# Quantco/tabmat

Hardware: AMD Instinct MI355X
Metric: SplitMatrix.sandwich GFLOP/s + effective HBM GB/s, 10M×1k mixed (higher is better)
Workload: dtype f64; 1 GPU; SplitMatrix.sandwich: dense128 + csr512@5% + cats(256,96,32), 10000000 rows/GPU, p=1024, float64 (BASELINE configs[3]); rows_per_gpu=10000000, p=1024, launch=eager, collective=none

## Files before the change

include/tabmat_hip.h:

```cpp
#ifndef TABMAT_HIP_H
#define TABMAT_HIP_H

#include <stddef.h>
#include <stdint.h>

#ifdef __cplusplus
extern "C" {
#endif

#define TM_OK 0
#define TM_EINVAL (-1)
#define TM_ENOMEM (-2)
#define TM_EUNSUPPORTED (-3)

int tm_version(void);
const char *tm_last_error(void);
int tm_device_count(int *count);
int tm_set_device(int device);
int tm_device_info(char *name, int name_len, int *compute_units, int64_t *hbm_bytes);
int tm_malloc(void **ptr, size_t bytes);
int tm_free(void *ptr);
int tm_memcpy_h2d(void *dst, const void *h_src, size_t bytes, void *stream);
int tm_memcpy_d2h(void *h_dst, const void *src, size_t bytes, void *stream);
int tm_memset(void *dst, int value, size_t bytes, void *stream);
// ... 408 lines not shown
                                    float *out, void *stream);
int tm_multi_cat_dense_sandwich_f64(const void *const *h_codes, const int64_t *h_ncols,
                                    const int32_t *h_drop_first, int n_cats, int64_t n,
                                    const double *d, const double *M, int64_t M_ncol, int order_f,
                                    double *out, void *stream);
int tm_multi_cat_dense_sandwich_rows_f32(const void *const *h_codes, const int64_t *h_ncols,
                                         const int32_t *h_drop_first, int n_cats, int64_t n,
                                         const float *d, const float *M, int64_t M_ncol,
                                         const int32_t *rows, int64_t n_rows, float *out,
                                         void *stream);
int tm_multi_cat_dense_sandwich_rows_f64(const void *const *h_codes, const int64_t *h_ncols,
                                         const int32_t *h_drop_first, int n_cats, int64_t n,
                                         const double *d, const double *M, int64_t M_ncol,
                                         const int32_t *rows, int64_t n_rows, double *out,
                                         void *stream);
int tm_multi_cat_sparse_sandwich_rows_f32(const void *const *h_codes, const int64_t *h_ncols,
                                          const int32_t *h_drop_first, int n_cats,
                                          const float *cm_data, const int32_t *cm_indices,
                                          const int32_t *row_ranges, const int32_t *rows,
                                          int64_t n_sel, int64_t m, const float *d_sel, float *out,
                                          void *stream);
int tm_multi_cat_sparse_sandwich_rows_f64(const void *const *h_codes, const int64_t *h_ncols,
                                          const int32_t *h_drop_first, int n_cats,
                                          const double *cm_data, const int32_t *cm_indices,
                                          const int32_t *row_ranges, const int32_t *rows,
                                          int64_t n_sel, int64_t m, const double *d_sel, double *out,
                                          void *stream);
int tm_multi_cat_sparse_sandwich_rows_u8_f32(const void *const *h_codes, const int64_t *h_ncols,
                                             const int32_t *h_drop_first, int n_cats,
                                             const float *cm_data, const uint8_t *cm_col8,
                                             const int32_t *row_ranges, const int32_t *rows,
                                             int64_t n_sel, int64_t m, const float *d_sel, float *out,
                                             void *stream);
int tm_multi_cat_sparse_sandwich_rows_u8_f64(const void *const *h_codes, const int64_t *h_ncols,
                                             const int32_t *h_drop_first, int n_cats,
                                             const double *cm_data, const uint8_t *cm_col8,
                                             const int32_t *row_ranges, const int32_t *rows,
                                             int64_t n_sel, int64_t m, const double *d_sel, double *out,
                                             void *stream);
int tm_multi_cat_sparse_sandwich_ent_f32(const void *const *h_codes, const int64_t *h_ncols,
                                         const int32_t *h_drop_first, int n_cats, int64_t n, const float *d,
                                         const float *vals, const uint16_t *meta, const uint32_t *bstart,
                                         int64_t n_slots, int64_t mk, float *out, void *stream);
int tm_multi_cat_sparse_sandwich_ent_f64(const void *const *h_codes, const int64_t *h_ncols,
                                         const int32_t *h_drop_first, int n_cats, int64_t n, const double *d,
                                         const double *vals, const uint16_t *meta, const uint32_t *bstart,
                                         int64_t n_slots, int64_t mk, double *out, void *stream);
int tm_multi_cat_pack_codes(const void *const *h_codes, const int64_t *h_ncols, const int32_t *h_drop_first, int n_cats,
                            int64_t n, uint32_t *packed, void *stream);
int tm_multi_cat_sparse_sandwich_entp_f32(const void *const *h_codes, const int64_t *h_ncols,
                                          const int32_t *h_drop_first, int n_cats, int64_t n, const float *d,
                                          const float *vals, const uint16_t *meta, const uint32_t *bstart,
                                          int64_t n_slots, int64_t mk, const uint32_t *packed, float *out, void *stream);
int tm_multi_cat_sparse_sandwich_entp_f64(const void *const *h_codes, const int64_t *h_ncols,
                                          const int32_t *h_drop_first, int n_cats, int64_t n, const double *d,
                                          const double *vals, const uint16_t *meta, const uint32_t *bstart,
                                          int64_t n_slots, int64_t mk, const uint32_t *packed, double *out, void *stream);

int tm_multi_cat_sparse_sandwich_slab_f32(const void *const *h_codes, const int64_t *h_ncols,
                                          const int32_t *h_drop_first, int n_cats, int64_t n,
                                          const float *d, const float *vals, const uint32_t *koff,
                                          const uint8_t *ecol, const int64_t *gptr, int64_t m,
                                          float *out, void *stream);
int tm_multi_cat_sparse_sandwich_slab_f64(const void *const *h_codes, const int64_t *h_ncols,
                                          const int32_t *h_drop_first, int n_cats, int64_t n,
                                          const double *d, const double *vals, const uint32_t *koff,
                                          const uint8_t *ecol, const int64_t *gptr, int64_t m,
                                          double *out, void *stream);

int tm_multi_cat_pairs_max_bins(void);
int tm_multi_cat_pairs_max_slots(void);
int tm_multi_cat_pairs_row_words(void);
int tm_multi_cat_pairs_f32(const int64_t *cat_tab, int64_t n, const float *d, const int32_t *rows,
                           int64_t n_rows, const int32_t *bundles, int n_bundles,
                           const int32_t *wg_map, int n_wg, int slots, int64_t bins,
                           const int64_t *desc, int64_t n_pairs, const int64_t *pos, double *tables,
                           double *out, int64_t p, void *stream);
int tm_multi_cat_pairs_f64(const int64_t *cat_tab, int64_t n, const double *d, const int32_t *rows,
                           int64_t n_rows, const int32_t *bundles, int n_bundles,
                           const int32_t *wg_map, int n_wg, int slots, int64_t bins,
                           const int64_t *desc, int64_t n_pairs, const int64_t *pos, double *tables,
                           double *out, int64_t p, void *stream);

int tm_multi_cat_matvec_f32(const int64_t *cat_tab, int n_cats, const int64_t *pos, const float *v,
                            int64_t n, float *out, void *stream);
int tm_multi_cat_matvec_f64(const int64_t *cat_tab, int n_cats, const int64_t *pos, const double *v,
                            int64_t n, double *out, void *stream);

int tm_csr_densify_cols_f32(const float *data, const int32_t *indices, const int64_t *indptr, int64_t n,
                            const int32_t *colmap, float *T, int64_t ld, void *stream);
int tm_csr_densify_cols_f64(const double *data, const int32_t *indices, const int64_t *indptr, int64_t n,
                            const int32_t *colmap, double *T, int64_t ld, void *stream);
int tm_csc_densify_cols_f32(const int32_t *rows, const float *vals, const int64_t *seg, const int32_t *tcol,
                            int64_t n_sel, int64_t max_len, float *T, int64_t ld, void *stream);
int tm_csc_densify_cols_f64(const int32_t *rows, const double *vals, const int64_t *seg, const int32_t *tcol,
                            int64_t n_sel, int64_t max_len, double *T, int64_t ld, void *stream);
int tm_dense_gather_cols_f32(const float *X, int64_t n, int64_t m, int order_f, const int32_t *cols,
                             int64_t n_sel, float *T, int64_t ld, int64_t t0, void *stream);
int tm_dense_gather_cols_f64(const double *X, int64_t n, int64_t m, int order_f, const int32_t *cols,
                             int64_t n_sel, double *T, int64_t ld, int64_t t0, void *stream);

int tm_scatter_block_f32(const float *src, int64_t nr, int64_t nc, const int64_t *ri,
                         const int64_t *ci, double *out, int64_t p, int mirror, int diag,
                         void *stream);
int tm_scatter_block_f64(const double *src, int64_t nr, int64_t nc, const int64_t *ri,
                         const int64_t *ci, double *out, int64_t p, int mirror, int diag,
                         void *stream);

int tm_sparse_sandwich_chunked_rows_f32(const float *cm_data, const int32_t *cm_indices,
                                        const int32_t *row_ranges, int64_t n_sel, int64_t m,
                                        int64_t nnz, const float *d_sel, float *out, void *stream);
int tm_sparse_sandwich_chunked_rows_f64(const double *cm_data, const int32_t *cm_indices,
                                        const int32_t *row_ranges, int64_t n_sel, int64_t m,
                                        int64_t nnz, const double *d_sel, double *out, void *stream);

int tm_sparse_sandwich_chunked_u8_f32(const float *cm_data, const uint8_t *cm_col8, const int32_t *cptr, int64_t n,
                                      int64_t m, int64_t nnz, const float *d, float *out, void *stream);
int tm_sparse_sandwich_chunked_u8_f64(const double *cm_data, const uint8_t *cm_col8, const int32_t *cptr, int64_t n,
                                      int64_t m, int64_t nnz, const double *d, double *out, void *stream);
int tm_sparse_sandwich_chunked_rows_u8_f32(const float *cm_data, const uint8_t *cm_col8, const int32_t *row_ranges,
                                           int64_t n_sel, int64_t m, int64_t nnz, const float *d_sel, float *out,
                                           void *stream);
int tm_sparse_sandwich_chunked_rows_u8_f64(const double *cm_data, const uint8_t *cm_col8, const int32_t *row_ranges,
                                           int64_t n_sel, int64_t m, int64_t nnz, const double *d_sel, double *out,
                                           void *stream);
int tm_sparse_sandwich_direct_f32(const float *csr_data, const int32_t *csr_indices,
                                  const int64_t *csr_indptr, int64_t n, int64_t m, const float *d,
                                  float *out, void *stream);
int tm_sparse_sandwich_direct_f64(const double *csr_data, const int32_t *csr_indices,
                                  const int64_t *csr_indptr, int64_t n, int64_t m, const double *d,
                                  double *out, void *stream);
int tm_csr_dense_sandwich_rows_f32(const float *cm_data, const int32_t *cm_indices,
                                   const int32_t *row_ranges, int64_t n_sel, const int32_t *rows,
                                   const float *d_sel, int64_t n, int64_t m, const float *B, int64_t r,
                                   int order_f, float *out, void *stream);
int tm_csr_dense_sandwich_rows_f64(const double *cm_data, const int32_t *cm_indices,
                                   const int32_t *row_ranges, int64_t n_sel, const int32_t *rows,
                                   const double *d_sel, int64_t n, int64_t m, const double *B, int64_t r,
                                   int order_f, double *out, void *stream);
int tm_csr_dense_sandwich_rows_u8_f32(const float *cm_data, const uint8_t *cm_col8,
                                      const int32_t *row_ranges, int64_t n_sel, const int32_t *rows,
                                      const float *d_sel, int64_t n, int64_t m, const float *B, int64_t r,
                                      int order_f, float *out, void *stream);
int tm_csr_dense_sandwich_rows_u8_f64(const double *cm_data, const uint8_t *cm_col8,
                                      const int32_t *row_ranges, int64_t n_sel, const int32_t *rows,
                                      const double *d_sel, int64_t n, int64_t m, const double *B, int64_t r,
                                      int order_f, double *out, void *stream);

int tm_cat_det_block_rows(void);
int tm_cat_transpose_matvec_det_f32(const int32_t *perm, const int64_t *bstart, int64_t n_blocks,
                                    const int64_t *cat_bptr, int64_t n_cols, const float *v,
                                    float *out, int accumulate, void *stream);
int tm_cat_transpose_matvec_det_f64(const int32_t *perm, const int64_t *bstart, int64_t n_blocks,
                                    const int64_t *cat_bptr, int64_t n_cols, const double *v,
                                    double *out, int accumulate, void *stream);

int tm_cat_dense_sandwich_sorted_f32(const int32_t *perm, const int64_t *bstart, int64_t n_blocks,
                                     const int64_t *cat_bptr, int64_t n_cols, const float *d,
                                     const float *Y, int64_t m, float *out, void *stream);
int tm_cat_dense_sandwich_sorted_f64(const int32_t *perm, const int64_t *bstart, int64_t n_blocks,
                                     const int64_t *cat_bptr, int64_t n_cols, const double *d,
                                     const double *Y, int64_t m, double *out, void *stream);
int tm_csc_dense_sandwich_sorted_f32(const int32_t *rows, const float *vals, const int64_t *bstart,
                                     int64_t n_blocks, const int64_t *col_bptr, int64_t n_cols,
                                     const float *d, const float *Y, int64_t m, float *out,
                                     void *stream);
// ... 56 lines not shown
```

tabmat_amd/csrc/cat.hip:

```cpp
#include <algorithm>

#include "common.hpp"
#include "reduce.hpp"

namespace tmh {

__global__ void fill_i32_kernel(int32_t *p, int64_t n, int32_t v) {
    int64_t i = (int64_t)blockIdx.x * blockDim.x + threadIdx.x;
    if (i < n) p[i] = v;
}

__global__ void scatter_iota_i32_kernel(int32_t *map, const int32_t *cols, int64_t n_cols) {
    int64_t i = (int64_t)blockIdx.x * blockDim.x + threadIdx.x;
    if (i < n_cols) map[cols[i]] = (int32_t)i;
}

int build_col_map(int32_t *map, int64_t m, const int32_t *cols, int64_t n_cols, hipStream_t st) {
    if (m > 0) {
        hipLaunchKernelGGL(fill_i32_kernel, dim3((unsigned)ceil_div(m, 256)), dim3(256), 0, st, map,
                           m, -1);
        TM_LAUNCH_CHECK();
    }
    if (n_cols > 0) {
        hipLaunchKernelGGL(scatter_iota_i32_kernel, dim3((unsigned)ceil_div(n_cols, 256)),
                           dim3(256), 0, st, map, cols, n_cols);
        TM_LAUNCH_CHECK();
    }
    return TM_OK;
}

template <typename F, bool TWO>
__global__ __launch_bounds__(1024) void hist_lds_kernel(
    const int32_t *__restrict__ ci, const int32_t *__restrict__ cj, const F *__restrict__ w,
    const int32_t *__restrict__ rows, int64_t n_iter, int64_t rows_per_block, int drop_i,
    int drop_j, int i_ncol, int j_ncol, int ti, const int32_t *__restrict__ col_map,
    F *__restrict__ ws, int64_t stride) {
    extern __shared__ __attribute__((aligned(16))) unsigned char smem_raw[];
    lds_acc_t *bins = reinterpret_cast<lds_acc_t *>(smem_raw);
    const int part = blockIdx.y;
    const int i0 = part * ti;
    const int i1 = min(i0 + ti, i_ncol);
    const int nbins = TWO ? (i1 - i0) * j_ncol : (i1 - i0);
    for (int b = threadIdx.x; b < nbins; b += blockDim.x) bins[b] = 0.0;
    __syncthreads();

    const int64_t t0 = (int64_t)blockIdx.x * rows_per_block;
    const int64_t t1 = min(t0 + rows_per_block, n_iter);
    int64_t tbeg = t0;
    if (!TWO && rows == nullptr && (t0 & 3) == 0 &&
        ((reinterpret_cast<uintptr_t>(ci) | reinterpret_cast<uintptr_t>(w)) & 15) == 0) {
        typedef int i4 __attribute__((ext_vector_type(4)));
        const int64_t nvec = (t1 - t0) / 4;
        for (int64_t q = threadIdx.x; q < nvec; q += blockDim.x) {
            const int64_t k = t0 + q * 4;
            const i4 cc = *reinterpret_cast<const i4 *>(ci + k);
            F ww[4];
#pragma unroll
            for (int e = 0; e < 4; ++e) ww[e] = w[k + e];
#pragma unroll
            for (int e = 0; e < 4; ++e) {
                const int c = cc[e] - drop_i;
                if (c >= i0 && c < i1 && !(col_map && col_map[c] < 0)) atomic_add(&bins[c - i0], (lds_acc_t)ww[e]);
            }
        }
        tbeg = t0 + nvec * 4;
    }
    for (int64_t t = tbeg + threadIdx.x; t < t1; t += blockDim.x) {
        const int64_t k = rows ? (int64_t)rows[t] : t;
        const int c = ci[k] - drop_i;
        if (c < i0 || c >= i1) continue;
        if (TWO) {
            const int c2 = cj[k] - drop_j;
            if (c2 < 0) continue;
            atomic_add(&bins[(c - i0) * j_ncol + c2], (lds_acc_t)w[k]);
        } else {
            if (col_map && col_map[c] < 0) continue;
            atomic_add(&bins[c - i0], (lds_acc_t)w[k]);
        }
    }
    __syncthreads();
    F *dst = ws + ((int64_t)part * gridDim.x + blockIdx.x) * stride;
    for (int b = threadIdx.x; b < nbins; b += blockDim.x) dst[b] = (F)bins[b];
}

template <typename F, bool TWO>
__global__ __launch_bounds__(256) void hist_global_kernel(
// ... 1137 lines not shown
        }
    }
    __syncthreads();
    F *dst = ws + ((int64_t)blockIdx.y * gridDim.x + blockIdx.x) * stride;
    for (int b = threadIdx.x; b < cs.total * GC; b += blockDim.x)
        dst[b] = (F)tile[(b / GC) * TSTR + (b % GC)];
}

template <typename F, typename IX>
__global__ __launch_bounds__(1024) void multi_cat_sparse_rows_kernel(
    CatSet cs, const F *__restrict__ cm_data, const IX *__restrict__ cm_ind,
    const int32_t *__restrict__ ranges, const int32_t *__restrict__ rows, const F *__restrict__ d_sel,
    int64_t n_sel, int64_t rows_per_block, F *__restrict__ ws, int64_t stride) {
    constexpr int GC = 32;
    extern __shared__ __attribute__((aligned(16))) unsigned char smem_raw[];
    lds_acc_t *tile = reinterpret_cast<lds_acc_t *>(smem_raw);
    constexpr int tstr = GC + 1;
    const int nel = cs.total * tstr;
    for (int b = threadIdx.x; b < nel; b += blockDim.x) tile[b] = 0.0;
    __syncthreads();
    static_assert(SPARSE_CHUNK_COLS == 4 * GC, "the chunk of the chunk-major twin must hold four 32-column groups");
    const int g = blockIdx.y;
    const int ch = g >> 2;
    const int lane = threadIdx.x & 63, wave = threadIdx.x >> 6, nwave = blockDim.x >> 6;
    const int lr = lane >> 3, lt = lane & 7;
    const int64_t t0 = (int64_t)blockIdx.x * rows_per_block;
    const int64_t t1 = min(t0 + rows_per_block, n_sel);
    const int32_t *rg = ranges + (int64_t)ch * n_sel * 2;
    for (int64_t k0 = t0 + wave * 8; k0 < t1; k0 += (int64_t)nwave * 8) {
        const int64_t k = k0 + lr;
        if (k >= t1) continue;
        const F dk = d_sel[k];
        if (dk == F(0)) continue;
        const int e0 = rg[2 * k], e1 = rg[2 * k + 1];
        if (e0 >= e1) continue;
        const int64_t row = rows[k];
        int off[MAX_CATS];
#pragma unroll
        for (int c = 0; c < MAX_CATS; ++c) {
            off[c] = -1;
            if (c < cs.n_cats) {
                const int col = cs.codes[c][row] - cs.drop[c];
                off[c] = col >= 0 ? (cs.off[c] + col) * tstr : -1;
            }
        }
        for (int e = e0 + lt; e < e1; e += 8) {
            const int col = (int)cm_ind[e] - (sizeof(IX) == 1 ? (g & 3) : g) * GC;
            if (col < 0 || col >= GC) continue;
            const lds_acc_t x = (lds_acc_t)(dk * cm_data[e]);
#pragma unroll
            for (int c = 0; c < MAX_CATS; ++c)
                if (off[c] >= 0) atomic_add(&tile[off[c] + col], x);
        }
    }
    __syncthreads();
    F *dst = ws + ((int64_t)blockIdx.y * gridDim.x + blockIdx.x) * stride;
    for (int b = threadIdx.x; b < cs.total * GC; b += blockDim.x)
        dst[b] = (F)tile[(b / GC) * tstr + (b % GC)];
}

static int make_catset(const void *const *h_codes, const int64_t *h_ncols, const int32_t *h_drop,
                       int n_cats, CatSet *cs) {
    if (n_cats < 1 || n_cats > MAX_CATS) {
        set_error("multi-cat call supports 1..%d categoricals, got %d", MAX_CATS, n_cats);
        return TM_EINVAL;
    }
    int off = 0;
    for (int c = 0; c < MAX_CATS; ++c) {
        cs->codes[c] = c < n_cats ? reinterpret_cast<const int32_t *>(h_codes[c]) : nullptr;
        cs->ncol[c] = c < n_cats ? (int)h_ncols[c] : 0;
        cs->drop[c] = c < n_cats ? h_drop[c] : 0;
        cs->off[c] = off;
        off += cs->ncol[c];
    }
    cs->n_cats = n_cats;
    cs->total = off;
    return TM_OK;
}

template <typename F>
static int run_multi_cat_dense(const void *const *h_codes, const int64_t *h_ncols,
                               const int32_t *h_drop, int n_cats, int64_t n, const F *d, const F *M,
                               int64_t m, int order_f, F *out, hipStream_t st,
                               const int32_t *rows = nullptr, int64_t n_rows = 0) {
    CatSet cs;
    int rc = make_catset(h_codes, h_ncols, h_drop, n_cats, &cs);
    if (rc) return rc;
    const int64_t total = (int64_t)cs.total * m;
    if (total == 0) return TM_OK;
    if (rows != nullptr) n = n_rows;
    if (n == 0) {
        TM_HIP(hipMemsetAsync(out, 0, sizeof(F) * (size_t)total, st));
        return TM_OK;
    }
    {
        constexpr int VEC = MCW_VEC;
        constexpr int TJW = 16 * VEC;
        const size_t tile_b = ((sizeof(lds_acc_t) * (size_t)cs.total * TJW + 15) / 16) * 16;
        const size_t lds_w = tile_b + (size_t)16 * MCW_RS * (sizeof(F) + (size_t)n_cats * sizeof(int));
        if (!order_f && n_cats <= 8 && m >= VEC && m % VEC == 0 &&
            (reinterpret_cast<uintptr_t>(M) & 15) == 0 && lds_w <= 150 * 1024 &&
            (int64_t)cs.total * TJW * (int64_t)sizeof(lds_acc_t) < (1ll << 30)) {
            const int64_t n_parts = ceil_div(m, TJW);
            const int64_t stride = (int64_t)cs.total * TJW;
            int64_t nblk = std::max<int64_t>(1, tune("catdense_rounds", 1) * NUM_CU / n_parts);
            nblk = std::min<int64_t>(nblk, std::max<int64_t>(1, ceil_div(n, 4096)));
            const int64_t rpb = ceil_div(ceil_div(n, nblk), MCW_RS) * MCW_RS;
            nblk = ceil_div(n, rpb);
            const size_t tmp_bytes = ((sizeof(F) * (size_t)(n_parts * stride) + 255) / 256) * 256;
            void *wsv = nullptr;
            rc = get_workspace(tmp_bytes + sizeof(F) * (size_t)(n_parts * nblk * stride) + 256, &wsv, st);
            if (rc) return rc;
            F *tmp = reinterpret_cast<F *>(wsv);
            F *ws = reinterpret_cast<F *>(reinterpret_cast<char *>(wsv) + tmp_bytes);
            auto gow = [&](auto kern) -> int {
                TM_HIP(hipFuncSetAttribute(reinterpret_cast<const void *>(kern),
                                           hipFuncAttributeMaxDynamicSharedMemorySize, (int)lds_w));
                prof_begin(st);
                const int nw_dflt = (sizeof(F) == 8 && tile_b > 64 * 1024) ? 8 : 16;
                const int nw = (int)std::min<int64_t>(16, std::max<int64_t>(4, tune("catdense_waves", nw_dflt)));
                hipLaunchKernelGGL(kern, dim3((unsigned)nblk, (unsigned)n_parts), dim3(nw * 64), lds_w, st,
                                   cs, d, M, n, m, rpb, ws, stride, rows, wg_log_ptr());
                prof_end(st);
                TM_LAUNCH_CHECK();
                return TM_OK;
            };
            if (n_cats == 1) rc = gow(&multi_cat_dense_wide_kernel<F, 1>);
            else if (n_cats == 2) rc = gow(&multi_cat_dense_wide_kernel<F, 2>);
            else if (n_cats == 3) rc = gow(&multi_cat_dense_wide_kernel<F, 3>);
            else if (n_cats == 4) rc = gow(&multi_cat_dense_wide_kernel<F, 4>);
            else if (n_cats == 5) rc = gow(&multi_cat_dense_wide_kernel<F, 5>);
            else if (n_cats == 6) rc = gow(&multi_cat_dense_wide_kernel<F, 6>);
            else if (n_cats == 7) rc = gow(&multi_cat_dense_wide_kernel<F, 7>);
            else rc = gow(&multi_cat_dense_wide_kernel<F, 8>);
            if (rc) return rc;
            rc = launch_reduce_partials<F>(ws, stride, (int)nblk, (int)n_parts, tmp, n_parts * stride,
                                           false, st);
            if (rc) return rc;
            hipLaunchKernelGGL((multi_cat_untile_kernel<F>), dim3((unsigned)ceil_div(total, 256)),
                               dim3(256), 0, st, tmp, (int64_t)cs.total, m, TJW, out);
            TM_LAUNCH_CHECK();
            return TM_OK;
        }
    }
    if (rows != nullptr) {
        set_error("multi_cat_dense: the row-list form needs the wide-load path");
        return TM_EUNSUPPORTED;
    }
    int TJ = 64;
    while (TJ > 1 && sizeof(lds_acc_t) * (size_t)cs.total * TJ > HIST_LDS_MAX) TJ >>= 1;
    while (TJ > 1 && TJ / 2 >= m) TJ >>= 1;
    if (sizeof(lds_acc_t) * (size_t)cs.total * TJ > HIST_LDS_MAX) {
        set_error("multi_cat_dense: %d stacked categories exceed the LDS tile", cs.total);
        return TM_EUNSUPPORTED;
    }
    const int64_t n_parts = ceil_div(m, TJ);
    const int64_t stride = (int64_t)cs.total * TJ;
    const size_t lds = sizeof(lds_acc_t) * (size_t)stride;
    int64_t nblk = std::max<int64_t>(1, NUM_CU / n_parts);
    nblk = std::min<int64_t>(nblk, std::max<int64_t>(1, ceil_div(n, 4096)));
    const int64_t rpb = ceil_div(n, nblk);
    nblk = ceil_div(n, rpb);
    const size_t tmp_bytes = ((sizeof(F) * (size_t)(n_parts * stride) + 255) / 256) * 256;
    void *wsv = nullptr;
    rc = get_workspace(tmp_bytes + sizeof(F) * (size_t)(n_parts * nblk * stride) + 256, &wsv, st);
    if (rc) return rc;
    F *tmp = reinterpret_cast<F *>(wsv);
    F *ws = reinterpret_cast<F *>(reinterpret_cast<char *>(wsv) + tmp_bytes);
    auto go = [&](auto kern) -> int {
        if (lds > 48 * 1024)
            TM_HIP(hipFuncSetAttribute(reinterpret_cast<const void *>(kern),
                                       hipFuncAttributeMaxDynamicSharedMemorySize, (int)lds));
        prof_begin(st);
        hipLaunchKernelGGL(kern, dim3((unsigned)nblk, (unsigned)n_parts), dim3(1024), lds, st, cs, d,
                           M, n, m, rpb, ws, stride);
        prof_end(st);
        TM_LAUNCH_CHECK();
        return TM_OK;
    };
#define TM_MCD_CASE(V)                                                                       \
    case V:                                                                                  \
        if (order_f) rc = go(&multi_cat_dense_f_kernel<F, V>);                               \
        else if (n_cats == 1) rc = go(&multi_cat_dense_c_kernel<F, V, 1>);                   \
        else if (n_cats == 2) rc = go(&multi_cat_dense_c_kernel<F, V, 2>);                   \
        else if (n_cats == 3) rc = go(&multi_cat_dense_c_kernel<F, V, 3>);                   \
        else if (n_cats == 4) rc = go(&multi_cat_dense_c_kernel<F, V, 4>);                   \
        else rc = go(&multi_cat_dense_c_kernel<F, V, 0>);                                    \
        break;
    switch (TJ) {
        TM_MCD_CASE(64)
        TM_MCD_CASE(32)
        TM_MCD_CASE(16)
        TM_MCD_CASE(8)
        TM_MCD_CASE(4)
        TM_MCD_CASE(2)
        TM_MCD_CASE(1)
        default:
            rc = TM_EINVAL;
    }
#undef TM_MCD_CASE
    if (rc) return rc;
    rc = launch_reduce_partials<F>(ws, stride, (int)nblk, (int)n_parts, tmp, n_parts * stride, false,
                                   st);
    if (rc) return rc;
    hipLaunchKernelGGL((multi_cat_untile_kernel<F>), dim3((unsigned)ceil_div(total, 256)),
                       dim3(256), 0, st, tmp, (int64_t)cs.total, m, TJ, out);
    TM_LAUNCH_CHECK();
    return TM_OK;
}

template <typename F, typename IX>
static int run_multi_cat_sparse_rows(const void *const *h_codes, const int64_t *h_ncols,
                                     const int32_t *h_drop, int n_cats, const F *cm_data,
                                     const IX *cm_ind, const int32_t *ranges, const int32_t *rows,
                                     int64_t n_sel, int64_t m, const F *d_sel, F *out, hipStream_t st);

template <typename F>
static int run_multi_cat_sparse(const void *const *h_codes, const int64_t *h_ncols,
                                const int32_t *h_drop, int n_cats, int64_t n, const F *d,
                                const F *vals, const unsigned *koff, const unsigned char *ecol,
                                const int64_t *gptr, int64_t m, int slab_rows, int group_cols,
                                F *out, hipStream_t st) {
    CatSet cs;
    int rc = make_catset(h_codes, h_ncols, h_drop, n_cats, &cs);
    if (rc) return rc;
    const int64_t total = (int64_t)cs.total * m;
    if (total == 0) return TM_OK;
    if (n == 0) {
        TM_HIP(hipMemsetAsync(out, 0, sizeof(F) * (size_t)total, st));
        return TM_OK;
    }
    const int64_t stride = (int64_t)cs.total * group_cols;
    const size_t tile_bytes = ((sizeof(lds_acc_t) * (size_t)cs.total * (group_cols + 1) + 15) / 16) * 16;
    if (tile_bytes > HIST_LDS_MAX) {
        set_error("multi_cat_sparse: %d stacked categories exceed the LDS tile", cs.total);
        return TM_EUNSUPPORTED;
    }
    const int nw = (int)std::min<int64_t>(16, std::max<int64_t>(4, tune("catsparse_waves", 16)));
    const size_t stage_bytes = (size_t)nw * slab_rows * (sizeof(F) + sizeof(int32_t) * (size_t)n_cats);
    const bool stage = tile_bytes + stage_bytes <= 150 * 1024;
    const size_t lds = tile_bytes + (stage ? stage_bytes : 0);
    const int n_groups = (int)ceil_div(m, group_cols);
    const int64_t n_slabs = ceil_div(n, slab_rows);
    int64_t nblk = std::max<int64_t>(1, tune("catsparse_rounds", 1) * NUM_CU / n_groups);
    nblk = std::min<int64_t>(nblk, n_slabs);
    const int64_t spb = ceil_div(n_slabs, nblk);
    nblk = ceil_div(n_slabs, spb);
    const size_t tmp_bytes = ((sizeof(F) * (size_t)(n_groups * stride) + 255) / 256) * 256;
    void *wsv = nullptr;
    rc = get_workspace(tmp_bytes + sizeof(F) * (size_t)((int64_t)n_groups * nblk * stride) + 256,
                       &wsv, st);
    if (rc) return rc;
    F *tmp = reinterpret_cast<F *>(wsv);
    F *ws = reinterpret_cast<F *>(reinterpret_cast<char *>(wsv) + tmp_bytes);
    if (stage && n_cats <= 8 && slab_rows == 128) {
        auto kpf = n_cats == 1   ? &multi_cat_sparse_pf_kernel<F, 1>
                   : n_cats == 2 ? &multi_cat_sparse_pf_kernel<F, 2>
                   : n_cats == 3 ? &multi_cat_sparse_pf_kernel<F, 3>
                   : n_cats == 4 ? &multi_cat_sparse_pf_kernel<F, 4>
                   : n_cats == 5 ? &multi_cat_sparse_pf_kernel<F, 5>
                   : n_cats == 6 ? &multi_cat_sparse_pf_kernel<F, 6>
                   : n_cats == 7 ? &multi_cat_sparse_pf_kernel<F, 7>
                                 : &multi_cat_sparse_pf_kernel<F, 8>;
        if (lds > 48 * 1024)
            TM_HIP(hipFuncSetAttribute(reinterpret_cast<const void *>(kpf),
                                       hipFuncAttributeMaxDynamicSharedMemorySize, (int)lds));
        prof_begin(st);
        hipLaunchKernelGGL(kpf, dim3((unsigned)nblk, (unsigned)n_groups), dim3(nw * 64), lds, st, cs, d,
                           vals, koff, ecol, gptr, n_groups, n_slabs, spb, group_cols, n, ws, stride,
                           wg_log_ptr());
        prof_end(st);
        TM_LAUNCH_CHECK();
    } else {
        auto kern = stage ? &multi_cat_sparse_kernel<F, true> : &multi_cat_sparse_kernel<F, false>;
        if (lds > 48 * 1024)
            TM_HIP(hipFuncSetAttribute(reinterpret_cast<const void *>(kern),
                                       hipFuncAttributeMaxDynamicSharedMemorySize, (int)lds));
        prof_begin(st);
        hipLaunchKernelGGL(kern, dim3((unsigned)nblk, (unsigned)n_groups), dim3(nw * 64), lds, st, cs,
                           d, vals, koff, ecol, gptr, n_groups, n_slabs, spb, slab_rows, group_cols,
                           n, ws, stride);
        prof_end(st);
        TM_LAUNCH_CHECK();
    }
    rc = launch_reduce_partials<F>(ws, stride, (int)nblk, n_groups, tmp,
                                   (int64_t)n_groups * stride, false, st);
    if (rc) return rc;
    hipLaunchKernelGGL((multi_cat_untile_kernel<F>), dim3((unsigned)ceil_div(total, 256)),
                       dim3(256), 0, st, tmp, (int64_t)cs.total, m, group_cols, out);
    TM_LAUNCH_CHECK();
    return TM_OK;
}

__global__ __launch_bounds__(256) void multi_cat_pack_codes_kernel(CatSet cs, int64_t n, unsigned *__restrict__ out) {
    for (int64_t r = (int64_t)blockIdx.x * blockDim.x + threadIdx.x; r < n; r += (int64_t)gridDim.x * blockDim.x) {
        unsigned pk = 0u;
#pragma unroll
        for (int c = 0; c < 3; ++c) {
            unsigned f = 1023u;
            if (c < cs.n_cats) {
                const int col = cs.codes[c][r] - cs.drop[c];
                if (col >= 0 && col < cs.ncol[c]) f = (unsigned)(cs.off[c] + col);
            }
            pk |= f << (10 * c);
        }
        out[r] = pk;
    }
}

template <typename F>
static int run_multi_cat_sparse_ent(const void *const *h_codes, const int64_t *h_ncols, const int32_t *h_drop,
                                    int n_cats, int64_t n, const F *d, const F *vals, const unsigned short *meta,
                                    const unsigned *bstart, int64_t mk, F *out, hipStream_t st,
                                    const unsigned *packed = nullptr, int64_t n_slots = 0) {
    CatSet cs;
    int rc = make_catset(h_codes, h_ncols, h_drop, n_cats, &cs);
    if (rc) return rc;
    const int64_t total = (int64_t)cs.total * mk;
    if (total == 0) return TM_OK;
    if (n == 0) {
        TM_HIP(hipMemsetAsync(out, 0, sizeof(F) * (size_t)total, st));
        return TM_OK;
    }
    TM_REQUIRE(mk % 16 == 0 && n_cats >= 1 && n_cats <= 8, "kernel columns in groups of 16, 1 .. 8 categoricals");
    TM_REQUIRE(n < (1ll << 28), "at most 2^28 - 1 rows per block");
    constexpr int GC = 32;
    const int64_t stride = (int64_t)cs.total * GC;
    const size_t lds = ((sizeof(lds_acc_t) * (size_t)cs.total * (GC + 1) + 15) / 16) * 16;
    if (lds > HIST_LDS_MAX) {
        set_error("multi_cat_sparse_ent: %d stacked categories exceed the LDS tile", cs.total);
        return TM_EUNSUPPORTED;
    }
    const int nw = (int)std::min<int64_t>(16, std::max<int64_t>(4, tune("catsparse_waves", 16)));
    const int n_groups = (int)(mk / 16);
    const int n_pairs = (n_groups + 1) / 2;
    const int64_t n_slabs = ceil_div(n, 64);
    int64_t nblk = std::max<int64_t>(1, tune("catsparse_rounds", 1) * NUM_CU / n_pairs);
    nblk = std::min<int64_t>(nblk, n_slabs);
    const int64_t spb = ceil_div(n_slabs, nblk);
    nblk = ceil_div(n_slabs, spb);
    const size_t tmp_bytes = ((sizeof(F) * (size_t)(n_pairs * stride) + 255) / 256) * 256;
    void *wsv = nullptr;
    rc = get_workspace(tmp_bytes + sizeof(F) * (size_t)((int64_t)n_pairs * nblk * stride) + 256, &wsv, st);
    if (rc) return rc;
    F *tmp = reinterpret_cast<F *>(wsv);
    F *ws = reinterpret_cast<F *>(reinterpret_cast<char *>(wsv) + tmp_bytes);
    auto kern = n_cats == 1   ? &multi_cat_sparse_ent_kernel<F, 1>
                : n_cats == 2 ? &multi_cat_sparse_ent_kernel<F, 2>
                : n_cats == 3 ? &multi_cat_sparse_ent_kernel<F, 3>
                : n_cats == 4 ? &multi_cat_sparse_ent_kernel<F, 4>
                : n_cats == 5 ? &multi_cat_sparse_ent_kernel<F, 5>
                : n_cats == 6 ? &multi_cat_sparse_ent_kernel<F, 6>
                : n_cats == 7 ? &multi_cat_sparse_ent_kernel<F, 7>
                              : &multi_cat_sparse_ent_kernel<F, 8>;
    TM_REQUIRE(packed == nullptr || (n_cats <= 3 && cs.total < 1023), "packed codes: at most 3 categoricals, 1022 levels");
    const int ncw = packed != nullptr ? 1 : n_cats;
    const size_t lds_staged = lds + (size_t)nw * 64 * (sizeof(F) + 4 * (size_t)ncw);
    const double fill = (double)n_slots / ((double)std::max(n_groups, 1) * (double)n_slabs);
    if (tune("catsparse_staged", 1) != 0 && lds_staged <= 156 * 1024 &&
        fill >= (double)tune("catsparse_staged_fill", 44)) {
        using KS = void (*)(CatSet, const F *, const F *, const unsigned short *, const unsigned *, int, int64_t, int64_t,
                            int64_t, F *, int64_t, const unsigned *, int);
        KS ks = nullptr;
        if (packed != nullptr) {
            ks = n_cats == 1 ? &multi_cat_sparse_ent_staged_kernel<F, 1, true>
                 : n_cats == 2 ? &multi_cat_sparse_ent_staged_kernel<F, 2, true>
                               : &multi_cat_sparse_ent_staged_kernel<F, 3, true>;
        } else {
            ks = n_cats == 1   ? &multi_cat_sparse_ent_staged_kernel<F, 1, false>
                 : n_cats == 2 ? &multi_cat_sparse_ent_staged_kernel<F, 2, false>
                 : n_cats == 3 ? &multi_cat_sparse_ent_staged_kernel<F, 3, false>
                 : n_cats == 4 ? &multi_cat_sparse_ent_staged_kernel<F, 4, false>
                 : n_cats == 5 ? &multi_cat_sparse_ent_staged_kernel<F, 5, false>
                 : n_cats == 6 ? &multi_cat_sparse_ent_staged_kernel<F, 6, false>
                 : n_cats == 7 ? &multi_cat_sparse_ent_staged_kernel<F, 7, false>
                               : &multi_cat_sparse_ent_staged_kernel<F, 8, false>;
        }
        if (lds_staged > 48 * 1024)
            TM_HIP(hipFuncSetAttribute(reinterpret_cast<const void *>(ks),
                                       hipFuncAttributeMaxDynamicSharedMemorySize, (int)lds_staged));
        prof_begin(st);
        hipLaunchKernelGGL(ks, dim3((unsigned)nblk, (unsigned)n_pairs), dim3(nw * 64), lds_staged, st, cs, d, vals,
                           meta, bstart, n_groups, n, n_slabs, spb, ws, stride, packed, (int)lds);
        prof_end(st);
        TM_LAUNCH_CHECK();
    } else {
        if (lds > 48 * 1024)
            TM_HIP(hipFuncSetAttribute(reinterpret_cast<const void *>(kern),
                                       hipFuncAttributeMaxDynamicSharedMemorySize, (int)lds));
        prof_begin(st);
        hipLaunchKernelGGL(kern, dim3((unsigned)nblk, (unsigned)n_pairs), dim3(nw * 64), lds, st, cs, d, vals, meta,
                           bstart, n_groups, n, n_slabs, spb, ws, stride, packed);
        prof_end(st);
        TM_LAUNCH_CHECK();
    }
    rc = launch_reduce_partials<F>(ws, stride, (int)nblk, n_pairs, tmp, (int64_t)n_pairs * stride, false, st);
    if (rc) return rc;
    hipLaunchKernelGGL((multi_cat_untile_kernel<F>), dim3((unsigned)ceil_div(total, 256)), dim3(256), 0, st, tmp,
                       (int64_t)cs.total, mk, GC, out);
    TM_LAUNCH_CHECK();
    return TM_OK;
}

}

using namespace tmh;

#define TM_CHECK_COMMON(nn) \
    TM_REQUIRE((nn) >= 0, "negative size")

extern "C" {

int tm_cat_transpose_matvec_f32(const int32_t *codes, int64_t n, int64_t n_cols, int drop_first,
                                const float *v, const int32_t *rows, int64_t n_rows,
                                const int32_t *cols, int64_t n_cols_sel, float *out, void *stream) {
    TM_CHECK_COMMON(n);
    return run_cat_tmv<float>(codes, n, n_cols, drop_first, v, rows, n_rows, cols, n_cols_sel, out,
                              as_stream(stream));
}
int tm_cat_transpose_matvec_f64(const int32_t *codes, int64_t n, int64_t n_cols, int drop_first,
                                const double *v, const int32_t *rows, int64_t n_rows,
                                const int32_t *cols, int64_t n_cols_sel, double *out,
                                void *stream) {
    TM_CHECK_COMMON(n);
    return run_cat_tmv<double>(codes, n, n_cols, drop_first, v, rows, n_rows, cols, n_cols_sel,
                               out, as_stream(stream));
}

int tm_cat_matvec_f32(const int32_t *codes, int64_t n, int64_t n_cols, int drop_first,
                      const float *v, const int32_t *cols, int64_t n_cols_sel, float *out,
                      void *stream) {
    TM_CHECK_COMMON(n);
    return run_cat_matvec<float>(codes, n, n_cols, drop_first, v, cols, n_cols_sel, out,
                                 as_stream(stream));
}
int tm_cat_matvec_f64(const int32_t *codes, int64_t n, int64_t n_cols, int drop_first,
                      const double *v, const int32_t *cols, int64_t n_cols_sel, double *out,
                      void *stream) {
    TM_CHECK_COMMON(n);
    return run_cat_matvec<double>(codes, n, n_cols, drop_first, v, cols, n_cols_sel, out,
                                  as_stream(stream));
}

int tm_cat_matvec_assign_f32(const int32_t *codes, int64_t n, int64_t n_cols, int drop_first,
                             const float *v, const int32_t *cols, int64_t n_cols_sel, float *out,
                             void *stream) {
    TM_CHECK_COMMON(n);
    return run_cat_matvec<float>(codes, n, n_cols, drop_first, v, cols, n_cols_sel, out,
                                 as_stream(stream), true);
}
int tm_cat_matvec_assign_f64(const int32_t *codes, int64_t n, int64_t n_cols, int drop_first,
                             const double *v, const int32_t *cols, int64_t n_cols_sel, double *out,
                             void *stream) {
    TM_CHECK_COMMON(n);
    return run_cat_matvec<double>(codes, n, n_cols, drop_first, v, cols, n_cols_sel, out,
                                  as_stream(stream), true);
}

int tm_cat_cat_sandwich_f32(const int32_t *i_codes, const int32_t *j_codes, int64_t n,
                            const float *d, const int32_t *rows, int64_t n_rows, int64_t i_ncol,
                            int64_t j_ncol, int i_drop_first, int j_drop_first, float *out,
                            void *stream) {
    TM_CHECK_COMMON(n);
    return run_hist<float, true>(i_codes, j_codes, d, rows, rows ? n_rows : n, i_drop_first,
                                 j_drop_first, i_ncol, j_ncol, nullptr, out, false,
                                 as_stream(stream));
}
int tm_cat_cat_sandwich_f64(const int32_t *i_codes, const int32_t *j_codes, int64_t n,
                            const double *d, const int32_t *rows, int64_t n_rows, int64_t i_ncol,
                            int64_t j_ncol, int i_drop_first, int j_drop_first, double *out,
                            void *stream) {
    TM_CHECK_COMMON(n);
    return run_hist<double, true>(i_codes, j_codes, d, rows, rows ? n_rows : n, i_drop_first,
                                  j_drop_first, i_ncol, j_ncol, nullptr, out, false,
                                  as_stream(stream));
}

int tm_cat_cat_sandwich_atomic_f32(const int32_t *i_codes, const int32_t *j_codes, int64_t n,
// ... 30 lines not shown
                                   as_stream(stream));
}

int tm_cat_dense_sandwich_f32(const int32_t *codes, int64_t n, int64_t i_ncol, int drop_first,
                              const float *d, const int32_t *rows, int64_t n_rows, const float *M,
                              int64_t M_ncol, int order_f, const int32_t *j_cols, int64_t n_j,
                              float *out, void *stream) {
    TM_CHECK_COMMON(n);
    return run_cat_dense<float>(codes, n, i_ncol, drop_first, d, rows, n_rows, M, M_ncol, order_f,
                                j_cols, j_cols ? n_j : M_ncol, out, as_stream(stream));
}
int tm_cat_dense_sandwich_f64(const int32_t *codes, int64_t n, int64_t i_ncol, int drop_first,
                              const double *d, const int32_t *rows, int64_t n_rows,
                              const double *M, int64_t M_ncol, int order_f, const int32_t *j_cols,
                              int64_t n_j, double *out, void *stream) {
    TM_CHECK_COMMON(n);
    return run_cat_dense<double>(codes, n, i_ncol, drop_first, d, rows, n_rows, M, M_ncol, order_f,
                                 j_cols, j_cols ? n_j : M_ncol, out, as_stream(stream));
}

int tm_cat_sparse_sandwich_f32(const int32_t *codes, int64_t n, int64_t i_ncol, int drop_first,
                               const float *csr_data, const int32_t *csr_indices,
                               const int64_t *csr_indptr, int64_t s_ncol, const float *d,
                               const int32_t *rows, int64_t n_rows, const int32_t *cols,
                               int64_t n_cols, float *out, void *stream) {
    TM_CHECK_COMMON(n);
    return run_cat_sparse<float>(codes, n, i_ncol, drop_first, csr_data, csr_indices, csr_indptr,
                                 s_ncol, d, rows, n_rows, cols, n_cols, out, as_stream(stream));
}
int tm_cat_sparse_sandwich_f64(const int32_t *codes, int64_t n, int64_t i_ncol, int drop_first,
                               const double *csr_data, const int32_t *csr_indices,
                               const int64_t *csr_indptr, int64_t s_ncol, const double *d,
                               const int32_t *rows, int64_t n_rows, const int32_t *cols,
                               int64_t n_cols, double *out, void *stream) {
    TM_CHECK_COMMON(n);
    return run_cat_sparse<double>(codes, n, i_ncol, drop_first, csr_data, csr_indices, csr_indptr,
                                  s_ncol, d, rows, n_rows, cols, n_cols, out, as_stream(stream));
}

int tm_multi_cat_dense_sandwich_f32(const void *const *h_codes, const int64_t *h_ncols,
                                    const int32_t *h_drop_first, int n_cats, int64_t n,
                                    const float *d, const float *M, int64_t M_ncol, int order_f,
                                    float *out, void *stream) {
    return run_multi_cat_dense<float>(h_codes, h_ncols, h_drop_first, n_cats, n, d, M, M_ncol,
                                      order_f, out, as_stream(stream));
}
int tm_multi_cat_dense_sandwich_f64(const void *const *h_codes, const int64_t *h_ncols,
                                    const int32_t *h_drop_first, int n_cats, int64_t n,
                                    const double *d, const double *M, int64_t M_ncol, int order_f,
                                    double *out, void *stream) {
    return run_multi_cat_dense<double>(h_codes, h_ncols, h_drop_first, n_cats, n, d, M, M_ncol,
                                       order_f, out, as_stream(stream));
}
int tm_multi_cat_dense_sandwich_rows_f32(const void *const *h_codes, const int64_t *h_ncols,
                                         const int32_t *h_drop_first, int n_cats, int64_t n,
                                         const float *d, const float *M, int64_t M_ncol,
                                         const int32_t *rows, int64_t n_rows, float *out,
                                         void *stream) {
    return run_multi_cat_dense<float>(h_codes, h_ncols, h_drop_first, n_cats, n, d, M, M_ncol, 0, out,
                                      as_stream(stream), rows, n_rows);
}
int tm_multi_cat_dense_sandwich_rows_f64(const void *const *h_codes, const int64_t *h_ncols,
                                         const int32_t *h_drop_first, int n_cats, int64_t n,
                                         const double *d, const double *M, int64_t M_ncol,
                                         const int32_t *rows, int64_t n_rows, double *out,
                                         void *stream) {
    return run_multi_cat_dense<double>(h_codes, h_ncols, h_drop_first, n_cats, n, d, M, M_ncol, 0, out,
                                       as_stream(stream), rows, n_rows);
}
int tm_multi_cat_sparse_sandwich_ent_f32(const void *const *h_codes, const int64_t *h_ncols,
                                         const int32_t *h_drop_first, int n_cats, int64_t n, const float *d,
                                         const float *vals, const uint16_t *meta, const uint32_t *bstart,
                                         int64_t n_slots, int64_t mk, float *out, void *stream) {
    return run_multi_cat_sparse_ent<float>(h_codes, h_ncols, h_drop_first, n_cats, n, d, vals, meta, bstart, mk,
                                           out, as_stream(stream), nullptr, n_slots);
}
int tm_multi_cat_sparse_sandwich_ent_f64(const void *const *h_codes, const int64_t *h_ncols,
                                         const int32_t *h_drop_first, int n_cats, int64_t n, const double *d,
                                         const double *vals, const uint16_t *meta, const uint32_t *bstart,
                                         int64_t n_slots, int64_t mk, double *out, void *stream) {
    return run_multi_cat_sparse_ent<double>(h_codes, h_ncols, h_drop_first, n_cats, n, d, vals, meta, bstart, mk,
                                            out, as_stream(stream), nullptr, n_slots);
}
int tm_multi_cat_pack_codes(const void *const *h_codes, const int64_t *h_ncols, const int32_t *h_drop_first, int n_cats,
                            int64_t n, uint32_t *packed, void *stream) {
    CatSet cs;
    int rc = make_catset(h_codes, h_ncols, h_drop_first, n_cats, &cs);
    if (rc) return rc;
    TM_REQUIRE(n_cats <= 3 && cs.total < 1023, "packed codes: at most 3 categoricals, 1022 stacked levels");
    if (n == 0) return TM_OK;
    hipLaunchKernelGGL(multi_cat_pack_codes_kernel, dim3((unsigned)std::min<int64_t>(4 * NUM_CU, ceil_div(n, 256))),
                       dim3(256), 0, as_stream(stream), cs, n, packed);
    TM_LAUNCH_CHECK();
    return TM_OK;
}
int tm_multi_cat_sparse_sandwich_entp_f32(const void *const *h_codes, const int64_t *h_ncols,
                                          const int32_t *h_drop_first, int n_cats, int64_t n, const float *d,
                                          const float *vals, const uint16_t *meta, const uint32_t *bstart,
                                          int64_t n_slots, int64_t mk, const uint32_t *packed, float *out, void *stream) {
    return run_multi_cat_sparse_ent<float>(h_codes, h_ncols, h_drop_first, n_cats, n, d, vals, meta, bstart, mk, out,
                                           as_stream(stream), packed, n_slots);
}
int tm_multi_cat_sparse_sandwich_entp_f64(const void *const *h_codes, const int64_t *h_ncols,
                                          const int32_t *h_drop_first, int n_cats, int64_t n, const double *d,
                                          const double *vals, const uint16_t *meta, const uint32_t *bstart,
                                          int64_t n_slots, int64_t mk, const uint32_t *packed, double *out, void *stream) {
    return run_multi_cat_sparse_ent<double>(h_codes, h_ncols, h_drop_first, n_cats, n, d, vals, meta, bstart, mk,
                                            out, as_stream(stream), packed, n_slots);
}
int tm_multi_cat_sparse_sandwich_slab_f32(const void *const *h_codes, const int64_t *h_ncols,
                                          const int32_t *h_drop_first, int n_cats, int64_t n,
                                          const float *d, const float *vals, const uint32_t *koff,
                                          const uint8_t *ecol, const int64_t *gptr, int64_t m,
                                          float *out, void *stream) {
    return run_multi_cat_sparse<float>(h_codes, h_ncols, h_drop_first, n_cats, n, d, vals, koff,
                                       ecol, gptr, m, tm_slab_rows(), tm_slab_group_cols(), out,
                                       as_stream(stream));
}
int tm_multi_cat_sparse_sandwich_slab_f64(const void *const *h_codes, const int64_t *h_ncols,
                                          const int32_t *h_drop_first, int n_cats, int64_t n,
                                          const double *d, const double *vals, const uint32_t *koff,
                                          const uint8_t *ecol, const int64_t *gptr, int64_t m,
                                          double *out, void *stream) {
    return run_multi_cat_sparse<double>(h_codes, h_ncols, h_drop_first, n_cats, n, d, vals, koff,
                                        ecol, gptr, m, tm_slab_rows(), tm_slab_group_cols(), out,
                                        as_stream(stream));
}

}

namespace tmh {
template <typename F, typename IX>
static int run_multi_cat_sparse_rows(const void *const *h_codes, const int64_t *h_ncols,
                                     const int32_t *h_drop, int n_cats, const F *cm_data,
                                     const IX *cm_ind, const int32_t *ranges, const int32_t *rows,
                                     int64_t n_sel, int64_t m, const F *d_sel, F *out, hipStream_t st) {
    CatSet cs;
    int rc = make_catset(h_codes, h_ncols, h_drop, n_cats, &cs);
    if (rc) return rc;
    const int64_t total = (int64_t)cs.total * m;
    if (total == 0) return TM_OK;
    if (n_sel == 0) {
        TM_HIP(hipMemsetAsync(out, 0, sizeof(F) * (size_t)total, st));
        return TM_OK;
    }
    constexpr int GC = 32;
    const size_t lds = ((sizeof(lds_acc_t) * (size_t)cs.total * (GC + 1) + 15) / 16) * 16;
    if (lds > HIST_LDS_MAX) {
        set_error("multi_cat_sparse_rows: %d stacked categories exceed the LDS tile", cs.total);
        return TM_EUNSUPPORTED;
    }
    const int n_groups = (int)ceil_div(m, GC);
    const int64_t stride = (int64_t)cs.total * GC;
    int64_t nblk = std::max<int64_t>(1, tune("catsparse_rounds", 1) * NUM_CU / n_groups);
    nblk = std::min<int64_t>(nblk, std::max<int64_t>(1, ceil_div(n_sel, 2048)));
    const int64_t rpb = ceil_div(n_sel, nblk);
    nblk = ceil_div(n_sel, rpb);
    const size_t tmp_bytes = ((sizeof(F) * (size_t)(n_groups * stride) + 255) / 256) * 256;
    void *wsv = nullptr;
    rc = get_workspace(tmp_bytes + sizeof(F) * (size_t)((int64_t)n_groups * nblk * stride) + 256, &wsv, st);
    if (rc) return rc;
    F *tmp = reinterpret_cast<F *>(wsv);
    F *ws = reinterpret_cast<F *>(reinterpret_cast<char *>(wsv) + tmp_bytes);
    auto kern = &multi_cat_sparse_rows_kernel<F, IX>;
    if (lds > 48 * 1024)
        TM_HIP(hipFuncSetAttribute(reinterpret_cast<const void *>(kern),
// ... 58 lines not shown
```

tabmat_amd/csrc/cat_pairs.hip:

```cpp
#include "common.hpp"
#include "reduce.hpp"

namespace tmh {

constexpr int CP_BINS = 16384;
constexpr int CP_SLOTS = 16;
constexpr int CP_ROW = 8 + 4 * CP_SLOTS;
constexpr int CP_NEG = -(1 << 28);

template <typename F, int NS>
__global__ __launch_bounds__(1024) void multi_cat_pairs_kernel(
    const int64_t *__restrict__ cat_tab, const F *__restrict__ d, const int32_t *__restrict__ rows,
    int64_t n_iter, const int32_t *__restrict__ bundles, const int32_t *__restrict__ wg_map,
    int max_bins, double *__restrict__ ws) {
    extern __shared__ double tile[];
    const int y = __builtin_amdgcn_readfirstlane(wg_map[blockIdx.x]);
    const int32_t *br = bundles + (int64_t)y * CP_ROW;
    const int na = __builtin_amdgcn_readfirstlane(br[0]), nb = __builtin_amdgcn_readfirstlane(br[1]);
    const int mode = __builtin_amdgcn_readfirstlane(br[2]), lbs = __builtin_amdgcn_readfirstlane(br[3]);
    const int wg0 = __builtin_amdgcn_readfirstlane(br[4]);
    const int bins = __builtin_amdgcn_readfirstlane(br[6]);
    const int parts = (int)min((int64_t)__builtin_amdgcn_readfirstlane(br[5]),
                               max((int64_t)1, (n_iter + 8191) / 8192));
    const int part = (int)blockIdx.x - wg0;
    if (part >= parts) return;
    for (int b = threadIdx.x; b < bins; b += blockDim.x) tile[b] = 0.0;
    __syncthreads();
    const int32_t *pa[NS], *pb[NS];
    int dropa[NS], dropb[NS], offa[NS], offb[NS];
    static_for<NS>([&](auto sc) {
        constexpr int s = decltype(sc)::value;
        pa[s] = pb[s] = nullptr;
        dropa[s] = dropb[s] = offa[s] = offb[s] = 0;
        if (s < na) {
            const int id = __builtin_amdgcn_readfirstlane(br[8 + 2 * s]);
            offa[s] = __builtin_amdgcn_readfirstlane(br[9 + 2 * s]);
            pa[s] = reinterpret_cast<const int32_t *>(cat_tab[4 * id]);
            dropa[s] = (int)cat_tab[4 * id + 1];
        }
        if (s < nb) {
            const int id = __builtin_amdgcn_readfirstlane(br[8 + 2 * CP_SLOTS + 2 * s]);
            offb[s] = __builtin_amdgcn_readfirstlane(br[9 + 2 * CP_SLOTS + 2 * s]);
            pb[s] = reinterpret_cast<const int32_t *>(cat_tab[4 * id]);
            dropb[s] = (int)cat_tab[4 * id + 1];
        }
    });
    constexpr int UNR = NS <= 8 ? 4 : 2;
    const int64_t rpp = (n_iter + parts - 1) / parts;
    const int64_t t0 = (int64_t)part * rpp, t1 = min(t0 + rpp, n_iter);
    for (int64_t tb = t0; tb < t1; tb += (int64_t)UNR * blockDim.x) {
        int64_t k[UNR], kc[UNR];
        double dk[UNR];
        int ya[UNR][NS], xb[UNR][NS];
#pragma unroll
        for (int u = 0; u < UNR; ++u) {
            const int64_t t = tb + (int64_t)u * blockDim.x + threadIdx.x;
            k[u] = t < t1 ? (rows ? (int64_t)rows[t] : t) : -1;
        }
#pragma unroll
        for (int u = 0; u < UNR; ++u) {
            kc[u] = k[u] >= 0 ? k[u] : 0;
            dk[u] = (double)d[kc[u]];
        }
        static_for<NS>([&](auto sc) {
            constexpr int s = decltype(sc)::value;
            if (s < na) {
#pragma unroll
                for (int u = 0; u < UNR; ++u) ya[u][s] = __builtin_nontemporal_load(pa[s] + kc[u]);
            }
        });
        if (mode == 0) {
            static_for<NS>([&](auto sc) {
                constexpr int s = decltype(sc)::value;
                if (s < nb) {
#pragma unroll
                    for (int u = 0; u < UNR; ++u) xb[u][s] = __builtin_nontemporal_load(pb[s] + kc[u]);
                }
            });
        }
        bool live[UNR];
#pragma unroll
        for (int u = 0; u < UNR; ++u) {
            if (k[u] < 0) dk[u] = 0.0;
            live[u] = dk[u] != 0.0;
        }
        static_for<NS>([&](auto sc) {
            constexpr int s = decltype(sc)::value;
#pragma unroll
            for (int u = 0; u < UNR; ++u) {
                const int ca = ya[u][s] - dropa[s];
                const int cb = (mode == 0 ? xb[u][s] : ya[u][s]) - dropb[s];
                ya[u][s] = (s < na && live[u] && ca >= 0) ? offa[s] + ca * lbs : CP_NEG;
                xb[u][s] = mode == 2 ? 0 : ((s < nb && cb >= 0) ? offb[s] + cb : CP_NEG);
            }
        });
        static_for<NS>([&](auto ac) {
            constexpr int a = decltype(ac)::value;
            if (a < na) {
                static_for<NS>([&](auto bc) {
                    constexpr int b = decltype(bc)::value;
                    const bool on = b == a ? (mode != 0 || b < nb)
                                           : (b < nb && (mode == 0 || (mode == 1 && b > a)));
                    if (on) {
#pragma unroll
                        for (int u = 0; u < UNR; ++u) {
                            const int bin = ya[u][a] + xb[u][b];
                            if (bin >= 0) atomicAdd(tile + bin, dk[u]);
                        }
                    }
                });
            }
        });
    }
    __syncthreads();
    double *dst = ws + (int64_t)blockIdx.x * max_bins;
    for (int b = threadIdx.x; b < bins; b += blockDim.x) dst[b] = tile[b];
}

__global__ __launch_bounds__(256) void multi_cat_pairs_reduce_kernel(
    const double *__restrict__ ws, const int32_t *__restrict__ bundles, int64_t n_iter, int max_bins,
    double *__restrict__ tables) {
    __shared__ double part_sum[4][64];
    const int32_t *br = bundles + (int64_t)blockIdx.x * CP_ROW;
    const int wg0 = br[4], bins = br[6];
    const int parts = (int)min((int64_t)br[5], max((int64_t)1, (n_iter + 8191) / 8192));
    const int lane = threadIdx.x & 63, sl = threadIdx.x >> 6;
    for (int e0 = blockIdx.y * 64; e0 < bins; e0 += gridDim.y * 64) {
        const int e = e0 + lane;
        double s0 = 0.0, s1 = 0.0;
        if (e < bins) {
            int q = sl;
            for (; q + 4 < parts; q += 8) {
                s0 += ws[(int64_t)(wg0 + q) * max_bins + e];
                s1 += ws[(int64_t)(wg0 + q + 4) * max_bins + e];
            }
            if (q < parts) s0 += ws[(int64_t)(wg0 + q) * max_bins + e];
        }
        part_sum[sl][lane] = s0 + s1;
        __syncthreads();
        if (sl == 0 && e < bins)
            tables[(int64_t)blockIdx.x * max_bins + e] =
                (part_sum[0][lane] + part_sum[1][lane]) + (part_sum[2][lane] + part_sum[3][lane]);
        __syncthreads();
    }
}

__global__ __launch_bounds__(256) void multi_cat_pairs_scatter_kernel(
    const double *__restrict__ tables, const int64_t *__restrict__ desc,
    const int64_t *__restrict__ pos, double *__restrict__ out, int64_t p) {
    const int64_t *q = desc + (int64_t)blockIdx.x * 8;
    const int64_t toff = q[0], li = q[1], lj = q[2], w = q[3], pi = q[4], pj = q[5];
    const bool diag = q[6] != 0;
    const int64_t total = diag ? li : li * lj;
    for (int64_t e = (int64_t)blockIdx.y * blockDim.x + threadIdx.x; e < total;
         e += (int64_t)gridDim.y * blockDim.x) {
        if (diag) {
            const int64_t r = pos[pi + e];
            if (r >= 0) out[r * p + r] = tables[toff + e * w];
        } else {
            const int64_t ei = e / lj, ej = e % lj;
            const double v = tables[toff + ei * w + ej];
            const int64_t r = pos[pi + ei], cc = pos[pj + ej];
            if (r >= 0 && cc >= 0) {
                out[r * p + cc] = v;
                out[cc * p + r] = v;
            }
        }
    }
}

template <typename F>
__global__ __launch_bounds__(256) void multi_cat_matvec_kernel(
    const int64_t *__restrict__ cat_tab, int n_cats, const int64_t *__restrict__ pos,
    const F *__restrict__ v, int64_t n, F *__restrict__ out) {
    constexpr int UNR = 4;
    const int lane = threadIdx.x & 63;
// ... 165 lines not shown
```

tabmat_amd/csrc/sparse_blocks.hip:

```cpp
#include <algorithm>

#include "common.hpp"
#include "reduce.hpp"

namespace tmh {

constexpr int KB_WAVES = 16;
constexpr int KB_TS = 128;

template <typename F>
__global__ void blocks_assemble_kernel(const F *__restrict__ tiles, int n_out, F *__restrict__ out) {
    const int j = blockIdx.x * blockDim.x + threadIdx.x;
    const int i = blockIdx.y;
    if (i >= n_out || j >= n_out) return;
    const int hi = max(i, j), lo = min(i, j);
    const int I = hi / KB_TS, J = lo / KB_TS;
    const int part = I * (I + 1) / 2 + J;
    out[(int64_t)i * n_out + j] = tiles[(int64_t)part * KB_TS * KB_TS + (hi % KB_TS) * KB_TS + (lo % KB_TS)];
}

constexpr int KB_FLAG_REP_A = 1 << 16;
constexpr int KB_FLAG_REP_B = 1 << 17;

template <typename F, bool U8, bool D12 = false>
__global__ __launch_bounds__(KB_WAVES * 64) void sparse_sandwich_blocks_kernel(
    const F *__restrict__ data, const int32_t *__restrict__ ind, const int32_t *__restrict__ cptr,
    int64_t n, int64_t nnz1, const int32_t *__restrict__ blocks, const int4 *__restrict__ wg_tab,
    const F *__restrict__ d, int max_nb, F *__restrict__ ws, WgLogBuf *__restrict__ wglog) {
    constexpr int TS = KB_TS;
    const unsigned long long t_begin = wg_log_begin(wglog);
    extern __shared__ __attribute__((aligned(16))) unsigned char smem_raw[];
    lds_acc_t *tile = reinterpret_cast<lds_acc_t *>(smem_raw);
    const int4 w = wg_tab[2 * blockIdx.x], x = wg_tab[2 * blockIdx.x + 1];
    const int part = __builtin_amdgcn_readfirstlane(w.x), slot = __builtin_amdgcn_readfirstlane(w.y);
    const int b0 = __builtin_amdgcn_readfirstlane(w.z), b1 = __builtin_amdgcn_readfirstlane(w.w);
    const int bfull = __builtin_amdgcn_readfirstlane(x.x);
    int wfull = __builtin_amdgcn_readfirstlane(x.y);
    {
        const int nwv = (int)(blockDim.x >> 6);
        if (nwv != KB_WAVES) {
            wfull = (wfull * nwv + KB_WAVES / 2) / KB_WAVES;
            if (bfull > b0) wfull = max(wfull, 1);
            if (b1 > bfull) wfull = min(wfull, nwv - 1);
            if (bfull == b0) wfull = 0;
            if (b1 == bfull) wfull = nwv;
        }
    }
    int I = (int)((sqrtf(8.0f * (float)part + 1.0f) - 1.0f) * 0.5f);
    while ((I + 1) * (I + 2) / 2 <= part) ++I;
    while (I * (I + 1) / 2 > part) --I;
    const int J = part - I * (I + 1) / 2;
    const int i0 = I * TS, j0 = J * TS;
    for (int b = threadIdx.x; b < TS * TS; b += blockDim.x) tile[b] = 0.0;
    __syncthreads();

    const int lane = threadIdx.x & 63;
    const int wave = __builtin_amdgcn_readfirstlane(threadIdx.x >> 6);
    const int lr = lane >> 3, lt = lane & 7;
    if (b1 > b0) {
        const int row_first = __builtin_amdgcn_readfirstlane(x.z), row_last = __builtin_amdgcn_readfirstlane(x.w);
        const int32_t *cpA = cptr + (int64_t)I * (n + 1), *cpB = cptr + (int64_t)J * (n + 1);
        const int baseA = __builtin_amdgcn_readfirstlane(cpA[row_first]);
        const int baseB = __builtin_amdgcn_readfirstlane(cpB[row_first]);
        const unsigned spanA1 = (unsigned)max(__builtin_amdgcn_readfirstlane(cpA[row_last + 1]) - baseA - 1, 0);
        const unsigned spanB1 = (unsigned)max(__builtin_amdgcn_readfirstlane(cpB[row_last + 1]) - baseB - 1, 0);
        const F *dataA = data + min((int64_t)baseA, nnz1), *dataB = data + min((int64_t)baseB, nnz1);
        const int32_t *indA = ind + min((int64_t)baseA, nnz1), *indB = ind + min((int64_t)baseB, nnz1);
        const unsigned char *ind8 = reinterpret_cast<const unsigned char *>(ind);
        const unsigned char *ind8A = ind8 + min((int64_t)baseA, nnz1), *ind8B = ind8 + min((int64_t)baseB, nnz1);
        const int i0c = U8 ? 0 : i0, j0c = U8 ? 0 : j0;
        const unsigned nrow1 = (unsigned)max(n - 1, (int64_t)0);
        auto ldi = [](const int32_t *base, unsigned i) {
            return *reinterpret_cast<const int32_t *>(reinterpret_cast<const char *>(base) + (i << 2));
        };
        auto ldf = [](const F *base, unsigned i) {
            return *reinterpret_cast<const F *>(reinterpret_cast<const char *>(base) + (i * (unsigned)sizeof(F)));
        };
        constexpr int SH = 3;
        constexpr int BIGKEY = 0x7ffffff0;
        char *const tile_bytes = reinterpret_cast<char *>(tile);
        auto add_pair = [&](int kb, int la, int ba, F prod) {
            if (kb <= la)
                atomic_add(reinterpret_cast<lds_acc_t *>(tile_bytes + (unsigned)(kb ^ ba)), (lds_acc_t)prod);
        };

        auto run_list = [&](auto diag_c, auto full_c, int s0, int s1, int w0, int nw) {
// ... 34 lines not shown
                const unsigned iA = min((unsigned)(sd.q.x - baseA) + min((unsigned)e.ta, (unsigned)max(e.nA - 1, 0)), spanA1);
                const unsigned iB = min((unsigned)(sd.q.y - baseB) + min((unsigned)e.tb, (unsigned)max(e.nB - 1, 0)), spanB1);
#ifdef KB_ABL_WRAP
                const unsigned iAw = iA & (unsigned)(KB_ABL_WRAP), iBw = iB & (unsigned)(KB_ABL_WRAP);
                e.ca = ldi(indA, min(iAw, spanA1));
                e.va = ldf(dataA, min(iAw, spanA1));
                e.cb = ldi(indB, min(iBw, spanB1));
                e.vb = ldf(dataB, min(iBw, spanB1));
                return e;
#endif
                e.ca = U8 ? (int)ind8A[iA] : ldi(indA, iA);
                e.va = ldf(dataA, iA);
                e.cb = U8 ? (int)ind8B[iB] : ldi(indB, iB);
                e.vb = ldf(dataB, iB);
                return e;
            };
            auto process = [&](const Grp &cur) {
                __builtin_amdgcn_s_setprio(1);
                const int colA = cur.ta < cur.nA ? cur.ca - i0c : -1;
                const int colB = cur.tb < cur.nB ? cur.cb - j0c : -1;
                const int la = (colA < 0 ? -8 : colA << SH) | offmask;
                const int ba = (int)(((unsigned)colA << (7 + SH)) | ((colA & 15) << (3 + SH)));
                const int kb = colB < 0 ? BIGKEY : colB << SH;
                const F av = cur.va * cur.d, vb = cur.vb;
                add_pair(kb, la, ba, av * vb);
                add_pair(dpp_xor_i32<1>(kb), la, ba, av * dpp_xor<1>(vb));
                add_pair(dpp_xor_i32<2>(kb), la, ba, av * dpp_xor<2>(vb));
                add_pair(dpp_xor_i32<3>(kb), la, ba, av * dpp_xor<3>(vb));
#ifndef KB_ABL_HALFSTEPS
                if constexpr (FULL) {
                    const int kb4 = dpp_xor_i32<4>(kb);
                    const F vb4 = dpp_xor<4>(vb);
                    add_pair(kb4, la, ba, av * vb4);
                    add_pair(dpp_xor_i32<1>(kb4), la, ba, av * dpp_xor<1>(vb4));
                    add_pair(dpp_xor_i32<2>(kb4), la, ba, av * dpp_xor<2>(vb4));
                    add_pair(dpp_xor_i32<3>(kb4), la, ba, av * dpp_xor<3>(vb4));
                }
#endif
                __builtin_amdgcn_s_setprio(0);
            };
            const int gstep = nw * 8;
            const int gw = (wave - w0) * 8;
            Grp ea[2], eb[2];
            Dsc ps[2];
            ea[0] = load_entries(load_desc(gw));
            ea[1] = load_entries(load_desc(gw + gstep));
            ps[0] = load_desc(gw + 2 * gstep);
            ps[1] = load_desc(gw + 3 * gstep);
            for (int g = gw; g < nseg; g += 4 * gstep) {
                eb[0] = load_entries(ps[0]);
                eb[1] = load_entries(ps[1]);
                ps[0] = load_desc(g + 4 * gstep);
                ps[1] = load_desc(g + 5 * gstep);
                process(ea[0]);
                if (g + gstep < nseg) process(ea[1]);
                if (g + 2 * gstep >= nseg) break;
                ea[0] = load_entries(ps[0]);
                ea[1] = load_entries(ps[1]);
                ps[0] = load_desc(g + 6 * gstep);
                ps[1] = load_desc(g + 7 * gstep);
                process(eb[0]);
                if (g + 3 * gstep < nseg) process(eb[1]);
            }
        };
        auto run_tile = [&](auto diag_c) {
            if (wave < wfull) run_list(diag_c, std::true_type{}, b0, bfull, 0, wfull);
            else run_list(diag_c, std::false_type{}, bfull, b1, wfull, (int)(blockDim.x >> 6) - wfull);
        };
        if (I == J) run_tile(std::true_type{});
        else run_tile(std::false_type{});
    }
    __syncthreads();
    if (threadIdx.x == 0) wg_log_end(wglog, t_begin, WG_K2);
    F *dst = ws + ((int64_t)part * max_nb + slot) * (TS * TS);
    for (int b = threadIdx.x; b < TS * TS; b += blockDim.x) {
        const int r = b / TS, c = b % TS;
        dst[b] = (F)tile[r * TS + (c ^ ((r & 15) << 3))];
    }
}

template <typename F, bool U8 = false, bool D12 = false>
static int run_sparse_sandwich_blocks(const F *data, const int32_t *ind, const int32_t *cptr, int64_t n,
                                      int64_t m, int64_t nnz, const int32_t *blocks, const int32_t *wg_tab,
                                      int n_wg, int max_nb, const F *d, F *out, hipStream_t st) {
    if (m == 0) return TM_OK;
    if (n == 0 || nnz == 0 || n_wg == 0) {
        TM_HIP(hipMemsetAsync(out, 0, sizeof(F) * (size_t)(m * m), st));
        return TM_OK;
    }
    constexpr int TS = KB_TS;
    const int nchunk = (int)ceil_div(m, TS);
    const int n_parts = nchunk * (nchunk + 1) / 2;
    TM_REQUIRE(nnz < (1ll << 31) && n < (1ll << 29), "sparse block too large for the block-list sandwich");
    TM_REQUIRE(!D12 || n < (1ll << 24), "12-byte block descriptors hold 24 bits of row");
    TM_REQUIRE(max_nb >= 1 && n_wg >= 1, "empty workgroup table");
    const size_t lds = sizeof(lds_acc_t) * (size_t)(TS * TS);
    const size_t tmp_bytes = (sizeof(F) * (size_t)n_parts * TS * TS + 255) / 256 * 256;
    const size_t ws_bytes = sizeof(F) * (size_t)n_parts * (size_t)max_nb * TS * TS;
    void *wsv = nullptr;
    int rc = get_workspace(tmp_bytes + ws_bytes + 256, &wsv, st);
    if (rc) return rc;
    F *tmp = reinterpret_cast<F *>(wsv);
    F *ws = reinterpret_cast<F *>(reinterpret_cast<char *>(wsv) + tmp_bytes);
    TM_HIP(hipMemsetAsync(ws, 0, ws_bytes, st));
    auto kern = &sparse_sandwich_blocks_kernel<F, U8, D12>;
    TM_HIP(hipFuncSetAttribute(reinterpret_cast<const void *>(kern),
                               hipFuncAttributeMaxDynamicSharedMemorySize, (int)lds));
    prof_begin(st);
    const int kb_waves = (int)std::min<int64_t>(KB_WAVES, std::max<int64_t>(2, tune("k2b_waves", KB_WAVES)));
    hipLaunchKernelGGL(kern, dim3((unsigned)n_wg), dim3(kb_waves * 64), lds, st, data, ind, cptr, n, nnz - 1,
                       blocks, reinterpret_cast<const int4 *>(wg_tab), d,
                       max_nb, ws, wg_log_ptr());
    prof_end(st);
    TM_LAUNCH_CHECK();
    rc = launch_reduce_partials<F>(ws, (int64_t)TS * TS, max_nb, n_parts, tmp, (int64_t)n_parts * TS * TS,
                                   false, st);
    if (rc) return rc;
    hipLaunchKernelGGL((blocks_assemble_kernel<F>), dim3((unsigned)ceil_div(m, 64), (unsigned)m), dim3(64),
                       0, st, tmp, (int)m, out);
    TM_LAUNCH_CHECK();
    return TM_OK;
}

}

extern "C" {

int tm_sparse_sandwich_blocks_f32(const float *cm_data, const int32_t *cm_indices, const int32_t *cptr,
                                  int64_t n, int64_t m, int64_t nnz, const int32_t *blocks,
                                  const int32_t *wg_tab, int n_wg, int max_nb, const float *d, float *out,
                                  void *stream) {
    return tmh::run_sparse_sandwich_blocks<float>(cm_data, cm_indices, cptr, n, m, nnz, blocks, wg_tab, n_wg,
                                                  max_nb, d, out, tmh::as_stream(stream));
}
int tm_sparse_sandwich_blocks_f64(const double *cm_data, const int32_t *cm_indices, const int32_t *cptr,
                                  int64_t n, int64_t m, int64_t nnz, const int32_t *blocks,
                                  const int32_t *wg_tab, int n_wg, int max_nb, const double *d, double *out,
                                  void *stream) {
    return tmh::run_sparse_sandwich_blocks<double>(cm_data, cm_indices, cptr, n, m, nnz, blocks, wg_tab, n_wg,
                                                   max_nb, d, out, tmh::as_stream(stream));
}

int tm_sparse_sandwich_blocks_u8_f32(const float *cm_data, const uint8_t *cm_col8, const int32_t *cptr,
                                     int64_t n, int64_t m, int64_t nnz, const int32_t *blocks,
                                     const int32_t *wg_tab, int n_wg, int max_nb, const float *d, float *out,
                                     void *stream) {
    return tmh::run_sparse_sandwich_blocks<float, true>(cm_data, reinterpret_cast<const int32_t *>(cm_col8), cptr, n, m,
                                                        nnz, blocks, wg_tab, n_wg, max_nb, d, out,
                                                        tmh::as_stream(stream));
}
int tm_sparse_sandwich_blocks_u8_f64(const double *cm_data, const uint8_t *cm_col8, const int32_t *cptr,
                                     int64_t n, int64_t m, int64_t nnz, const int32_t *blocks,
                                     const int32_t *wg_tab, int n_wg, int max_nb, const double *d, double *out,
                                     void *stream) {
    return tmh::run_sparse_sandwich_blocks<double, true>(cm_data, reinterpret_cast<const int32_t *>(cm_col8), cptr, n, m,
                                                         nnz, blocks, wg_tab, n_wg, max_nb, d, out,
                                                         tmh::as_stream(stream));
}

int tm_sparse_sandwich_blocks_p12_f32(const float *cm_data, const uint8_t *cm_col8, const int32_t *cptr,
                                      int64_t n, int64_t m, int64_t nnz, const int32_t *blocks12,
                                      const int32_t *wg_tab, int n_wg, int max_nb, const float *d, float *out,
                                      void *stream) {
    return tmh::run_sparse_sandwich_blocks<float, true, true>(cm_data, reinterpret_cast<const int32_t *>(cm_col8), cptr,
                                                              n, m, nnz, blocks12, wg_tab, n_wg, max_nb, d, out,
                                                              tmh::as_stream(stream));
}
int tm_sparse_sandwich_blocks_p12_f64(const double *cm_data, const uint8_t *cm_col8, const int32_t *cptr,
                                      int64_t n, int64_t m, int64_t nnz, const int32_t *blocks12,
                                      const int32_t *wg_tab, int n_wg, int max_nb, const double *d, double *out,
                                      void *stream) {
    return tmh::run_sparse_sandwich_blocks<double, true, true>(cm_data, reinterpret_cast<const int32_t *>(cm_col8), cptr,
                                                               n, m, nnz, blocks12, wg_tab, n_wg, max_nb, d, out,
                                                               tmh::as_stream(stream));
}

}
```

tabmat_amd/csrc/sparse_ent.hip:

```cpp
#include "common.hpp"
#include "reduce.hpp"

namespace tmh {

constexpr int EN_R = 64;
constexpr int EN_C = 16;
constexpr int EN_NW = 16;
constexpr int EN_THREADS = EN_NW * 64;
constexpr int EN_W = 128;
constexpr int EN_B = 16;
constexpr int EN_SB = 64;

template <typename F>
struct EnLds {
    static constexpr int ROWB = EN_W * (int)sizeof(F);
    static constexpr int SLABB = EN_R * ROWB;
    static constexpr int SCR_OFF = ROWB + 2 * SLABB;
    static constexpr int CS_OFF = SCR_OFF + EN_NW * EN_SB * 16;
    static constexpr int TOTAL = CS_OFF + EN_NW * EN_C * (int)sizeof(double);
};

constexpr int EN_CVGPR = 24;
#define EN_LD "40"

#if defined(__HIP_DEVICE_COMPILE__)
typedef __amdgpu_buffer_rsrc_t en_rsrc_t;
__device__ __forceinline__ en_rsrc_t en_rsrc(const void *base, int64_t bytes) {
    const unsigned nb = bytes <= 0 ? 0u : (bytes > 0xFFFFFFFFll ? 0xFFFFFFFFu : (unsigned)bytes);
    return __builtin_amdgcn_make_buffer_rsrc(const_cast<void *>(base), 0, (int)nb, 0x00020000);
}
__device__ __forceinline__ void en_buf_to_lds16(en_rsrc_t rs, void *lds, int voff, int soff) {
    __builtin_amdgcn_raw_ptr_buffer_load_lds(rs, (__attribute__((address_space(3))) void *)lds, 16, voff,
                                             soff, 0, 0);
}
template <typename F>
__device__ __forceinline__ void en_zero_acc() {
    if constexpr (sizeof(F) == 8) {
        static_for<16>([&](auto jc) {
            asm volatile("v_mov_b32 v[64+4*%0], 0\n\tv_mov_b32 v[64+4*%0+1], 0\n\t"
                         "v_mov_b32 v[64+4*%0+2], 0\n\tv_mov_b32 v[64+4*%0+3], 0"
                         :: "n"(decltype(jc)::value) : "v127");
        });
    } else {
        static_for<16>([&](auto jc) {
            asm volatile("v_mov_b32 v[64+2*%0], 0\n\tv_mov_b32 v[64+2*%0+1], 0" :: "n"(decltype(jc)::value) : "v95");
        });
    }
}
template <int K>
__device__ __forceinline__ unsigned en_read_acc() {
    unsigned x;
    asm volatile("v_mov_b32 %0, v[64+%1]" : "=v"(x) : "n"(K));
    return x;
}
template <typename F>
__device__ __forceinline__ void en_load_stream(unsigned voff_v, const F *vp, unsigned voff_m, const unsigned short *mp) {
    if constexpr (sizeof(F) == 8)
        asm volatile("global_load_dwordx2 v[" EN_LD ":" EN_LD "+1], %0, %1\n\t"
                     "global_load_ushort v[" EN_LD "+2], %2, %3" :: "v"(voff_v), "s"(vp), "v"(voff_m), "s"(mp) : "memory");
    else
        asm volatile("global_load_dword v[" EN_LD "], %0, %1\n\t"
                     "global_load_ushort v[" EN_LD "+2], %2, %3" :: "v"(voff_v), "s"(vp), "v"(voff_m), "s"(mp) : "memory");
}
template <typename F>
__device__ __forceinline__ void en_load_d(unsigned voff, const F *dp) {
    if constexpr (sizeof(F) == 8)
        asm volatile("global_load_dwordx2 v[" EN_LD "+4:" EN_LD "+5], %0, %1" :: "v"(voff), "s"(dp) : "memory");
    else
        asm volatile("global_load_dword v[" EN_LD "+4], %0, %1" :: "v"(voff), "s"(dp) : "memory");
}
template <int N>
__device__ __forceinline__ void en_take(double &v, unsigned &m, double &dd) {
    unsigned vl, vh, dl, dh;
    asm volatile("s_waitcnt vmcnt(%5)\n\t"
                 "v_mov_b32 %0, v[" EN_LD "]\n\tv_mov_b32 %1, v[" EN_LD "+1]\n\tv_mov_b32 %2, v[" EN_LD "+2]\n\t"
                 "v_mov_b32 %3, v[" EN_LD "+4]\n\tv_mov_b32 %4, v[" EN_LD "+5]"
                 : "=v"(vl), "=v"(vh), "=v"(m), "=v"(dl), "=v"(dh) : "n"(N) : "memory");
    v = __hiloint2double((int)vh, (int)vl);
    dd = __hiloint2double((int)dh, (int)dl);
}
template <int N>
__device__ __forceinline__ void en_take(float &v, unsigned &m, float &dd) {
    unsigned vl, dl;
    asm volatile("s_waitcnt vmcnt(%3)\n\t"
// ... 194 lines not shown
        if (q != 3) enext = scratch[(q + 1) * EN_B + l16];
        EN_TICK(pt_a)
        const int slab = __builtin_amdgcn_readlane((int)e[3], 1);
        while (w < slab) end_slab();
        if (ncopied == 0 && w + 1 < ns) {
            issue_pieces((w & 1) ^ 1, 0, NV);

            ncopied = NV;
            psince += NV;
            lsince = 0;
        }
        EN_TICK(pt_p)
        F a;
        if constexpr (sizeof(F) == 8) a = __hiloint2double((int)e[1], (int)e[0]);
        else a = __uint_as_float(e[0]);
#if defined(EN_ABL_NOBATCH)
        asm volatile("" ::"v"(a), "v"(e[2]), "v"(e[3]));
#else
        const unsigned live = (unsigned)__builtin_amdgcn_ballot_w64(a != F(0)) & 0xffffu;
        const int nq = live ? ((31 - __builtin_clz(live)) >> 2) + 1 : 0;
        unsigned p0 = (unsigned)__builtin_amdgcn_readlane((int)e[3], 0);
        unsigned p1 = (unsigned)__builtin_amdgcn_readlane((int)e[3], 4);
        unsigned p2 = (unsigned)__builtin_amdgcn_readlane((int)e[3], 8);
        unsigned p3 = (unsigned)__builtin_amdgcn_readlane((int)e[3], 12);
        if (nq == 4) en_batch_asm<16, F>(p0, p1, p2, p3, a, e[2], lane_off);
        else if (nq == 3) en_batch_asm<12, F>(p0, p1, p2, p3, a, e[2], lane_off);
        else if (nq == 2) en_batch_asm<8, F>(p0, p1, p2, p3, a, e[2], lane_off);
        else if (nq == 1) en_batch_asm<4, F>(p0, p1, p2, p3, a, e[2], lane_off);
#endif
        EN_TICK(pt_x)
#if defined(EN_PROF)
        ++pt_n;
#endif
    }
    while (w < ns) end_slab();
    wait_loads(std::integral_constant<int, 0>{});
#if defined(EN_PROF)
    if (prof != nullptr && lane == 0) {
        long long *o = prof + (((int64_t)blockIdx.z * gridDim.y + blockIdx.y) * gridDim.x + blockIdx.x) * (EN_NW * 8) + wave * 8;
        o[0] = pt_a; o[1] = pt_p; o[2] = pt_x; o[3] = pt_b; o[4] = pt_bar; o[5] = pt_n; o[6] = clock64() - pt_start; o[7] = ns;
    }
#endif

    if (active) {
        F *dst = ws + (((int64_t)blockIdx.y * gridDim.x + blockIdx.x) * n_groups + group) * (EN_C * EN_W);
        static_for<EN_C>([&](auto jc) {
            constexpr int j = decltype(jc)::value;
            if constexpr (sizeof(F) == 8) {
                const u4 o = u4{en_read_acc<4 * j>(), en_read_acc<4 * j + 1>(), en_read_acc<4 * j + 2>(),
                                en_read_acc<4 * j + 3>()};
                *reinterpret_cast<u4 *>(dst + j * EN_W + 2 * lane) = o;
            } else {
                typedef unsigned u2 __attribute__((ext_vector_type(2)));
                const u2 o = u2{en_read_acc<2 * j>(), en_read_acc<2 * j + 1>()};
                *reinterpret_cast<u2 *>(dst + j * EN_W + 2 * lane) = o;
            }
        });
        if constexpr (CSUM) {
            if (blockIdx.y == 0 && lane < EN_C)
                ws_csum[(int64_t)blockIdx.x * (n_groups * EN_C) + group * EN_C + lane] = (F)cs_lds[lane];
        }
    }
}

template <typename F>
__global__ void en_untile_kernel(const F *__restrict__ tmp, int64_t m, int64_t nB, F *__restrict__ out) {
    const int64_t e = (int64_t)blockIdx.x * blockDim.x + threadIdx.x;
    if (e >= m * nB) return;
    const int64_t i = e / nB, j = e % nB;
    out[e] = tmp[((j / EN_W) * m + i) * EN_W + (j % EN_W)];
}

template <typename F>
__global__ void en_csum_kernel(const F *__restrict__ part, int nblk, int64_t m, F *__restrict__ csum) {
    const int64_t c = (int64_t)blockIdx.x * blockDim.x + threadIdx.x;
    if (c >= m) return;
    double a = 0.0;
    for (int b = 0; b < nblk; ++b) a += (double)part[(int64_t)b * m + c];
    csum[c] = (F)a;
}

template <typename F>
static int run_csr_dense_ent(const F *vals, const uint16_t *meta, const uint32_t *bstart, int64_t n, int64_t m,
                             const F *B, int64_t r, const F *d, F *out, F *colsum, hipStream_t st) {
    const int64_t nB = r;
    const int64_t total = m * nB;
    if (total == 0) return TM_OK;
    constexpr int VEC = 16 / (int)sizeof(F);
    if ((reinterpret_cast<uintptr_t>(B) & 15) != 0 || r % VEC != 0 || nB < VEC) {
        set_error("tm_csr_dense_sandwich_ent: B must be C-ordered with 16-byte aligned rows");
        return TM_EUNSUPPORTED;
    }
    if (m % EN_C != 0) {
        set_error("tm_csr_dense_sandwich_ent: m must be a multiple of tm_ent_group_cols()");
        return TM_EINVAL;
    }
    if (n >= (1ll << 28)) {
        set_error("tm_csr_dense_sandwich_ent: at most 2^28 - 1 rows per block (work in row parts)");
        return TM_EUNSUPPORTED;
    }
    const int64_t n_slabs = ceil_div(n, EN_R);
    const int n_groups = (int)(m / EN_C);
    const int n_parts = (int)ceil_div(nB, EN_W);
    const int nz = (int)ceil_div(n_groups, EN_NW);
    const bool want_csum = colsum != nullptr;
    if (n_slabs == 0) {
        TM_HIP(hipMemsetAsync(out, 0, sizeof(F) * (size_t)total, st));
        if (want_csum) TM_HIP(hipMemsetAsync(colsum, 0, sizeof(F) * (size_t)m, st));
        return TM_OK;
    }
    int64_t nblk = std::max<int64_t>(1, tune("ent_rounds", 1) * NUM_CU / ((int64_t)n_parts * nz));
    nblk = std::min<int64_t>(nblk, n_slabs);
    const int64_t spb = ceil_div(n_slabs, nblk);
    nblk = ceil_div(n_slabs, spb);
    const int64_t stride = m * EN_W;
    const size_t tmp_bytes = (sizeof(F) * (size_t)(n_parts * stride) + 255) / 256 * 256;
    const size_t part_bytes = (sizeof(F) * (size_t)((int64_t)n_parts * nblk * stride) + 255) / 256 * 256;
    const size_t csum_bytes = ((want_csum ? sizeof(F) * (size_t)(nblk * m) : 0) + 255) / 256 * 256 + 256;
    void *wsv = nullptr;
    int rc = get_workspace(tmp_bytes + part_bytes + csum_bytes + 256, &wsv, st);
    if (rc) return rc;
    F *tmp = reinterpret_cast<F *>(wsv);
    F *ws = reinterpret_cast<F *>(reinterpret_cast<char *>(wsv) + tmp_bytes);
    F *ws_csum = reinterpret_cast<F *>(reinterpret_cast<char *>(wsv) + tmp_bytes + part_bytes);
    const size_t lds = (size_t)EnLds<F>::TOTAL;
    auto kern = want_csum ? &csr_dense_ent_kernel<F, true> : &csr_dense_ent_kernel<F, false>;
    TM_HIP(hipFuncSetAttribute(reinterpret_cast<const void *>(kern),
                               hipFuncAttributeMaxDynamicSharedMemorySize, (int)lds));
    prof_begin(st);
    hipLaunchKernelGGL(kern, dim3((unsigned)nblk, (unsigned)n_parts, (unsigned)nz), dim3(EN_THREADS), lds, st,
                       vals, meta, bstart, n_groups, n_slabs, spb, B, n, r, (int)nB, d, ws, ws_csum,
                       reinterpret_cast<long long *>((uintptr_t)tune("ent_prof", 0)));
    prof_end(st);
    TM_LAUNCH_CHECK();
    rc = launch_reduce_partials<F>(ws, stride, (int)nblk, n_parts, tmp, n_parts * stride, false, st);
    if (rc) return rc;
    hipLaunchKernelGGL((en_untile_kernel<F>), dim3((unsigned)ceil_div(total, 256)), dim3(256), 0, st, tmp, m,
                       nB, out);
    TM_LAUNCH_CHECK();
    if (want_csum) {
        hipLaunchKernelGGL((en_csum_kernel<F>), dim3((unsigned)ceil_div(m, 256)), dim3(256), 0, st, ws_csum,
                           (int)nblk, m, colsum);
        TM_LAUNCH_CHECK();
    }
    return TM_OK;
}

}

extern "C" {
int tm_ent_rows(void) { return tmh::EN_R; }
int tm_ent_group_cols(void) { return tmh::EN_C; }
int tm_ent_batch_slots(void) { return tmh::EN_B; }

int tm_csr_dense_sandwich_ent_f32(const float *vals, const uint16_t *meta, const uint32_t *bstart, int64_t n,
                                  int64_t m, const float *B, int64_t r, const float *d, float *out,
                                  float *colsum, void *stream) {
    return tmh::run_csr_dense_ent<float>(vals, meta, bstart, n, m, B, r, d, out, colsum, tmh::as_stream(stream));
}
int tm_csr_dense_sandwich_ent_f64(const double *vals, const uint16_t *meta, const uint32_t *bstart, int64_t n,
                                  int64_t m, const double *B, int64_t r, const double *d, double *out,
                                  double *colsum, void *stream) {
    return tmh::run_csr_dense_ent<double>(vals, meta, bstart, n, m, B, r, d, out, colsum, tmh::as_stream(stream));
}
}
```

tabmat_amd/ext/sparse.py:

```python
from __future__ import annotations

import os


from .. import _device as D
from .._lib import call
from ._types import CsrDev, DenseDev, SlabCsc, SlabEll, SlabEnt, SlabLg


def _csr_args(A: CsrDev):
    return (D.p(A.data), D.p(A.indices), D.p(A.indptr), A.n, A.m)


def sparse_sandwich(A: CsrDev, d, rows, cols):
    m = A.m if cols is None else D.nlen(cols)
    out = D.zeros((m, m), A.dtype)
    if m == 0 or (rows is not None and D.nlen(rows) == 0):
        return out
    D.same_float("sparse_sandwich", A.data, d)
    call(f"tm_sparse_sandwich_{D.fsuf(A.data)}", *_csr_args(A), D.p(d), D.p(rows), D.nlen(rows),
         D.p(cols), D.nlen(cols), D.p(out), D.stream_ptr())
    return out


# ... 55 lines not shown

def csr_matvec_multi(X: CsrDev, V, rows, cols, transpose):
    K = int(V.shape[1])
    n_cols = X.m if cols is None else D.nlen(cols)
    n_rows = X.n if rows is None else D.nlen(rows)
    out = D.zeros((n_cols if transpose else n_rows, K), X.dtype)
    if K == 0 or n_rows == 0 or n_cols == 0:
        return out
    D.same_float("csr_matvec_multi", X.data, V)
    Vc = V.contiguous()
    fn = "tm_csr_rmatvec_multi_" if transpose else "tm_csr_matvec_multi_"
    call(fn + D.fsuf(X.data), *_csr_args(X), D.p(Vc), K, D.p(rows), D.nlen(rows), D.p(cols),
         D.nlen(cols), D.p(out), D.stream_ptr())
    return out


def csr_dense_sandwich_slab(A: SlabCsc, B: DenseDev, d):
    assert B.n == A.n
    out = D.zeros((A.m, B.m), A.vals.dtype)
    if A.m == 0 or B.m == 0 or A.n == 0:
        return out
    D.same_float("csr_dense_sandwich_slab", A.vals, B.buf, d)
    call(f"tm_csr_dense_sandwich_slab_{D.fsuf(A.vals)}", D.p(A.vals), D.p(A.koff), D.p(A.cnt),
         D.p(A.gptr), A.n, A.m, D.p(B.buf), B.m, B.order_f, D.p(d), D.p(out), D.stream_ptr())
    return out


def ell_supported(B: DenseDev) -> bool:
    vec = 16 // B.buf.element_size()
    return (not B.order_f) and B.m % vec == 0 and B.m >= vec and B.buf.data_ptr() % 16 == 0


def csr_dense_sandwich_ell(A: SlabEll, B: DenseDev, d):
    assert B.n == A.n and ell_supported(B)
    if A.m == 0 or B.m == 0 or A.n == 0:
        return D.zeros((A.m, B.m), A.vals.dtype)
    out = D.zeros((A.mk, B.m), A.vals.dtype)
    D.same_float("csr_dense_sandwich_ell", A.vals, B.buf, d)
    fn = "tm_csr_dense_sandwich_ellw_" if A.wide else "tm_csr_dense_sandwich_ell_"
    call(fn + D.fsuf(A.vals), D.p(A.vals), D.p(A.koff), D.p(A.gptr),
         A.n, A.mk, D.p(B.buf), B.m, D.p(d), D.p(out), D.stream_ptr())
    return out[A.inv]


def csr_dense_sandwich_lg(A: SlabLg, B: DenseDev, d, unc=None, want_colsum=False):
    assert B.n == A.n and ell_supported(B)
    dt = A.dtype
    if A.m == 0 or B.m == 0 or A.n == 0:
        z = D.zeros((A.m, B.m), dt)
        return (z, D.zeros((A.m,), dt)) if want_colsum else z
    out = D.out_buf((A.mk, B.m), dt)
    u = int(A.unc if unc is None else unc)
    cs = D.out_buf((A.mk,), dt) if want_colsum else None
    if A.cvals is not None:
        D.same_float("csr_dense_sandwich_lg", A.cvals, B.buf, d)
        call("tm_csr_dense_sandwich_lgc_" + D.fsuf(A.cvals), D.p(A.cvals), D.p(A.cmap), D.p(A.crec),
             D.p(A.xkoff), A.n, A.mk, D.p(B.buf), B.m, D.p(d), u, D.p(out), D.p(cs), D.stream_ptr())
    elif want_colsum:
        D.same_float("csr_dense_sandwich_lg", A.vals, B.buf, d)
        call("tm_csr_dense_sandwich_lg_xtd_" + D.fsuf(A.vals), D.p(A.vals), D.p(A.koff), D.p(A.xptr),
             D.p(A.xvals), D.p(A.xkoff), A.n, A.mk, D.p(B.buf), B.m, D.p(d), u, D.p(out), D.p(cs),
             D.stream_ptr())
    else:
        D.same_float("csr_dense_sandwich_lg", A.vals, B.buf, d)
        call("tm_csr_dense_sandwich_lg_" + D.fsuf(A.vals), D.p(A.vals), D.p(A.koff), D.p(A.xptr),
             D.p(A.xvals), D.p(A.xkoff), A.n, A.mk, D.p(B.buf), B.m, D.p(d), u, D.p(out), D.stream_ptr())
    return (out[A.inv], cs[A.inv]) if want_colsum else out[A.inv]


def csr_dense_sandwich_ent(A: SlabEnt, B: DenseDev, d, want_colsum=False):
    assert B.n == A.n and ell_supported(B)
    dt = A.dtype
    if A.m == 0 or B.m == 0 or A.n == 0:
        z = D.zeros((A.m, B.m), dt)
        return (z, D.zeros((A.m,), dt)) if want_colsum else z
    out = D.out_buf((A.mk, B.m), dt)
    cs = D.out_buf((A.mk,), dt) if want_colsum else None
    D.same_float("csr_dense_sandwich_ent", A.vals, B.buf, d)
    call("tm_csr_dense_sandwich_ent_" + D.fsuf(A.vals), D.p(A.vals), D.p(A.meta), D.p(A.bstart), A.n, A.mk,
         D.p(B.buf), B.m, D.p(d), D.p(out), D.p(cs), D.stream_ptr())
    return (out[A.inv], cs[A.inv]) if want_colsum else out[A.inv]


def _row_table(A: CsrDev, rows, d, as_set: bool):
    import weakref

    import torch

    cm_data, cm_c8, cptr = A.chunk_major()
    cached = getattr(A, "_row_table", None)
    stamp = (rows.data_ptr(), rows._version, int(rows.numel()))
    if cached is not None and cached[0]() is rows and cached[4] == stamp:
        _, r64, dup, tabs, _ = cached
    else:
        r64 = torch.sort(rows.to(torch.int64)).values
        dup = bool((r64[1:] == r64[:-1]).any().item()) if r64.numel() > 1 else False
        tabs = {}
        A._row_table = (weakref.ref(rows), r64, dup, tabs, stamp)
    key = bool(as_set and dup)
    if key not in tabs:
        rr = torch.unique_consecutive(r64) if key else r64
        tabs[key] = (rr, torch.stack([cptr[:, rr], cptr[:, rr + 1]], dim=2).contiguous())
    rr, ranges = tabs[key]
    return cm_data, cm_c8, ranges, rr.to(torch.int32).contiguous(), d[rr].contiguous()


def sparse_sandwich_rows(A: CsrDev, d, rows):
    out = D.zeros((A.m, A.m), A.dtype)
    if A.m == 0 or D.nlen(rows) == 0 or A.data.numel() == 0:
        return out
    D.same_float("sparse_sandwich_rows", A.data, d)
    cm_data, cm_c8, ranges, r32, d_sel = _row_table(A, rows, d, True)
    cols = cm_c8 if K2B_U8 else A.chunk_cols32()
    call(f"tm_sparse_sandwich_chunked_rows_{'u8_' if K2B_U8 else ''}{D.fsuf(A.data)}", D.p(cm_data),
         D.p(cols), D.p(ranges),
         int(r32.numel()), A.m, int(cm_data.numel()), D.p(d_sel), D.p(out), D.stream_ptr())
    return out


def csr_dense_sandwich_rows(A: CsrDev, B: DenseDev, d, rows):
    out = D.zeros((A.m, B.m), A.dtype)
    if A.m == 0 or B.m == 0 or D.nlen(rows) == 0 or A.data.numel() == 0:
        return out
    D.same_float("csr_dense_sandwich_rows", A.data, B.buf, d)
    cm_data, cm_c8, ranges, r32, d_sel = _row_table(A, rows, d, False)
    call(f"tm_csr_dense_sandwich_rows_u8_{D.fsuf(A.data)}", D.p(cm_data), D.p(cm_c8), D.p(ranges),
         int(r32.numel()), D.p(r32), D.p(d_sel), A.n, A.m, D.p(B.buf), B.m, B.order_f, D.p(out),
         D.stream_ptr())
    return out


def sparse_sandwich_chunked(A: CsrDev, d):
    if A.m == 0 or A.n == 0:
        return D.zeros((A.m, A.m), A.dtype)
    out = D.out_buf((A.m, A.m), A.dtype)
    D.same_float("sparse_sandwich_chunked", A.data, d)
    cm_data, cm_c8, cptr = A.chunk_major()
    cols = cm_c8 if K2B_U8 else A.chunk_cols32()
    call(f"tm_sparse_sandwich_chunked_{'u8_' if K2B_U8 else ''}{D.fsuf(A.data)}", D.p(cm_data),
         D.p(cols), D.p(cptr),
         A.n, A.m, int(cm_data.numel()), D.p(d), D.p(out), D.stream_ptr())
    return out


K2_BLOCKS = True


def blocks_sandwich_pays(A: CsrDev) -> bool:
    import torch

    if not K2_BLOCKS or A.n == 0 or A.m == 0 or A.n >= 2**29:
        return False
    nnz = int(A.data.numel())
    nch = -(-A.m // 128)
    if not (0 < nnz < 2**31) or nnz / (A.n * nch) <= 4.5 or nch > 32:
        return False
    est = 16 * 2 * A.n * nch * (nch + 1) // 2
    return est * 3 < torch.cuda.mem_get_info(A.data.device)[0] or bool(getattr(A, "_pb", None))


K2B_U8 = os.environ.get("TABMAT_AMD_K2B_U8", "1") == "1"


def sparse_sandwich_blocks(A: CsrDev, d):
    if A.m == 0 or A.n == 0:
        return D.zeros((A.m, A.m), A.dtype)
    out = D.out_buf((A.m, A.m), A.dtype)
    D.same_float("sparse_sandwich_blocks", A.data, d)
    cm_data, cm_c8, cptr = A.chunk_major()
    blocks, wg_tab, max_nb = A.pair_blocks(d12=None if K2B_U8 else False)
    if int(blocks.shape[1]) == 3:
        call(f"tm_sparse_sandwich_blocks_p12_{D.fsuf(A.data)}", D.p(cm_data), D.p(cm_c8), D.p(cptr), A.n, A.m,
             int(cm_data.numel()), D.p(blocks), D.p(wg_tab), int(wg_tab.shape[0]), int(max_nb), D.p(d),
             D.p(out), D.stream_ptr())
        return out
    if K2B_U8:
        call(f"tm_sparse_sandwich_blocks_u8_{D.fsuf(A.data)}", D.p(cm_data), D.p(cm_c8), D.p(cptr), A.n, A.m,
             int(cm_data.numel()), D.p(blocks), D.p(wg_tab), int(wg_tab.shape[0]), int(max_nb), D.p(d),
             D.p(out), D.stream_ptr())
        return out
    cm_ind = A.chunk_cols32()
    call(f"tm_sparse_sandwich_blocks_{D.fsuf(A.data)}", D.p(cm_data), D.p(cm_ind), D.p(cptr), A.n, A.m,
         int(cm_data.numel()), D.p(blocks), D.p(wg_tab), int(wg_tab.shape[0]), int(max_nb), D.p(d),
         D.p(out), D.stream_ptr())
    return out


def sparse_sandwich_pairs(A: CsrDev, d):
    if A.m == 0 or A.n == 0:
        return D.zeros((A.m, A.m), A.dtype)
    out = D.out_buf((A.m, A.m), A.dtype)
    D.same_float("sparse_sandwich_pairs", A.data, d)
    _, _, cptr = A.chunk_major()
    if K2_PAIRS_PACKED and A.n < 2**25:
        rec = A.chunk_records_packed()
        call(f"tm_sparse_sandwich_pairs_pk_{D.fsuf(A.data)}", D.p(rec), D.p(cptr), A.n, A.m, int(A.data.numel()), D.p(d),
             D.p(out), D.stream_ptr())
        return out
    rec = A.chunk_records()
    call(f"tm_sparse_sandwich_pairs_{D.fsuf(A.data)}", D.p(rec), D.p(cptr), A.n, A.m, int(rec.shape[0]), D.p(d),
         D.p(out), D.stream_ptr())
    return out


def csc_dense_sandwich_sorted(A: CsrDev, B: DenseDev, d):
    if A.m == 0 or B.m == 0:
        return D.zeros((A.m, B.m), A.dtype)
    rows, vals, bstart, n_blocks, col_bptr = A.csc_blocks()
    out = D.out_buf((A.m, B.m), A.dtype)
    D.same_float("csc_dense_sandwich_sorted", vals, B.buf, d)
    call(f"tm_csc_dense_sandwich_sorted_{D.fsuf(vals)}", D.p(rows), D.p(vals), D.p(bstart),
         int(n_blocks), D.p(col_bptr), A.m, D.p(d), D.p(B.buf), B.m, D.p(out), D.stream_ptr())
    return out


def sparse_sandwich_direct(A: CsrDev, d):
    if A.m == 0 or A.n == 0:
        return D.zeros((A.m, A.m), A.dtype)
    out = D.out_buf((A.m, A.m), A.dtype)
    D.same_float("sparse_sandwich_direct", A.data, d)
    call(f"tm_sparse_sandwich_direct_{D.fsuf(A.data)}", D.p(A.data), D.p(A.indices), D.p(A.indptr),
         A.n, A.m, D.p(d), D.p(out), D.stream_ptr())
    return out


def direct_sandwich_pays(A: CsrDev) -> bool:
    nnz, n, m = int(A.data.numel()), A.n, A.m
    if n == 0 or nnz == 0 or m <= 1024:
        return False
    nch = (m + 127) // 128
    per_row = nnz / n
    pairs = n * per_row * (per_row + 1.0) / 2.0 * 1.3
    if nch > 32:
        return pairs / 15e9 < n * (nch * (nch + 1) / 2) * 0.3e-9
    if per_row / nch > 0.6:
        return False
    return pairs / 15e9 < n * (nch * (nch + 1) / 2) * 15e-12


K2_PAIRS = "auto"
K2_PAIRS_PACKED = os.environ.get("TABMAT_AMD_K2_PAIRS_PACKED", "1") == "1"
K2_PAIRS_MAX_M = 16384
K2_PAIRS_MAX_NNZ = 2**31 - 4 * 16 * 64


def pairs_sandwich_pays(A: CsrDev) -> bool:
    if K2_PAIRS != "auto":
        return K2_PAIRS == "1" and A.m <= K2_PAIRS_MAX_M and 0 < int(A.data.numel()) < K2_PAIRS_MAX_NNZ
    nnz, n, m = int(A.data.numel()), A.n, A.m
    if n == 0 or nnz == 0 or m <= 512 or m > K2_PAIRS_MAX_M or nnz >= K2_PAIRS_MAX_NNZ:
        return False
    nch = (m + 127) // 128
    parts = nch * (nch + 1) / 2
    per_row = nnz / n
    k = per_row / nch
    pairs = n * per_row * (per_row + 2.0) / 2.0
    pk = 0.75 if (K2_PAIRS_PACKED and n < 2**25) else 1.0
    t_pairs = (nnz * (nch + 1) / 2.0 * 2.3e-12 * pk * min(6.0, max(1.0, (1.6 / k) ** 0.8)) + pairs * 2.7e-12 * pk
               + min(parts, 768) * 0.8e-6 + max(0.0, parts - 768) * 0.1e-6)
    t_direct = pairs / 21e9
    if nch > 32:
        t_tiled = n * parts * 0.3e-9
    else:
        t_tiled = pairs * 1.15e-12 if k > 4.5 else n * parts * 17e-12 + pairs * 0.8e-12
    return t_pairs < 0.9 * min(t_direct, t_tiled)


def transpose_square_dot_weights(A: CsrDev, weights):
# ... 51 lines not shown
```

tabmat_amd/ext/split.py:

```python
from __future__ import annotations

import ctypes as C

import numpy as np

from .. import _device as D
from .._lib import call
from ._types import CsrDev, DenseDev, SlabCsc


def sandwich_cat_dense(i_indices, i_ncol, d, mat_j: DenseDev, rows, j_cols, drop_first=False):
    n_j = mat_j.m if j_cols is None else D.nlen(j_cols)
    res = D.zeros((i_ncol, n_j), mat_j.dtype)
    n_rows = i_indices.numel() if rows is None else D.nlen(rows)
    if d.numel() == 0 or n_rows == 0 or n_j == 0 or i_ncol == 0:
        return res
    D.same_float("sandwich_cat_dense", mat_j.buf, d)
    call(f"tm_cat_dense_sandwich_{D.fsuf(mat_j.buf)}", D.p(i_indices), i_indices.numel(), i_ncol,
         int(drop_first), D.p(d), D.p(rows), D.nlen(rows), D.p(mat_j.buf), mat_j.m, mat_j.order_f,
         D.p(j_cols), D.nlen(j_cols), D.p(res), D.stream_ptr())
    return res


def sandwich_cat_cat(i_indices, j_indices, i_ncol, j_ncol, d, rows, i_drop_first=False,
                     j_drop_first=False, hot=None):
    if i_ncol == 0 or j_ncol == 0 or (rows is not None and D.nlen(rows) == 0):
        return D.zeros((i_ncol, j_ncol), d.dtype)
    res = D.out_buf((i_ncol, j_ncol), d.dtype)
    fn = "tm_cat_cat_sandwich_atomic_" if (hot is not None and hot <= 4096) else "tm_cat_cat_sandwich_"
    call(fn + D.fsuf(d), D.p(i_indices), D.p(j_indices), i_indices.numel(),
         D.p(d), D.p(rows), D.nlen(rows), i_ncol, j_ncol, int(i_drop_first), int(j_drop_first),
         D.p(res), D.stream_ptr())
    return res


CAT_CAT_SORTED_MIN_ROWS = 500_000


def cat_cat_sorted_pays(n, i_ncol, j_ncol, itemsize=8) -> bool:
    if not (n >= CAT_CAT_SORTED_MIN_ROWS and 0 < j_ncol * 8 <= 128 * 1024 and i_ncol * j_ncol < 2**31 - 1):
        return False
    ti = (128 * 1024) // (8 * j_ncol)
    return -(-i_ncol // ti) >= 8


def sandwich_cat_cat_sorted(twin, i_ncol, j_ncol, d):
    ci_s, cj_s, perm, lptr = twin
    res = D.out_buf((i_ncol, j_ncol), d.dtype)
    call("tm_cat_cat_sandwich_sorted_" + D.fsuf(d), D.p(ci_s), D.p(cj_s), D.p(perm), D.p(lptr), int(perm.numel()),
         D.p(d), i_ncol, j_ncol, D.p(res), D.stream_ptr())
    return res


def sandwich_cat_sparse(i_indices, i_ncol, d, S: CsrDev, rows, cols, drop_first=False):
    n_cols = S.m if cols is None else D.nlen(cols)
    res = D.zeros((i_ncol, n_cols), S.dtype)
    if i_ncol == 0 or n_cols == 0 or (rows is not None and D.nlen(rows) == 0):
        return res
    D.same_float("sandwich_cat_sparse", S.data, d)
    call(f"tm_cat_sparse_sandwich_{D.fsuf(S.data)}", D.p(i_indices), i_indices.numel(), i_ncol,
         int(drop_first), D.p(S.data), D.p(S.indices), D.p(S.indptr), S.m, D.p(d), D.p(rows),
         D.nlen(rows), D.p(cols), D.nlen(cols), D.p(res), D.stream_ptr())
    return res


def cat_dense_sandwich_sorted(plan, n_cols, d, mat_j: DenseDev):
    perm, bstart, n_blocks, cat_bptr = plan
    if n_cols == 0 or mat_j.m == 0:
        return D.zeros((n_cols, mat_j.m), mat_j.dtype)
    res = D.out_buf((n_cols, mat_j.m), mat_j.dtype)
    D.same_float("cat_dense_sandwich_sorted", mat_j.buf, d)
    call(f"tm_cat_dense_sandwich_sorted_{D.fsuf(mat_j.buf)}", D.p(perm), D.p(bstart), int(n_blocks),
         D.p(cat_bptr), int(n_cols), D.p(d), D.p(mat_j.buf), mat_j.m, D.p(res), D.stream_ptr())
    return res


def cat_dense_sorted_ok(mat_j: DenseDev) -> bool:
    vec = 16 // mat_j.buf.element_size()
    return (not mat_j.order_f and mat_j.m >= vec and mat_j.m % vec == 0
            and mat_j.buf.data_ptr() % 16 == 0)


def cat_sparse_sandwich_sorted(plan, n_cols, d, S: CsrDev):
    perm, bstart, n_blocks, cat_bptr = plan
    if n_cols == 0 or S.m == 0:
        return D.zeros((n_cols, S.m), S.dtype)
    res = D.out_buf((n_cols, S.m), S.dtype)
    D.same_float("cat_sparse_sandwich_sorted", S.data, d)
    call(f"tm_cat_sparse_sandwich_sorted_{D.fsuf(S.data)}", D.p(perm), D.p(bstart), int(n_blocks),
         D.p(cat_bptr), int(n_cols), D.p(d), D.p(S.data), D.p(S.indices), D.p(S.indptr), S.m, D.p(res),
         D.stream_ptr())
    return res


class CatPairsPlan:

    N_WG = 512

    def __init__(self, cats, pos_arrays, diag_only=False):
        from .._lib import lib
        import torch

        self.cat_ids = [c[0] for c in cats]
        k = len(cats)
        cap = int(lib().tm_multi_cat_pairs_max_bins())
        slots = int(lib().tm_multi_cat_pairs_max_slots())
        roww = int(lib().tm_multi_cat_pairs_row_words())
        L = [int(c[1]) for c in cats]
        bundles = []
        lone = []

        def tot(g):
            return sum(L[a] for a in g)

        def halves(g):
            h = len(g) // 2
            return g[:h], g[h:]

        def cross(A, B):
            if tot(A) * tot(B) <= cap and len(A) <= slots and len(B) <= slots:
                bundles.append((A, B, 0))
            elif len(A) == 1 and len(B) == 1:
                return
            elif len(B) == 1 or (len(A) > 1 and (tot(A) >= tot(B) or len(A) > slots)
                                 and not len(B) > slots):
                a1, a2 = halves(A)
                cross(a1, B)
                cross(a2, B)
            else:
                b1, b2 = halves(B)
                cross(A, b1)
                cross(A, b2)

        def tri(G):
            if tot(G) ** 2 <= cap and len(G) <= slots:
                bundles.append((G, G, 1))
            elif len(G) == 1:
                lone.append(G[0])
            else:
                g1, g2 = halves(G)
                tri(g1)
                tri(g2)
                cross(g1, g2)

        live = [a for a in range(k) if L[a] > 0]
        if diag_only:
            lone = list(live)
        elif live:
            tri(live)
        cur = []
        for a in lone:
            if L[a] > cap:
                continue
            if cur and (tot(cur) + L[a] > cap or len(cur) >= slots):
                bundles.append((cur, cur, 2))
                cur = []
            cur.append(a)
        if cur:
            bundles.append((cur, cur, 2))
        self.n_bundles = len(bundles)
        self.slots = max((max(len(A), len(B)) for A, B, _ in bundles), default=1)
        def cost(A, B, mode):
            nt = len(A) * len(B) if mode == 0 else (len(A) * (len(A) + 1) // 2 if mode == 1 else len(A))
            nl = len(A) + (len(B) if mode == 0 else 0)
            return nt + 0.5 * nl + 1.0

        costs = [cost(*bd) for bd in bundles]
        n_wg = max(self.N_WG, self.n_bundles)
        share = [max(1, int(n_wg * c / max(sum(costs), 1e-9))) for c in costs]
        rows_w = np.zeros((max(self.n_bundles, 1), roww), dtype=np.int32)
        pstart = self.pstart = np.concatenate([[0], np.cumsum(L)]).astype(np.int64)
        desc, self.pairs, wg_map = [], [], []
        self.bins = max((tot(A) * (tot(B) if mode != 2 else 1) for A, B, mode in bundles), default=1)
        for y, (A, B, mode) in enumerate(bundles):
            width = tot(B) if mode != 2 else 1
            r = rows_w[y]
            r[0], r[1], r[2], r[3] = len(A), len(B), mode, width
            r[4], r[5], r[6] = len(wg_map), share[y], tot(A) * width
            wg_map += [y] * share[y]
            ra = np.concatenate([[0], np.cumsum([L[a] for a in A])]).astype(np.int64)
            cb = np.concatenate([[0], np.cumsum([L[b] for b in B])]).astype(np.int64)
            for s, a in enumerate(A):
                r[8 + 2 * s], r[9 + 2 * s] = a, ra[s] * width
            for s, b in enumerate(B):
                r[8 + 2 * slots + 2 * s], r[9 + 2 * slots + 2 * s] = b, (cb[s] if mode != 2 else 0)
            base = y * self.bins
            for s, a in enumerate(A):
                for t, b in enumerate(B):
                    if (mode == 1 and t < s) or (mode == 2 and t != s):
                        continue
                    if a == b:
                        off = base + ra[s] * width + (cb[s] if mode == 1 else 0)
                        stride = width + 1 if mode == 1 else 1
                        desc.append([off, L[a], L[a], stride, pstart[a], pstart[a], 1, 0])
                    else:
                        i, j = (a, b)
                        off = base + ra[s] * width + cb[t]
                        stride = width
                        desc.append([off, L[i], L[j], stride, pstart[i], pstart[j], 0, 0])
                    self.pairs.append((self.cat_ids[a], self.cat_ids[b], int(off), L[a], L[b], int(stride)))
        self.n_wg = len(wg_map)
        self.n_pairs = len(desc)
        self.h_bundles = rows_w
        self.h_wg_map = np.asarray(wg_map if wg_map else [0], dtype=np.int32)
        self.h_desc = np.asarray(desc, dtype=np.int64).reshape(-1, 8)
        if pos_arrays is None:
            self.covered = {(min(i, j), max(i, j)) for i, j, *_ in self.pairs}
            return
        self.bundles = D.to_dev(rows_w.reshape(-1))
        self.wg_map = D.to_dev(self.h_wg_map)
        self.desc = D.to_dev(self.h_desc)
        self.pos = torch.cat([p.to(torch.int64) for p in pos_arrays]) if pos_arrays else \
            D.zeros((0,), torch.int64)
        self.covered = {(min(i, j), max(i, j)) for i, j, *_ in self.pairs}
        self._cat_tab = (None, None)

    def cat_tab(self, cats):
        key = tuple((c[0].data_ptr(), bool(c[2])) for c in cats)
        if self._cat_tab[0] != key:
            tab = np.asarray([[c[0].data_ptr(), int(bool(c[2])), int(self.pstart[a]), 0]
                              for a, c in enumerate(cats)], dtype=np.int64)
            self._cat_tab = (key, D.to_dev(tab.reshape(-1)))
        return self._cat_tab[1]


def multi_cat_pairs(plan: CatPairsPlan, cats, d, rows, out, vector=False, pos=None):
    import torch

    tables = D.out_buf((max(plan.n_bundles, 1) * plan.bins,), torch.float64)
    if plan.n_pairs == 0:
        return tables
    if rows is not None and rows.numel() == 0:
        return tables.zero_()
    nrows = int(cats[0][0].numel())
    call(f"tm_multi_cat_pairs_{D.fsuf(d)}", D.p(plan.cat_tab(cats)), nrows, D.p(d), D.p(rows),
         D.nlen(rows), D.p(plan.bundles), plan.n_bundles, D.p(plan.wg_map), plan.n_wg, plan.slots,
         plan.bins, D.p(plan.desc), plan.n_pairs, D.p(plan.pos if pos is None else pos), D.p(tables),
         D.p(out), 0 if (vector or out is None) else out.shape[0], D.stream_ptr())
    return tables


def multi_cat_matvec(plan: CatPairsPlan, cats, v, out):
    D.same_float("multi_cat_matvec", v, out)
    call(f"tm_multi_cat_matvec_{D.fsuf(v)}", D.p(plan.cat_tab(cats)), len(cats), D.p(plan.pos), D.p(v),
         int(cats[0][0].numel()), D.p(out), D.stream_ptr())
    return out


def scatter_block(src, ri, ci, out, mirror=False, diag=False):
    p = out.shape[0]
    if diag:
        nr, nc = src.numel(), 1
    else:
        nr, nc = src.shape
    if nr == 0 or nc == 0:
        return
    call(f"tm_scatter_block_{D.fsuf(src)}", D.p(src), nr, nc, D.p(ri), D.p(ci), D.p(out), p,
         int(mirror), int(diag), D.stream_ptr())


def _col_maps(self):
    maps = self.__dict__.get("_col_maps", False)
    if maps is False:
        maps = None
        inds = [np.asarray(i) for i in self.indices]
        p = int(sum(i.size for i in inds))
        if all(i.size < 2 or bool((i[1:] > i[:-1]).all()) for i in inds) and \
                all(i.size == 0 or (i.min() >= 0 and i.max() < p) for i in inds):
            block_of = np.full(p, -1, dtype=np.int64)
            local_of = np.zeros(p, dtype=np.int32)
            for j, i in enumerate(inds):
                block_of[i] = j
                local_of[i] = np.arange(i.size, dtype=np.int32)
            if p == 0 or block_of.min() >= 0:
                maps = (block_of, local_of)
        self.__dict__["_col_maps"] = maps
    return maps


def split_col_subsets(self, cols: np.ndarray):
    cols = np.asarray(cols, dtype=np.int32)
    n_blocks = len(self.indices)
    maps = _col_maps(self)
    if maps is not None and (cols.size < 2 or bool((cols[1:] > cols[:-1]).all())):
        block_of, local_of = maps
        b, loc = block_of[cols], local_of[cols]
        order = np.argsort(b, kind="stable").astype(np.int32)
        ends = np.cumsum(np.bincount(b, minlength=n_blocks))
        starts = np.concatenate([[0], ends[:-1]])
        return ([order[s:e] for s, e in zip(starts, ends)],
                [loc[order[s:e]] for s, e in zip(starts, ends)], len(cols))
    next_idx = [0] * n_blocks
    sub_idx = [[] for _ in range(n_blocks)]
    sub_cols = [[] for _ in range(n_blocks)]
    for i, c in enumerate(cols.tolist()):
        for j in range(n_blocks):
            ind = self.indices[j]
            k = next_idx[j]
            while k < len(ind) and ind[k] < c:
                k += 1
            next_idx[j] = k
            if k < len(ind) and ind[k] == c:
                sub_idx[j].append(i)
                sub_cols[j].append(k)
                next_idx[j] = k + 1
                break
    return (
        [np.array(s, dtype=np.int32) for s in sub_idx],
        [np.array(s, dtype=np.int32) for s in sub_cols],
        len(cols),
    )


def is_sorted(a) -> bool:
    a = np.asarray(a)
    return bool(np.all(a[1:] >= a[:-1]))


MAX_FUSED_CATS = 16


def _cat_args(cats):
    n = len(cats)
    codes = (C.c_void_p * n)(*[c[0].data_ptr() for c in cats])
    ncols = (C.c_int64 * n)(*[int(c[1]) for c in cats])
    drop = (C.c_int32 * n)(*[int(bool(c[2])) for c in cats])
    return codes, ncols, drop, n


def multi_cat_dense_wide_ok(cats, mat_j: DenseDev) -> bool:
    fb = mat_j.buf.element_size()
    vec = 2
    total = sum(int(c[1]) for c in cats)
    tile = (total * 16 * vec * 8 + 15) // 16 * 16
    lds = tile + 16 * 32 * (fb + 4 * len(cats))
    return (not mat_j.order_f and 1 <= len(cats) <= 8 and mat_j.m >= vec and mat_j.m % vec == 0
            and mat_j.buf.data_ptr() % 16 == 0 and lds <= 150 * 1024)


def multi_cat_dense_tile_ok(cats, mat_j: DenseDev) -> bool:
    total = sum(int(c[1]) for c in cats)
    m = mat_j.m
    if total == 0 or m == 0 or not 1 <= len(cats) <= 16:
        return False
    tj = 64
    while tj > 1 and 8 * total * tj > 128 * 1024:
        tj >>= 1
    while tj > 1 and tj // 2 >= m:
        tj >>= 1
    return 8 * total * tj <= 128 * 1024 and (m + tj - 1) // tj <= 2


def multi_cat_dense_sandwich(cats, d, mat_j: DenseDev, rows=None):
    total = sum(int(c[1]) for c in cats)
    if total == 0 or mat_j.m == 0 or mat_j.n == 0 or (rows is not None and D.nlen(rows) == 0):
        return D.zeros((total, mat_j.m), mat_j.dtype)
    res = D.out_buf((total, mat_j.m), mat_j.dtype)
    codes, ncols, drop, n = _cat_args(cats)
    if rows is not None:
        D.same_float("multi_cat_dense_sandwich", mat_j.buf, d)
        call(f"tm_multi_cat_dense_sandwich_rows_{D.fsuf(mat_j.buf)}", codes, ncols, drop, n, mat_j.n,
             D.p(d), D.p(mat_j.buf), mat_j.m, D.p(rows), D.nlen(rows), D.p(res), D.stream_ptr())
        return res
    D.same_float("multi_cat_dense_sandwich", mat_j.buf, d)
    call(f"tm_multi_cat_dense_sandwich_{D.fsuf(mat_j.buf)}", codes, ncols, drop, n, mat_j.n,
         D.p(d), D.p(mat_j.buf), mat_j.m, mat_j.order_f, D.p(res), D.stream_ptr())
    return res


def multi_cat_sparse_sandwich(cats, d, S: SlabCsc):
    total = sum(int(c[1]) for c in cats)
    if total == 0 or S.m == 0 or S.n == 0:
        return D.zeros((total, S.m), S.vals.dtype)
    res = D.out_buf((total, S.m), S.vals.dtype)
    codes, ncols, drop, n = _cat_args(cats)
    D.same_float("multi_cat_sparse_sandwich", S.vals, d)
    call(f"tm_multi_cat_sparse_sandwich_slab_{D.fsuf(S.vals)}", codes, ncols, drop, n, S.n, D.p(d),
         D.p(S.vals), D.p(S.koff), D.p(S.ecol), D.p(S.gptr), S.m, D.p(res), D.stream_ptr())
    return res


PACKED_CODES = True


def pack_codes(cats):
    import torch

    total = sum(int(c[1]) for c in cats)
    if not PACKED_CODES or len(cats) > 3 or total >= 1023 or len(cats) == 0:
        return None
    codes, ncols, drop, n = _cat_args(cats)
    nrow = int(cats[0][0].numel())
    out = torch.empty((nrow,), dtype=torch.int32, device=cats[0][0].device)
    call("tm_multi_cat_pack_codes", codes, ncols, drop, n, nrow, D.p(out), D.stream_ptr())
    return out


def multi_cat_sparse_sandwich_ent(cats, d, E, packed=None):
    total = sum(int(c[1]) for c in cats)
    if total == 0 or E.m == 0 or E.n == 0:
        return D.zeros((total, E.m), E.vals.dtype)
    res = D.out_buf((total, E.mk), E.vals.dtype)
    codes, ncols, drop, n = _cat_args(cats)
    D.same_float("multi_cat_sparse_sandwich_ent", E.vals, d)
    if packed is not None:
        call(f"tm_multi_cat_sparse_sandwich_entp_{D.fsuf(E.vals)}", codes, ncols, drop, n, E.n, D.p(d),
             D.p(E.vals), D.p(E.meta), D.p(E.bstart), E.n_slots(), E.mk, D.p(packed), D.p(res), D.stream_ptr())
        return res[:, E.inv]
    call(f"tm_multi_cat_sparse_sandwich_ent_{D.fsuf(E.vals)}", codes, ncols, drop, n, E.n, D.p(d),
         D.p(E.vals), D.p(E.meta), D.p(E.bstart), E.n_slots(), E.mk, D.p(res), D.stream_ptr())
    return res[:, E.inv]


def multi_cat_sparse_sandwich_rows(cats, d, A, rows):
    from . import sparse as xs

    total = sum(int(c[1]) for c in cats)
    if total == 0 or A.m == 0 or D.nlen(rows) == 0 or A.data.numel() == 0:
        return D.zeros((total, A.m), A.data.dtype)
    res = D.out_buf((total, A.m), A.data.dtype)
    codes, ncols, drop, n = _cat_args(cats)
    D.same_float("multi_cat_sparse_sandwich_rows", A.data, d)
    cm_data, cm_c8, ranges, r32, d_sel = xs._row_table(A, rows, d, False)
    call(f"tm_multi_cat_sparse_sandwich_rows_u8_{D.fsuf(A.data)}", codes, ncols, drop, n, D.p(cm_data),
         D.p(cm_c8), D.p(ranges), D.p(r32), int(r32.numel()), A.m, D.p(d_sel), D.p(res), D.stream_ptr())
    return res
```

tabmat_amd/sparse_matrix.py:

```python
from __future__ import annotations

import os

import numpy as np
import torch
from scipy import sparse as sps

from . import _device as D
from .ext import sparse as xs
from .ext._types import CsrDev, SlabCsc, SlabEll, SlabEnt, SlabLg
from .matrix_base import MatrixBase
from .util import (
    check_indexer,
    check_matvec_dimensions,
    check_matvec_out_shape,
    check_sandwich_compatible,
    check_transpose_matvec_out_shape,
    normalize_index,
    device_row_index,
    selects_all_columns,
)


ELL_MAX_PAD = 8.0
# ... 141 lines not shown
    @property
    def indices(self):
        return self._host().indices

    @property
    def indptr(self):
        return self._host().indptr

    @property
    def data(self):
        return self._host().data

    __array_ufunc__ = None

    def tocsc(self, copy=False):
        return self._host().tocsc(copy=copy)

    def unpack(self):
        return self._host()

    def toarray(self):
        return self._host().toarray()

    def dot(self, other):
        return self._host().dot(other)

    def transpose(self):
        return type(self)(self._host().T)

    T = property(transpose)

    def getcol(self, i):
        return type(self)(self._host()[:, [i]], column_names=[self._colnames[i]],
                          term_names=[self._terms[i]])

    def astype(self, dtype, order="K", casting="unsafe", copy=True):
        return type(self)(self._host().astype(dtype, casting, copy))

    def __getitem__(self, key):
        row, col = check_indexer(key)
        if self._devblk is not None and selects_all_columns(col, self.shape[1]):
            sub = type(self).from_device(self._devblk.take_rows(*device_row_index(row, self.shape[0])))
            sub._colnames, sub._terms = list(self._colnames), list(self._terms)
            return sub
        names = np.array(self._colnames, dtype=object)[col].ravel().tolist()
        terms = np.array(self._terms, dtype=object)[col].ravel().tolist()
        return type(self)(self._host()[row, col], column_names=names, term_names=terms)

    def __matmul__(self, other):
        return self.matvec(other)

    def multiply(self, other):
        if other.ndim == 1:
            return type(self)(self._host().multiply(other[:, np.newaxis]))
        return type(self)(self._host().multiply(other))

    def _row_parts(self):
        parts = self.__dict__.get("_parts_cache", False)
        if parts is False:
            parts = None
            ptr = self._dev().indptr
            nnz = int(self._dev().data.numel())
            if nnz >= PART_NNZ:
                n = self.shape[0]
                k = -(-nnz // max(1, int(0.8 * PART_NNZ)))
                targets = torch.arange(1, k, device=ptr.device, dtype=torch.int64) * nnz // k
                cuts = sorted(set([0] + torch.searchsorted(ptr, targets).clamp_(0, n).tolist() + [n]))
                parts = [(a, b, self[a:b]) for a, b in zip(cuts[:-1], cuts[1:]) if b > a]
            self.__dict__["_parts_cache"] = parts
        return parts

    def _narrow_pays(self, w: int) -> bool:
        n, mcols = self.shape
        nnz = float(self._dev().data.numel())
        per_row = nnz / max(n, 1)
        pairs = n * per_row * (per_row + 1) / 2
        nch = -(-mcols // 128)
        t_full = max(31e-12 * (nch * (nch + 1) / 2) * n, 1.6e-12 * pairs)
        if getattr(self, "_direct_pays", None):
            t_full = pairs / 22e9
        t_narrow = 0.2e-3 + n * w * 4.5e-12 + nnz * w / max(mcols, 1) * 40e-12
        return t_narrow < 0.8 * t_full

    def _sandwich_dev(self, d, rows, cols):
        parts = self._row_parts()
        if parts is not None:
            out = None
            for a, b, part in parts:
                r = None
                if rows is not None:
                    r64 = rows.to(torch.int64)
                    sel = r64[(r64 >= a) & (r64 < b)]
                    if sel.numel() == 0:
                        continue
                    r = (sel - a).to(torch.int32)
                res = part._sandwich_dev(d[a:b], r, cols)
                out = res if out is None else out + res
            if out is None:
                k = self.shape[1] if cols is None else D.nlen(cols)
                out = D.zeros((k, k), d.dtype)
            return out
        A = self._dev()
        from . import categorical_matrix as _cm

        if _cm.DETERMINISTIC and A.data.numel() > 0 and self.shape[0] > 0:
            res = self._sandwich_deterministic(d, rows, cols)
            if res is not None:
                return res
            import warnings

            warnings.warn("TABMAT_AMD_DETERMINISTIC=1: this sparse block has no entry twin, its self sandwich "
                          "falls back to the LDS-atomic kernels and is NOT bit-reproducible from run to run",
                          RuntimeWarning, stacklevel=3)
        if getattr(self, "_direct_pays", None) is None:
            self._direct_pays = xs.direct_sandwich_pays(A)
        w = D.nlen(cols) if cols is not None else 0
        if (0 < w <= NARROW_COLS and 2 * w < self.shape[1] and self.shape[0] > 0 and A.data.numel() > 0
                and self._narrow_pays(w)
                and self.shape[0] * w * A.data.element_size() * 4 < torch.cuda.mem_get_info()[0]):
            from .ext import dense as xd
            from .ext._types import DenseDev

            rws, vls, bstart, _, col_bptr = A.csc_blocks()
            mx = getattr(self, "_max_col_len", None)
            if mx is None:
                ends = bstart[col_bptr]
                mx = self._max_col_len = int((ends[1:] - ends[:-1]).max().item())
            cd = cols.to(torch.int64)
            seg = torch.stack([bstart[col_bptr[cd]], bstart[col_bptr[cd + 1]]], dim=1).contiguous()
            T = torch.zeros((self.shape[0], w), dtype=A.data.dtype, device=A.data.device)
            xs.csc_densify_cols(rws, vls, seg, torch.arange(w, dtype=torch.int32, device=A.data.device),
                                mx, T)
            return xd.dense_sandwich(DenseDev(T, self.shape[0], w, 0), d, rows, None)
        pp = getattr(self, "_pairs_pay", None)
        if pp is None:
            pp = self._pairs_pay = xs.pairs_sandwich_pays(A)
        if pp and (rows is None or D.nlen(rows) > 0.3 * self.shape[0]):
            d = D.masked_d(d, rows, as_set=True)
            res = xs.sparse_sandwich_pairs(A, d)
            if cols is not None:
                c64 = cols.to(torch.int64)
                res = res[c64][:, c64].contiguous()
            return res
        pays = getattr(self, "_direct_pays", None)
        if pays is None:
            pays = self._direct_pays = xs.direct_sandwich_pays(A)
        if pays:
            d = D.masked_d(d, rows, as_set=True)
            res = xs.sparse_sandwich_direct(A, d)
            if cols is not None:
                c64 = cols.to(torch.int64)
                res = res[c64][:, c64].contiguous()
            return res
        if A.data.numel() > 0 and A.data.numel() < 2**31 and self.shape[1] <= 128 * 32:
            if rows is not None and 0 < D.nlen(rows) <= ROW_LIST_FRACTION * self.shape[0]:
                res = xs.sparse_sandwich_rows(A, d, rows)
                if cols is not None:
                    c64 = cols.to(torch.int64)
                    res = res[c64][:, c64].contiguous()
                return res
            d = D.masked_d(d, rows, as_set=True)
            bl = getattr(self, "_blocks_pay", None)
            if bl is None:
                bl = self._blocks_pay = xs.blocks_sandwich_pays(A)
            res = xs.sparse_sandwich_blocks(A, d) if bl else xs.sparse_sandwich_chunked(A, d)
            if cols is not None:
                c64 = cols.to(torch.int64)
                res = res[c64][:, c64].contiguous()
            return res
        return xs.sparse_sandwich(A, d, rows, cols)

    def _ent_det(self):
        ent = self._ent()
        if ent is None:
            hit = getattr(self, "_entblk_det", None)
            if hit is None:
                twin = SlabEnt.from_csr(self._dev(), max_pad=None)
                hit = self._entblk_det = twin if twin is not None else False
            ent = hit or None
        return ent

    def _sandwich_deterministic(self, d, rows, cols=None):
        from .ext._types import DenseDev

        ent = self._ent_det()
        if ent is None:
            return None
        n, m = self.shape
        A = self._dev()
        d = D.masked_d(d, rows, as_set=True)
        inv = None
        if cols is None:
            sel = torch.arange(m, dtype=torch.int64, device=d.device)
        else:
            sel, inv = torch.unique(cols.to(torch.int64), return_inverse=True)
            if int(sel.numel()) == int(inv.numel()) and bool((sel == cols.to(torch.int64)).all()):
                inv = None
        k = int(sel.numel())
        out = torch.empty((m, k), dtype=d.dtype, device=d.device)
        W = 128
        for c0 in range(0, k, W):
            w = min(W, k - c0)
            w_pad = (w + 3) // 4 * 4
            colmap = torch.full((m,), -1, dtype=torch.int32, device=d.device)
            colmap[sel[c0:c0 + w]] = torch.arange(w, dtype=torch.int32, device=d.device)
            T = torch.zeros((n, w_pad), dtype=A.data.dtype, device=d.device)
            xs.csr_densify_cols(A, colmap, T)
            res = xs.csr_dense_sandwich_ent(ent, DenseDev(T, n, w_pad, 0), d)
            out[:, c0:c0 + w] = res[:, :w]
            del T
        out = out if cols is None else out[sel]
        low = torch.tril(out)
        full = low + torch.tril(out, -1).T
        if inv is not None:
            full = full.index_select(0, inv).index_select(1, inv)
        return full

    def _sdiag_dev(self, d, rows, want_s1=False):
        parts = self._row_parts()
        if parts is not None:
            s1 = D.zeros((self.shape[1],), d.dtype) if want_s1 else None
            s2 = D.zeros((self.shape[1],), d.dtype)
            for a, b, part in parts:
                r = None
                if rows is not None:
                    r64 = rows.to(torch.int64)
                    sel = r64[(r64 >= a) & (r64 < b)]
                    if sel.numel() == 0:
                        continue
                    r = (sel - a).to(torch.int32)
                p1, p2 = part._sdiag_dev(d[a:b], r, want_s1)
                s2 += p2
                if want_s1:
                    s1 += p1
            return s1, s2
        A = self._dev()
        if rows is not None and A.data.numel() > 0 and not self._values_finite():
            r64 = rows.to(torch.int64)
            return xs.csr_sandwich_diag(A.take_rows("index", r64), d[r64].contiguous(), want_s1)
        return xs.csr_sandwich_diag(A, D.masked_d(d, rows).contiguous(), want_s1)

    def sandwich_diag(self, d, rows=None, cols=None):
        from .matrix_base import _sd_args

        a = _sd_args(self, d, rows, cols)
        if a.trivial is not None:
            return a.finish(a.trivial)
        tdt = D.torch_dtype(self.dtype)
        _, g = self._sdiag_dev(D.to_dev(a.d, tdt), D.idx_dev(a.rows))
        if a.cols is not None:
            g = g[D.idx_dev(a.cols, torch.int64)]
        return a.finish(g)

    def sandwich(self, d, rows=None, cols=None):
        on_dev = D.is_dev(d)
        if not on_dev:
            d = np.asarray(d)
        check_sandwich_compatible(self, d)
        res = self._sandwich_dev(D.to_dev(d), D.idx_dev(normalize_index(rows, self.shape[0])),
                                 D.idx_dev(normalize_index(cols, self.shape[1])))
        return res if on_dev else D.to_host(res)

    def _cross_sandwich_dev(self, other, d, rows, L_cols, R_cols, colsum_box=None):
        from .categorical_matrix import CategoricalMatrix
        from .dense_matrix import DenseMatrix

        if isinstance(other, DenseMatrix):
            if other.dtype != self.dtype:
                raise TypeError(
                    "self, B and d all need to be of same dtype, either np.float64 or "
                    f"np.float32. This matrix is of type {self.dtype}, B is of type "
                    f"{other.dtype}.")
            Bd = other._dev_c()
            A = self._dev()
            if (rows is not None and 0 < D.nlen(rows) <= ROW_LIST_FRACTION_K3 * self.shape[0]
                    and 0 < A.data.numel() < 2**31 and self.shape[1] <= 128 * 32):
                res = xs.csr_dense_sandwich_rows(A, Bd, d, rows)
                if L_cols is not None:
                    res = res[L_cols.to(torch.int64)]
                if R_cols is not None:
                    res = res[:, R_cols.to(torch.int64)]
                return res
            if self.shape[0] > 0 and self._dev().data.numel() > 0 and (
                    rows is None or self._values_finite()):
                d = D.masked_d(d, rows)
                if (A.data.numel() <= SORTED_K3_NNZ_PER_ROW * self.shape[0] and self.shape[1] >= 1024
                        and xs.ell_supported(Bd)):
                    res = xs.csc_dense_sandwich_sorted(A, Bd, d)
                    if L_cols is not None:
                        res = res[L_cols.to(torch.int64)]
                    if R_cols is not None:
                        res = res[:, R_cols.to(torch.int64)]
                    return res
                wide = Bd.m > 64 and xs.ell_supported(Bd)
                ent = self._ent() if wide else None
                lg = self._lg() if (wide and ent is None) else None
                ell = None
                if ent is None and lg is None and xs.ell_supported(Bd):
                    ell = self._ell(wide=Bd.m > 64)
                if ent is not None and colsum_box is not None:
                    res, cs = xs.csr_dense_sandwich_ent(ent, Bd, d, want_colsum=True)
                    colsum_box.append(cs if L_cols is None else cs[L_cols.to(torch.int64)])
                elif ent is not None:
                    res = xs.csr_dense_sandwich_ent(ent, Bd, d)
                elif lg is not None and colsum_box is not None:
                    res, cs = xs.csr_dense_sandwich_lg(lg, Bd, d, want_colsum=True)
                    colsum_box.append(cs if L_cols is None else cs[L_cols.to(torch.int64)])
                elif lg is not None:
                    res = xs.csr_dense_sandwich_lg(lg, Bd, d)
                elif ell is not None:
                    res = xs.csr_dense_sandwich_ell(ell, Bd, d)
                else:
                    res = xs.csr_dense_sandwich_slab(self._slab(), Bd, d)
                if L_cols is not None:
                    res = res[L_cols.to(torch.int64)]
                if R_cols is not None:
                    res = res[:, R_cols.to(torch.int64)]
                return res
            return xs.csr_dense_sandwich(self._dev(), Bd, d, rows, L_cols, R_cols)
        if isinstance(other, CategoricalMatrix):
            return other._cross_sandwich_dev(self, d, rows, R_cols, L_cols).T
        raise TypeError

    def _cross_sandwich(self, other, d, rows, L_cols=None, R_cols=None):
        on_dev = D.is_dev(d)
        if not on_dev:
            d = np.asarray(d)
        check_sandwich_compatible(self, d)
        res = self._cross_sandwich_dev(
            other, D.to_dev(d), D.idx_dev(normalize_index(rows, self.shape[0])),
            D.idx_dev(normalize_index(L_cols, self.shape[1])),
            D.idx_dev(normalize_index(R_cols, other.shape[1])))
        return res if on_dev else D.to_host(res)

    def sandwich_dense(self, B, d, rows, L_cols, R_cols):
        from .dense_matrix import DenseMatrix

        Bm = B if isinstance(B, DenseMatrix) else DenseMatrix(B)
        return self._cross_sandwich(Bm, d, rows, L_cols, R_cols)

    def _matvec_dev(self, vec, rows, cols, out, transpose):
        fn = xs.csc_rmatvec if transpose else xs.csr_matvec
        return fn(self._dev(), vec, rows, cols, out)

    def _matvec_helper(self, vec, rows, cols, out, transpose):
        on_dev = D.is_dev(vec)
        if not on_dev:
            vec = np.asarray(vec)
        check_matvec_dimensions(self, vec, transpose)
        n, m = self.shape
        rows_n = normalize_index(rows, n)
        cols_n = normalize_index(cols, m)
        if rows_n is not None and len(rows_n) == n:
            rows_n = None
        if cols_n is not None and len(cols_n) == m:
            cols_n = None
        tdt = D.torch_dtype(self.dtype)
        v_dev = D.to_dev(vec, tdt)
        rd, cd = D.idx_dev(rows_n), D.idx_dev(cols_n)
        if v_dev.ndim == 1:
            res = self._matvec_dev(v_dev, rd, cd, None, transpose)
        else:
            res = xs.csr_matvec_multi(self._dev(), v_dev, rd, cd, transpose)
        if not on_dev:
            res = D.to_host(res)
        if out is None:
            return res
        if transpose and cols_n is not None:
            out[cols_n if not D.is_dev(out) else D.idx_dev(cols_n, torch.int64)] += res
        else:
            out += res
        return out

    def matvec(self, vec, cols=None, out=None):
        check_matvec_out_shape(self, out)
        return self._matvec_helper(vec, None, cols, out, False)

    def transpose_matvec(self, vec, rows=None, cols=None, out=None):
        check_transpose_matvec_out_shape(self, out)
        return self._matvec_helper(vec, rows, cols, out, True)

    def _get_col_stds(self, weights, col_means):
        tdt = D.torch_dtype(self.dtype)
        ex2 = D.to_host(xs.transpose_square_dot_weights(self._dev(),
                                                        D.to_dev(np.asarray(weights), tdt)))
# ... 4 lines not shown
```

tabmat_amd/split_matrix.py:

```python
from __future__ import annotations

import os
import warnings
from collections.abc import Sequence
from typing import Optional, Union

import numpy as np
import torch
from scipy import sparse as sps

from . import _device as D
from .categorical_matrix import CategoricalMatrix
from .dense_matrix import DenseMatrix, _centre_and_shift
from .ext import split as xsplit
from .ext.dense import dense_glm_loss_grad as xd_glm
from .ext.dense import dense_sandwich_matvec as xd_smv
from .matrix_base import MatrixBase
from .sparse_matrix import SparseMatrix
from .standardized_mat import StandardizedMatrix
from .util import (
    check_matvec_dimensions,
    check_matvec_out_shape,
    check_sandwich_compatible,
    check_transpose_matvec_out_shape,
    collapse_identity,
    normalize_index,
    set_up_rows_or_cols,
)


ROW_LIST_FRACTION_CATSPARSE = 0.04
DIAG_FROM_PAIRS = True
CAT_PAIRS_FUSED = os.environ.get("TABMAT_AMD_CAT_PAIRS", "1") != "0"
FULL_THEN_SELECT = float(os.environ.get("TABMAT_AMD_FULL_THEN_SELECT", "0.5"))
FULL_RESULT_MAX_BYTES = 256 << 20
FULL_UNSELECTED_SHARE = 0.2
FULL_THEN_SELECT_MV = 0.0
NARROW_COLS = int(os.environ.get("TABMAT_AMD_NARROW_COLS", "128"))
from . import categorical_matrix as _cm
from . import sparse_matrix as _spm


class _Centering:
    NARROW_GROUP = 1 << 20

    def __init__(self, vec):
        self.vec = dict(vec)
        self.cs_centered = set()
        self.groups = None

    def get(self, b):
        return self.vec.get(b)


class _Xtv:

    def __init__(self, v):
        self.v = v
        self.out = {}


def as_tabmat(a):
    if isinstance(a, (MatrixBase, StandardizedMatrix)):
        return a
    if sps.issparse(a):
        return SparseMatrix(a.tocsc(copy=False))
    if isinstance(a, np.ndarray):
        return DenseMatrix(a)
    raise ValueError(f"Cannot convert type {type(a)} to Matrix.")


def hstack(tup: Sequence) -> MatrixBase:
    mats = [as_tabmat(a) for a in tup]
    if not mats:
        raise ValueError("Need at least one array to concatenate.")
    if all(isinstance(m, SparseMatrix) for m in mats):
        return SparseMatrix(sps.hstack([m.array_csc for m in mats]))
    if all(isinstance(m, DenseMatrix) for m in mats):
        return DenseMatrix(np.hstack([m.toarray() for m in mats]))
    return SplitMatrix(mats)


def _merge_same_kind(matrices, indices):
    for kind in (DenseMatrix, SparseMatrix):
        which = [i for i, m in enumerate(matrices) if isinstance(m, kind)]
        if len(which) <= 1:
            continue
        gidx = np.concatenate([indices[i] for i in which])
        order = np.argsort(gidx)
        names = np.concatenate([np.array(matrices[i]._colnames, dtype=object) for i in which])
        terms = np.concatenate([np.array(matrices[i]._terms, dtype=object) for i in which])
        if kind is DenseMatrix:
            merged = DenseMatrix(np.hstack([matrices[i].toarray() for i in which])[:, order])
        else:
            merged = SparseMatrix(sps.hstack([matrices[i].array_csc for i in which]).tocsc()[:, order])
        merged._colnames = names[order].tolist()
        merged._terms = terms[order].tolist()
        matrices[which[0]] = merged
        indices[which[0]] = gidx[order]
        drop = set(which[1:])
        matrices = [m for i, m in enumerate(matrices) if i not in drop]
        indices = [x for i, x in enumerate(indices) if i not in drop]
    return matrices, indices


def _block_sdiag(mb, d, rows, center=None, want_s1=False):
    d = d.to(D.torch_dtype(mb.dtype))
    if isinstance(mb, DenseMatrix):
        return mb._sdiag_dev(d, rows, None if center is None else center.to(d.dtype).contiguous()), None
    if isinstance(mb, SparseMatrix):
        s1, s2 = mb._sdiag_dev(d, rows, want_s1)
        return s2, s1
    if isinstance(mb, CategoricalMatrix):
        h = mb._sandwich_diag_dev(d, rows, None)
        return h, (h if want_s1 else None)
    r = None if rows is None else D.to_host(rows)
# ... 178 lines not shown
        key = np.asarray(cols_host).tobytes()
        hit = self.__dict__.get("_plan_cache")
        if hit is not None and hit[0] == key:
            return hit[1]
        pos, sub_cols, n_cols = self._split_col_subsets(cols_host)
        pos_d = self._dev_idx(pos)
        sub_d = [None if sc is None else D.idx_dev(sc) for sc in sub_cols]
        self._cols_dev64(cols_host)
        if CAT_PAIRS_FUSED:
            plan = self._cat_pairs_plan()
            if plan is not None and plan.n_pairs > 0:
                self._pairs_pos_sel(plan, cols_host, (pos, sub_cols))
        self.__dict__["_plan_cache"] = (key, (pos_d, sub_d, n_cols))
        return pos_d, sub_d, n_cols

    def _blocks_finite(self) -> bool:
        return all(mb._values_finite() for mb in self.matrices
                   if isinstance(mb, (DenseMatrix, SparseMatrix)))

    def _cols_dev64(self, cols_host):
        key = np.asarray(cols_host).tobytes()
        hit = self.__dict__.get("_cols64")
        if hit is None or hit[0] != key:
            hit = self.__dict__["_cols64"] = (key, D.idx_dev(cols_host, torch.int64))
        return hit[1]

    def _pairs_pos_sel(self, plan, cols_host, split=None):
        key = np.asarray(cols_host).tobytes()
        hit = self.__dict__.get("_pos_sel")
        if hit is not None and hit[0] == key:
            return hit[1]
        pos_h, sub_h = split if split is not None else self._split_col_subsets(cols_host)[:2]
        pf = np.full(int(plan.pstart[-1]), -1, dtype=np.int64)
        for a, i in enumerate(plan.cat_ids):
            if len(sub_h[i]):
                pf[int(plan.pstart[a]) + np.asarray(sub_h[i], dtype=np.int64)] = pos_h[i]
        t = D.to_dev(pf)
        self.__dict__["_pos_sel"] = (key, t)
        return t

    def _sandwich_xtd_dev(self, d, rows, cols_host, center=None):
        colsum = [None] * len(self.matrices)
        out = self._sandwich_dev(d, rows, cols_host, colsum=colsum, center=center)
        pos_d, sub_d, n_cols = self._sandwich_plan(cols_host)
        xtd = D.zeros((n_cols,), torch.float64)
        cmask = None if center is None else torch.zeros((n_cols,), dtype=torch.bool, device=xtd.device)
        for i, (mi, pd, sd) in enumerate(zip(self.matrices, pos_d, sub_d)):
            if sd is not None and D.nlen(sd) == 0:
                continue
            cs = colsum[i]
            if cs is None:
                if isinstance(mi, CategoricalMatrix):
                    full = D.zeros((mi.shape[1],), d.dtype)
                    mi._transpose_matvec_dev(d, rows, sd, full)
                    cs = full if sd is None else full[sd.to(torch.int64)]
                else:
                    cs = mi._matvec_dev(d, rows, sd, None, True)
            elif center is not None and i in center.cs_centered:
                cmask[pd] = True
            xtd[pd] = cs.to(torch.float64)
        if center is not None:
            return out, xtd, cmask, center.groups
        return out, xtd

    FUSED_LEVELS = 496
    FUSED_CATS = 8

    def _cat_groups(self, cat_ids):
        groups, cur, tot = [], [], 0
        for i in cat_ids:
            k = self.matrices[i].shape[1]
            if k > self.FUSED_LEVELS:
                continue
            if cur and (len(cur) == self.FUSED_CATS or tot + k > self.FUSED_LEVELS):
                groups.append(cur)
                cur, tot = [], 0
            cur.append(i)
            tot += k
        if cur:
            groups.append(cur)
        return groups

    def _cat_pairs_plan(self):
        plan = self.__dict__.get("_cp_plan", False)
        if plan is False:
            plan = None
            ids = [i for i, m in enumerate(self.matrices)
                   if isinstance(m, CategoricalMatrix) and m.shape[1] > 0]
            if len(ids) >= 1:
                pos = self._full_dev_indices()
                plan = xsplit.CatPairsPlan([(i, self.matrices[i].shape[1]) for i in ids],
                                           [pos[i] for i in ids])
            self.__dict__["_cp_plan"] = plan
        return plan

    def _cat_hist_plan(self):
        plan = self.__dict__.get("_ch_plan", False)
        if plan is False:
            plan = None
            ids = [i for i, m in enumerate(self.matrices)
                   if isinstance(m, CategoricalMatrix) and m.shape[1] > 0 and m.shape[0] > 0]
            if len(ids) >= 2:
                pos = self._full_dev_indices()
                plan = xsplit.CatPairsPlan([(i, self.matrices[i].shape[1]) for i in ids],
                                           [pos[i] for i in ids], diag_only=True)
            self.__dict__["_ch_plan"] = plan
        return plan

    def _fused_cats(self, mw, cats, cat_ids, d_eff, rows, total, budget, d_rows=None):
        if isinstance(mw, DenseMatrix) and xsplit.multi_cat_dense_wide_ok(cats, mw._dev_c()):
            if rows is not None and D.nlen(rows) <= 0.5 * self.shape[0]:
                return xsplit.multi_cat_dense_sandwich(cats, d_rows, mw._dev_c(), rows)
            return xsplit.multi_cat_dense_sandwich(cats, d_eff, mw._dev_c())
        if isinstance(mw, DenseMatrix) and xsplit.multi_cat_dense_tile_ok(cats, mw._dev_c()):
            return xsplit.multi_cat_dense_sandwich(cats, d_eff, mw._dev_c())
        if isinstance(mw, DenseMatrix):
            if xsplit.cat_dense_sorted_ok(mw._dev_c()):
                return None
            from .ext import sparse as xs

            oh, inv = self._onehot_slab(cat_ids)
            return xs.csr_dense_sandwich_slab(oh, mw._dev_c(), d_eff)[inv]
        if (isinstance(mw, SparseMatrix) and total * 33 <= budget and rows is not None
                and 0 < D.nlen(rows) <= ROW_LIST_FRACTION_CATSPARSE * self.shape[0]
                and 0 < mw._dev().data.numel() < 2**31):
            return xsplit.multi_cat_sparse_sandwich_rows(cats, d_rows, mw._dev(), rows)
        if (isinstance(mw, SparseMatrix) and total * 33 <= budget
                and mw._dev().data.numel() > 0 and (rows is None or mw._values_finite())):
            ent = None
            if len(cats) <= 8 and (getattr(mw, "_entblk", None) or any(
                    isinstance(mo, DenseMatrix) and mo.shape[1] > 64 and mo.dtype == mw.dtype
                    for mo in self.matrices)):
                ent = mw._ent()
            if ent is not None:
                pk_cache = self.__dict__.setdefault("_packed_codes", {})
                key = tuple(cat_ids)
                if key not in pk_cache:
                    pk_cache[key] = xsplit.pack_codes(cats)
                return xsplit.multi_cat_sparse_sandwich_ent(cats, d_eff, ent, pk_cache[key])
            return xsplit.multi_cat_sparse_sandwich(cats, d_eff, mw._slab())
        return None

    def _parts(self):
        parts = self.__dict__.get("_row_parts", False)
        if parts is False:
            parts = None
            big = [m for m in self.matrices
                   if isinstance(m, SparseMatrix) and m._dev().data.numel() >= _spm.PART_NNZ]
            if big:
                n = self.shape[0]
                lead = max(big, key=lambda m: m._dev().data.numel())
                ptr = lead._dev().indptr
                nnz = int(ptr[-1].item())
                k = -(-nnz // max(1, int(0.8 * _spm.PART_NNZ)))
                while True:
                    targets = torch.arange(1, k, device=ptr.device, dtype=torch.int64) * nnz // k
                    cuts = [0] + torch.searchsorted(ptr, targets).clamp_(0, n).tolist() + [n]
                    cuts = sorted(set(int(c) for c in cuts))
                    ok = all(int((m._dev().indptr[cuts[1:]] - m._dev().indptr[cuts[:-1]]).max().item())
                             < _spm.PART_NNZ for m in big)
                    if ok or k >= n:
                        break
                    k += 1
                parts = [(a, b, self[a:b]) for a, b in zip(cuts[:-1], cuts[1:]) if b > a]
            self.__dict__["_row_parts"] = parts
        return parts

    def _sandwich_parts(self, parts, d, rows, cols_host, colsum, center=None):
        out = None
        for a, b, part in parts:
            r = None
            if rows is not None:
                r64 = rows.to(torch.int64)
                sel = r64[(r64 >= a) & (r64 < b)]
                if sel.numel() == 0:
                    continue
                r = (sel - a).to(torch.int32)
            cs = [None] * len(self.matrices) if colsum is not None else None
            sub_cen = None if center is None else _Centering(center.vec)
            res = part._sandwich_dev(d[a:b], r, cols_host, None, cs, center=sub_cen)
            if sub_cen is not None:
                center.groups = sub_cen.groups
            if sub_cen is not None and colsum is not None:
                dsum = (d[a:b] if r is None else d[a:b][r.to(torch.int64)]).sum(dtype=torch.float64)
                _, sub_p, _ = self._sandwich_plan(cols_host)
                for i in sub_cen.cs_centered:
                    if cs[i] is not None and sub_cen.get(i) is not None:
                        cv = sub_cen.get(i).to(torch.float64)
                        if sub_p[i] is not None:
                            cv = cv[sub_p[i].to(torch.int64)]
                        cs[i] = cs[i].to(torch.float64) + cv * dsum
            out = res if out is None else out + res
            if colsum is not None:
                for i, c in enumerate(cs):
                    if c is None:
                        colsum[i] = False
                    elif colsum[i] is not False:
                        colsum[i] = c if colsum[i] is None else colsum[i] + c
        if colsum is not None:
            for i, c in enumerate(colsum):
                if c is False:
                    colsum[i] = None
        if out is None:
            _, _, n_cols = self._sandwich_plan(cols_host)
            out = D.zeros((n_cols, n_cols), torch.float64)
        return out

    def _full_product_pays(self, sub_h) -> bool:
        p = self.shape[1]
        if p * p * 8 > FULL_RESULT_MAX_BYTES:
            return False
        n = max(self.shape[0], 1)
        tot = unsel = 0.0
        for b, mb in enumerate(self.matrices):
            if isinstance(mb, DenseMatrix):
                wb = float(mb.shape[1])
            elif isinstance(mb, SparseMatrix):
                nnz = mb._devblk.data.numel() if mb._devblk is not None else mb._host().nnz
                wb = max(1.0, float(nnz) / n)
            else:
                wb = 1.0 + mb.shape[1] / 256.0
            tot += wb
            if len(sub_h[b]) == 0:
                unsel += wb
        return unsel <= FULL_UNSELECTED_SHARE * tot

    def _full_product_pays_cols(self, cols_host) -> bool:
        key = np.asarray(cols_host).tobytes()
        hit = self.__dict__.get("_fpp_cache")
        if hit is None or hit[0] != key:
            hit = self.__dict__["_fpp_cache"] = (key, self._full_product_pays(self._split_col_subsets(cols_host)[1]))
        return hit[1]

    def _narrow_plan(self, cols_host):
        key = np.asarray(cols_host).tobytes()
        hit = self.__dict__.get("_narrow_cache")
        if hit is not None and hit[0] == key:
            return hit[1]
        nar = None
        pos_h, sub_h, n_cols = self._split_col_subsets(cols_host)
        mats = self.matrices
        noncat = [b for b, mb in enumerate(mats) if not isinstance(mb, CategoricalMatrix)]
        cat = [b for b, mb in enumerate(mats) if isinstance(mb, CategoricalMatrix) and len(sub_h[b]) > 0]
        w = sum(len(sub_h[b]) for b in noncat)
        itemsize = np.dtype(self.dtype).itemsize
        if (noncat and 0 < w <= NARROW_COLS and self.shape[0] > 0
                and all(isinstance(mats[b], (DenseMatrix, SparseMatrix)) and mats[b].dtype == self.dtype
# ... 42 lines not shown
        n = self.shape[0]
        T = torch.zeros((n, nar["w_pad"]), dtype=d.dtype, device=d.device)
        for b, t0, s, idx in nar["parts"]:
            mb = self.matrices[b]
            if isinstance(mb, SparseMatrix):
                xs.csc_densify_cols(*idx, T)
            else:
                xd.dense_gather_cols(mb._dev(), idx, T, t0)
        tmp = nar["tmp"]
        if tmp is None:
            tmp = nar["tmp"] = SplitMatrix([DenseMatrix(T)] + [self.matrices[i] for i in nar["cat"]],
                                           nar["indices"])
        dm = tmp.matrices[0]
        dm._devblk = DenseDev(T, n, nar["w_pad"], 0)
        sub_cen = None
        if center is not None:
            tc = torch.zeros((nar["w_pad"],), dtype=d.dtype, device=d.device)
            for b, t0, s, idx in nar["parts"]:
                if center.get(b) is not None:
                    tc[t0:t0 + s] = center.get(b)[idx.to(torch.int64)]
            sub_cen = _Centering({0: tc})
        try:
            cs_tmp = [None] * len(tmp.matrices) if colsum is not None else None
            full = tmp._sandwich_dev(d, rows, None, None, cs_tmp, center=sub_cen)
        finally:
            dm._devblk = None
        if colsum is not None:
            if cs_tmp[0] is not None:
                for b, t0, s, _ in nar["parts"]:
                    colsum[b] = cs_tmp[0][t0:t0 + s]
                    if sub_cen is not None and 0 in sub_cen.cs_centered:
                        center.cs_centered.add(b)
            for k, i in enumerate(nar["cat"]):
                if cs_tmp[1 + k] is not None and i in nar["cat_sub"]:
                    colsum[i] = cs_tmp[1 + k][nar["cat_sub"][i]]
        if center is not None:
            g = torch.full_like(nar["sel"], -1, dtype=torch.int32)
            g[nar["sel"] < nar["w_pad"]] = _Centering.NARROW_GROUP
            center.groups = g
        sel = nar["sel"]
        return full.index_select(0, sel).index_select(1, sel)

    def _sandwich_dev(self, d, rows, cols_host, plan=None, colsum=None, center=None, xtv=None):
        if cols_host is not None and len(cols_host) >= FULL_THEN_SELECT * self.shape[1] \
                and len(cols_host) > 0 and self._full_product_pays_cols(cols_host):
            pos_d, sub_d, n_cols = plan if plan is not None else self._sandwich_plan(cols_host)
            cs_full = [None] * len(self.matrices) if colsum is not None else None
            full = self._sandwich_dev(d, rows, None, None, cs_full, center=center, xtv=xtv)
            if colsum is not None:
                for i, c in enumerate(cs_full):
                    if c is not None:
                        colsum[i] = c if sub_d[i] is None else c[sub_d[i].to(torch.int64)]
            cd = self._cols_dev64(cols_host)
            return full.index_select(0, cd).index_select(1, cd)
        parts = self._parts()
        if parts is not None:
            return self._sandwich_parts(parts, d, rows, cols_host, colsum, center)
        if cols_host is not None and plan is None and NARROW_COLS > 0:
            nar = self._narrow_plan(cols_host)
            if nar == "wide":
                cs_full = [None] * len(self.matrices) if colsum is not None else None
                full = self._sandwich_dev(d, rows, None, None, cs_full, center=center, xtv=xtv)
                if colsum is not None:
                    _, sub_sel, _ = self._sandwich_plan(cols_host)
                    for i, c in enumerate(cs_full):
                        if c is not None:
                            colsum[i] = c if sub_sel[i] is None else c[sub_sel[i].to(torch.int64)]
                cd = self._cols_dev64(cols_host)
                return full.index_select(0, cd).index_select(1, cd)
            if nar is not None and d.dtype == D.torch_dtype(self.dtype):
                return self._sandwich_narrow(nar, d, rows, colsum, center)
        pos_d, sub_d, n_cols = plan if plan is not None else self._sandwich_plan(cols_host)
        out = D.zeros((n_cols, n_cols), torch.float64)
        mats = self.matrices
        empty = [sd is not None and D.nlen(sd) == 0 for sd in sub_d]
        done = set()
        return self._sandwich_terms(d, rows, cols_host, colsum, out, pos_d, sub_d, empty, done, center,
                                    xtv if cols_host is None else None)

    def _sandwich_terms(self, d, rows, cols_host, colsum, out, pos_d, sub_d, empty, done, center=None, xtv=None):
        from .ext import dense as xd

        mats = self.matrices
        cat_ids = [i for i, m in enumerate(mats) if isinstance(m, CategoricalMatrix) and not empty[i]
                   and m.shape[1] > 0]
        budget = (128 * 1024) // 8
        groups = self._cat_groups(cat_ids)
        if groups:
            d_eff = D.masked_d(d, rows)
        for grp in groups:
            cats = [(mats[i]._dev(), mats[i].shape[1], mats[i].drop_first) for i in grp]
            total = sum(c[1] for c in cats)
            offs = np.concatenate([[0], np.cumsum([c[1] for c in cats])])
            for w, mw in enumerate(mats):
                if empty[w] or mw.dtype != self.dtype or d.dtype != D.torch_dtype(self.dtype):
                    continue
                stacked = self._fused_cats(mw, cats, grp, d_eff, rows, total, budget, d)
                if stacked is None:
                    continue
                whole = cols_host is None and len(grp) > 1
                if whole:
                    cache = self.__dict__.setdefault("_group_pos", {})
                    gpos = cache.get(tuple(grp))
                    if gpos is None:
                        gpos = cache[tuple(grp)] = torch.cat([pos_d[i] for i in grp])
                    xsplit.scatter_block(stacked.contiguous(), gpos, pos_d[w], out, mirror=True)
                for ci, i in enumerate(grp):
                    res = stacked[int(offs[ci]):int(offs[ci + 1])]
                    if (colsum is not None and colsum[w] is None and not mats[i].drop_first
                            and not mats[i]._has_missings):
                        cs = res.sum(dim=0)
                        colsum[w] = cs if sub_d[w] is None else cs[sub_d[w].to(torch.int64)]
                    if not whole:
                        res = CategoricalMatrix._restrict(res, sub_d[i], sub_d[w])
                        xsplit.scatter_block(res.contiguous(), pos_d[i], pos_d[w], out, mirror=True)
                    done.add((min(i, w), max(i, w)))
        big = [i for i in cat_ids if mats[i].shape[1] > self.FUSED_LEVELS]
        if len(big) >= 2 and len(big) <= 16 and d.dtype == D.torch_dtype(self.dtype):
            cats = [(mats[i]._dev(), mats[i].shape[1], mats[i].drop_first) for i in big]
            offs = np.concatenate([[0], np.cumsum([c[1] for c in cats])])
            d_big = None
            for w, mw in enumerate(mats):
                if (empty[w] or not isinstance(mw, DenseMatrix) or mw.dtype != self.dtype
                        or not xsplit.multi_cat_dense_tile_ok(cats, mw._dev_c())):
                    continue
                if d_big is None:
                    d_big = D.masked_d(d, rows)
                stacked = xsplit.multi_cat_dense_sandwich(cats, d_big, mw._dev_c())
                for ci, i in enumerate(big):
                    res = stacked[int(offs[ci]):int(offs[ci + 1])]
                    if (colsum is not None and colsum[w] is None and not mats[i].drop_first
                            and not mats[i]._has_missings):
                        cs = res.sum(dim=0)
                        colsum[w] = cs if sub_d[w] is None else cs[sub_d[w].to(torch.int64)]
                    res = CategoricalMatrix._restrict(res, sub_d[i], sub_d[w])
                    xsplit.scatter_block(res.contiguous(), pos_d[i], pos_d[w], out, mirror=True)
                    done.add((min(i, w), max(i, w)))
        cat_diag = {}
        diag_scattered = set()
        det = _cm.DETERMINISTIC
        plan = self._cat_pairs_plan() if CAT_PAIRS_FUSED and not det else None
        if (plan is not None and plan.n_pairs > 0
                and d.dtype in (torch.float32, torch.float64)
                and d.dtype == D.torch_dtype(self.dtype)):
            cl = [(mats[i]._dev(), mats[i].shape[1], mats[i].drop_first) for i in plan.cat_ids]
            pos_sel = None if cols_host is None else self._pairs_pos_sel(plan, cols_host)
            tables = xsplit.multi_cat_pairs(plan, cl, d, rows, out, pos=pos_sel)
            for i, j, toff, li, lj, stride in plan.pairs:
                if i == j:
                    if not empty[i]:
                        full = tables[toff:toff + (li - 1) * stride + 1:stride]
                        if sub_d[i] is not None and colsum is not None:
                            full = full[sub_d[i].to(torch.int64)]
                        cat_diag[i] = full.to(d.dtype)
                        diag_scattered.add(i)
                else:
                    done.add((i, j))
        complete = [isinstance(m, CategoricalMatrix) and not m.drop_first and not m._has_missings
                    and sub_d[k] is None and not empty[k] for k, m in enumerate(mats)]
        for i, mi in enumerate(mats):
            if empty[i] or not isinstance(mi, CategoricalMatrix):
                continue
            for j in range(i + 1, len(mats)):
                if empty[j] or not isinstance(mats[j], CategoricalMatrix) or (i, j) in done:
                    continue
                res = mi._cross_sandwich_dev(mats[j], d, rows, sub_d[i], sub_d[j])
                xsplit.scatter_block(res.contiguous(), pos_d[i], pos_d[j], out, mirror=True)
                done.add((i, j))
                if DIAG_FROM_PAIRS and not det and complete[j] and i not in cat_diag:
                    cat_diag[i] = res.sum(dim=1)
                if DIAG_FROM_PAIRS and not det and complete[i] and j not in cat_diag:
                    cat_diag[j] = res.sum(dim=0)
        for i, mi in enumerate(mats):
            if empty[i]:
                continue
            if isinstance(mi, CategoricalMatrix):
                diag = cat_diag[i] if i in cat_diag else mi._sandwich_diag_dev(d, rows, sub_d[i])
                if colsum is not None:
                    colsum[i] = diag
                if i not in diag_scattered:
                    xsplit.scatter_block(diag, pos_d[i], pos_d[i], out, diag=True)
            elif (xtv is not None and colsum is None and center is None and isinstance(mi, DenseMatrix)
                  and sub_d[i] is None and (both := mi._sandwich_xtv_dev(d, xtv.v, rows)) is not None):
                res, xtv.out[i] = both
                xsplit.scatter_block(res, pos_d[i], pos_d[i], out)
            elif (colsum is not None and colsum[i] is None and isinstance(mi, DenseMatrix)
                  and rows is None and sub_d[i] is None
                  and (both := mi._sandwich_xtd_dev(d, cen_i := (center.get(i) if center else None))) is not None):
                res, colsum[i] = both
                if cen_i is not None:
                    center.cs_centered.add(i)
                xsplit.scatter_block(res, pos_d[i], pos_d[i], out)
            elif isinstance(mi, DenseMatrix) and center is not None and center.get(i) is not None:
                res = mi._sandwich_dev(d, rows, sub_d[i], center=center.get(i))
                xsplit.scatter_block(res, pos_d[i], pos_d[i], out)
            else:
                res = mi._sandwich_dev(d, rows, sub_d[i])
                xsplit.scatter_block(res, pos_d[i], pos_d[i], out)
        for i, mi in enumerate(mats):
            if empty[i]:
                continue
            for j in range(i + 1, len(mats)):
                if empty[j] or (i, j) in done:
                    continue
                si, di = (i, j) if isinstance(mi, SparseMatrix) else (j, i)
                if (colsum is not None and colsum[si] is None and isinstance(mats[si], SparseMatrix)
                        and isinstance(mats[di], DenseMatrix)):
                    box = []
                    res = mats[si]._cross_sandwich_dev(mats[di], d, rows, sub_d[si], sub_d[di],
                                                       colsum_box=box)
                    if box:
                        colsum[si] = box[0]
                    if si != i:
                        res = res.T
                else:
                    res = mi._cross_sandwich_dev(mats[j], d, rows, sub_d[i], sub_d[j])
                xsplit.scatter_block(res.contiguous(), pos_d[i], pos_d[j], out, mirror=True)
        return out

    def sandwich_graph(self, d, rows=None, cols=None):
        from .graph import CapturedProduct

        check_sandwich_compatible(self, d)
        rows_d = D.idx_dev(normalize_index(rows, self.shape[0]))
        cols_n = collapse_identity(normalize_index(cols, self.shape[1]), self.shape[1])
        plan = self._sandwich_plan(cols_n)
        return CapturedProduct(lambda dd: self._sandwich_dev(dd, rows_d, cols_n, plan), d)

    def sandwich(self, d, rows=None, cols=None):
        on_dev = D.is_dev(d)
        if not on_dev:
            d = np.asarray(d)
        check_sandwich_compatible(self, d)
        rows_n = normalize_index(rows, self.shape[0])
        cols_n = collapse_identity(normalize_index(cols, self.shape[1]), self.shape[1])
        out = self._sandwich_dev(D.to_dev(d), D.idx_dev(rows_n), cols_n)
        return out if on_dev else D.to_host(out)

    def sandwich_and_transpose_matvec(self, d, v, rows=None, cols=None):
        from .matrix_base import _check_1d

        _check_1d(v)
        d_dev_side, v_dev_side = D.is_dev(d), D.is_dev(v)
        if not d_dev_side:
            d = np.asarray(d)
        if not v_dev_side:
            v = np.asarray(v)
        check_sandwich_compatible(self, d)
        check_matvec_dimensions(self, v, transpose=True)
        rows_n = normalize_index(rows, self.shape[0])
        cols_n = collapse_identity(normalize_index(cols, self.shape[1]), self.shape[1])
        tdt = D.torch_dtype(self.dtype)
        v_dev = D.to_dev(v, tdt)
        acc = None
        if (tdt == torch.float64 and not _cm.DETERMINISTIC
                and (rows_n is None or len(rows_n) < self.shape[0])):
            acc = _Xtv(v_dev)
        H = self._sandwich_dev(D.to_dev(d), D.idx_dev(rows_n), cols_n, xtv=acc)
        g, _ = self._transpose_matvec_dev(v_dev, rows_n, cols_n, done=None if acc is None else acc.out)
        if not v_dev_side:
            g = D.to_host(g)
            if np.issubdtype(v.dtype, np.floating):
                g = g.astype(np.result_type(self.dtype, v.dtype), copy=False)
        return (H if d_dev_side else D.to_host(H)), g

    def sandwich_matvec(self, d, u, rows=None, cols=None):
        from .matrix_base import _smv_args, _smv_compose

        a = _smv_args(self, d, u, rows, cols, h_dtype=np.float64)
        if a.trivial is not None:
            return a.finish(a.trivial)
        tdt = D.torch_dtype(self.dtype)
        res = None
        if (rows is None and cols is None) or self._blocks_finite():
            res = self._smv_dev(a.d_masked(tdt), a.u_full(tdt))
        if res is None:
            return a.finish(_smv_compose(self, a))
        g = res[0]
        if a.cols is not None:
            g = g[self._cols_dev64(a.cols)]
        return a.finish(g)

    def _sdiag_dev(self, d, rows, cols_host=None, centers=None, want_s1=False):
        p = self.shape[1]
        parts = self._parts()
        if parts is not None:
            s2 = D.zeros((p,), torch.float64)
            s1 = D.zeros((p,), torch.float64) if want_s1 else None
            for a, b, part in parts:
                r = None
                if rows is not None:
                    r64 = rows.to(torch.int64)
                    sel = r64[(r64 >= a) & (r64 < b)]
                    if sel.numel() == 0:
                        continue
# ... 241 lines not shown
```

Before: 1046 GB/s.

## Fuse partial reduction with scatter into output for split sandwich blocks

Adds 'into' variants of the multi-cat dense/sparse, CSR-dense and sparse-block sandwich kernels. A new finish kernel reduces the per-block partials and writes each result symmetrically into the final p×p output through row and column index maps. This replaces the separate reduce, untile and scatter_block passes along with their temporary buffers. It also changes the cat-pairs plan to split pairs, using per-bundle range bounds on the first slot, and adds env flags to turn both behaviours off. The cost is more code paths to keep correct, plus potential duplicate writes on mirrored entries.

Result: no change. 1046 GB/s (-0.0%).

```diff
diff --git a/include/tabmat_hip.h b/include/tabmat_hip.h
--- a/include/tabmat_hip.h
+++ b/include/tabmat_hip.h
@@ -514,6 +514,47 @@
                            const int64_t *desc, int64_t n_pairs, const int64_t *pos, double *tables,
                            double *out, int64_t p, void *stream);
 
+int tm_csr_dense_sandwich_ent_into_f32(const float *vals, const uint16_t *meta, const uint32_t *bstart, int64_t n,
+                                       int64_t m, const float *B, int64_t r, const float *d, double *res,
+                                       int64_t p, const int64_t *ri, const int64_t *ci, void *stream);
+int tm_csr_dense_sandwich_ent_into_f64(const double *vals, const uint16_t *meta, const uint32_t *bstart, int64_t n,
+                                       int64_t m, const double *B, int64_t r, const double *d, double *res,
+                                       int64_t p, const int64_t *ri, const int64_t *ci, void *stream);
+int tm_sparse_sandwich_blocks_u8_into_f32(const float *cm_data, const uint8_t *cm_col8, const int32_t *cptr,
+                                          int64_t n, int64_t m, int64_t nnz, const int32_t *blocks,
+                                          const int32_t *wg_tab, int n_wg, int max_nb, const float *d, double *res,
+                                          int64_t p, const int64_t *pos, void *stream);
+int tm_sparse_sandwich_blocks_u8_into_f64(const double *cm_data, const uint8_t *cm_col8, const int32_t *cptr,
+                                          int64_t n, int64_t m, int64_t nnz, const int32_t *blocks,
+                                          const int32_t *wg_tab, int n_wg, int max_nb, const double *d, double *res,
+                                          int64_t p, const int64_t *pos, void *stream);
+int tm_sparse_sandwich_blocks_p12_into_f32(const float *cm_data, const uint8_t *cm_col8, const int32_t *cptr,
+                                           int64_t n, int64_t m, int64_t nnz, const int32_t *blocks12,
+                                           const int32_t *wg_tab, int n_wg, int max_nb, const float *d, double *res,
+                                           int64_t p, const int64_t *pos, void *stream);
+int tm_sparse_sandwich_blocks_p12_into_f64(const double *cm_data, const uint8_t *cm_col8, const int32_t *cptr,
+                                           int64_t n, int64_t m, int64_t nnz, const int32_t *blocks12,
+                                           const int32_t *wg_tab, int n_wg, int max_nb, const double *d, double *res,
+                                           int64_t p, const int64_t *pos, void *stream);
+int tm_multi_cat_dense_sandwich_into_f32(const void *const *h_codes, const int64_t *h_ncols,
+                                         const int32_t *h_drop_first, int n_cats, int64_t n, const float *d,
+                                         const float *M, int64_t M_ncol, int order_f, double *res, int64_t p,
+                                         const int64_t *ri, const int64_t *ci, void *stream);
+int tm_multi_cat_dense_sandwich_into_f64(const void *const *h_codes, const int64_t *h_ncols,
+                                         const int32_t *h_drop_first, int n_cats, int64_t n, const double *d,
+                                         const double *M, int64_t M_ncol, int order_f, double *res, int64_t p,
+                                         const int64_t *ri, const int64_t *ci, void *stream);
+int tm_multi_cat_sparse_sandwich_ent_into_f32(const void *const *h_codes, const int64_t *h_ncols,
+                                              const int32_t *h_drop_first, int n_cats, int64_t n, const float *d,
+                                              const float *vals, const uint16_t *meta, const uint32_t *bstart,
+                                              int64_t n_slots, int64_t mk, const uint32_t *packed, double *res,
+                                              int64_t p, const int64_t *ri, const int64_t *ci, void *stream);
+int tm_multi_cat_sparse_sandwich_ent_into_f64(const void *const *h_codes, const int64_t *h_ncols,
+                                              const int32_t *h_drop_first, int n_cats, int64_t n, const double *d,
+                                              const double *vals, const uint16_t *meta, const uint32_t *bstart,
+                                              int64_t n_slots, int64_t mk, const uint32_t *packed, double *res,
+                                              int64_t p, const int64_t *ri, const int64_t *ci, void *stream);
+
 int tm_multi_cat_matvec_f32(const int64_t *cat_tab, int n_cats, const int64_t *pos, const float *v,
                             int64_t n, float *out, void *stream);
 int tm_multi_cat_matvec_f64(const int64_t *cat_tab, int n_cats, const int64_t *pos, const double *v,
diff --git a/tabmat_amd/csrc/cat.hip b/tabmat_amd/csrc/cat.hip
--- a/tabmat_amd/csrc/cat.hip
+++ b/tabmat_amd/csrc/cat.hip
@@ -2,6 +2,7 @@
 
 #include "common.hpp"
 #include "reduce.hpp"
+#include "finish.hpp"
 
 namespace tmh {
 
@@ -1305,7 +1306,8 @@
 static int run_multi_cat_dense(const void *const *h_codes, const int64_t *h_ncols,
                                const int32_t *h_drop, int n_cats, int64_t n, const F *d, const F *M,
                                int64_t m, int order_f, F *out, hipStream_t st,
-                               const int32_t *rows = nullptr, int64_t n_rows = 0) {
+                               const int32_t *rows = nullptr, int64_t n_rows = 0,
+                               const FinishInto *fin = nullptr) {
     CatSet cs;
     int rc = make_catset(h_codes, h_ncols, h_drop, n_cats, &cs);
     if (rc) return rc;
@@ -1313,6 +1315,7 @@
     if (total == 0) return TM_OK;
     if (rows != nullptr) n = n_rows;
     if (n == 0) {
+        if (fin) return launch_finish_zero(cs.total, m, *fin, st);
         TM_HIP(hipMemsetAsync(out, 0, sizeof(F) * (size_t)total, st));
         return TM_OK;
     }
@@ -1357,6 +1360,8 @@
             else if (n_cats == 7) rc = gow(&multi_cat_dense_wide_kernel<F, 7>);
             else rc = gow(&multi_cat_dense_wide_kernel<F, 8>);
             if (rc) return rc;
+            if (fin)
+                return launch_finish_partials<F>(ws, stride, (int)nblk, (int)n_parts, PanelMap{TJW, m}, *fin, st);
             rc = launch_reduce_partials<F>(ws, stride, (int)nblk, (int)n_parts, tmp, n_parts * stride,
                                            false, st);
             if (rc) return rc;
@@ -1423,6 +1428,7 @@
     }
 #undef TM_MCD_CASE
     if (rc) return rc;
+    if (fin) return launch_finish_partials<F>(ws, stride, (int)nblk, (int)n_parts, PanelMap{TJ, m}, *fin, st);
     rc = launch_reduce_partials<F>(ws, stride, (int)nblk, (int)n_parts, tmp, n_parts * stride, false,
                                    st);
     if (rc) return rc;
@@ -1535,13 +1541,15 @@
 static int run_multi_cat_sparse_ent(const void *const *h_codes, const int64_t *h_ncols, const int32_t *h_drop,
                                     int n_cats, int64_t n, const F *d, const F *vals, const unsigned short *meta,
                                     const unsigned *bstart, int64_t mk, F *out, hipStream_t st,
-                                    const unsigned *packed = nullptr, int64_t n_slots = 0) {
+                                    const unsigned *packed = nullptr, int64_t n_slots = 0,
+                                    const FinishInto *fin = nullptr) {
     CatSet cs;
     int rc = make_catset(h_codes, h_ncols, h_drop, n_cats, &cs);
     if (rc) return rc;
     const int64_t total = (int64_t)cs.total * mk;
     if (total == 0) return TM_OK;
     if (n == 0) {
+        if (fin) return launch_finish_zero(cs.total, mk, *fin, st);
         TM_HIP(hipMemsetAsync(out, 0, sizeof(F) * (size_t)total, st));
         return TM_OK;
     }
@@ -1617,6 +1625,7 @@
         prof_end(st);
         TM_LAUNCH_CHECK();
     }
+    if (fin) return launch_finish_partials<F>(ws, stride, (int)nblk, n_pairs, PanelMap{GC, mk}, *fin, st);
     rc = launch_reduce_partials<F>(ws, stride, (int)nblk, n_pairs, tmp, (int64_t)n_pairs * stride, false, st);
     if (rc) return rc;
     hipLaunchKernelGGL((multi_cat_untile_kernel<F>), dim3((unsigned)ceil_div(total, 256)), dim3(256), 0, st, tmp,
@@ -1813,6 +1822,31 @@
     return run_multi_cat_sparse_ent<double>(h_codes, h_ncols, h_drop_first, n_cats, n, d, vals, meta, bstart, mk,
                                             out, as_stream(stream), nullptr, n_slots);
 }
+#define TM_MULTI_CAT_INTO(SUF, F)                                                                                    \
+    int tm_multi_cat_dense_sandwich_into_##SUF(const void *const *h_codes, const int64_t *h_ncols,                   \
+                                               const int32_t *h_drop_first, int n_cats, int64_t n, const F *d,       \
+                                               const F *M, int64_t M_ncol, int order_f, double *res, int64_t p,      \
+                                               const int64_t *ri, const int64_t *ci, void *stream) {                 \
+        const FinishInto fin{res, p, ri, ci};                                                                        \
+        if (int rc = check_finish(fin, "tm_multi_cat_dense_sandwich_into")) return rc;                               \
+        return run_multi_cat_dense<F>(h_codes, h_ncols, h_drop_first, n_cats, n, d, M, M_ncol, order_f, nullptr,     \
+                                      as_stream(stream), nullptr, 0, &fin);                                          \
+    }                                                                                                                \
+    int tm_multi_cat_sparse_sandwich_ent_into_##SUF(const void *const *h_codes, const int64_t *h_ncols,              \
+                                                    const int32_t *h_drop_first, int n_cats, int64_t n, const F *d,  \
+                                                    const F *vals, const uint16_t *meta, const uint32_t *bstart,     \
+                                                    int64_t n_slots, int64_t mk, const uint32_t *packed,             \
+                                                    double *res, int64_t p, const int64_t *ri, const int64_t *ci,    \
+                                                    void *stream) {                                                  \
+        const FinishInto fin{res, p, ri, ci};                                                                        \
+        if (int rc = check_finish(fin, "tm_multi_cat_sparse_sandwich_ent_into")) return rc;                          \
+        return run_multi_cat_sparse_ent<F>(h_codes, h_ncols, h_drop_first, n_cats, n, d, vals, meta, bstart, mk,     \
+                                           nullptr, as_stream(stream), packed, n_slots, &fin);                       \
+    }
+TM_MULTI_CAT_INTO(f32, float)
+TM_MULTI_CAT_INTO(f64, double)
+#undef TM_MULTI_CAT_INTO
+
 int tm_multi_cat_pack_codes(const void *const *h_codes, const int64_t *h_ncols, const int32_t *h_drop_first, int n_cats,
                             int64_t n, uint32_t *packed, void *stream) {
     CatSet cs;
diff --git a/tabmat_amd/csrc/cat_pairs.hip b/tabmat_amd/csrc/cat_pairs.hip
--- a/tabmat_amd/csrc/cat_pairs.hip
+++ b/tabmat_amd/csrc/cat_pairs.hip
@@ -5,7 +5,8 @@
 
 constexpr int CP_BINS = 16384;
 constexpr int CP_SLOTS = 16;
-constexpr int CP_ROW = 8 + 4 * CP_SLOTS;
+constexpr int CP_RNG = 8 + 4 * CP_SLOTS;
+constexpr int CP_ROW = CP_RNG + 4;
 constexpr int CP_NEG = -(1 << 28);
 
 template <typename F, int NS>
@@ -28,6 +29,8 @@
     __syncthreads();
     const int32_t *pa[NS], *pb[NS];
     int dropa[NS], dropb[NS], offa[NS], offb[NS];
+    const unsigned cnta0 = (unsigned)__builtin_amdgcn_readfirstlane(br[CP_RNG + 1]);
+    const unsigned cntb0 = (unsigned)__builtin_amdgcn_readfirstlane(br[CP_RNG + 3]);
     static_for<NS>([&](auto sc) {
         constexpr int s = decltype(sc)::value;
         pa[s] = pb[s] = nullptr;
@@ -36,13 +39,13 @@
             const int id = __builtin_amdgcn_readfirstlane(br[8 + 2 * s]);
             offa[s] = __builtin_amdgcn_readfirstlane(br[9 + 2 * s]);
             pa[s] = reinterpret_cast<const int32_t *>(cat_tab[4 * id]);
-            dropa[s] = (int)cat_tab[4 * id + 1];
+            dropa[s] = (int)cat_tab[4 * id + 1] + (s == 0 ? __builtin_amdgcn_readfirstlane(br[CP_RNG]) : 0);
         }
         if (s < nb) {
             const int id = __builtin_amdgcn_readfirstlane(br[8 + 2 * CP_SLOTS + 2 * s]);
             offb[s] = __builtin_amdgcn_readfirstlane(br[9 + 2 * CP_SLOTS + 2 * s]);
             pb[s] = reinterpret_cast<const int32_t *>(cat_tab[4 * id]);
-            dropb[s] = (int)cat_tab[4 * id + 1];
+            dropb[s] = (int)cat_tab[4 * id + 1] + (s == 0 ? __builtin_amdgcn_readfirstlane(br[CP_RNG + 2]) : 0);
         }
     });
     constexpr int UNR = NS <= 8 ? 4 : 2;
@@ -90,8 +93,10 @@
             for (int u = 0; u < UNR; ++u) {
                 const int ca = ya[u][s] - dropa[s];
                 const int cb = (mode == 0 ? xb[u][s] : ya[u][s]) - dropb[s];
-                ya[u][s] = (s < na && live[u] && ca >= 0) ? offa[s] + ca * lbs : CP_NEG;
-                xb[u][s] = mode == 2 ? 0 : ((s < nb && cb >= 0) ? offb[s] + cb : CP_NEG);
+                const bool ina = s == 0 ? (unsigned)ca < cnta0 : ca >= 0;
+                const bool inb = s == 0 ? (unsigned)cb < cntb0 : cb >= 0;
+                ya[u][s] = (s < na && live[u] && ina) ? offa[s] + ca * lbs : CP_NEG;
+                xb[u][s] = mode == 2 ? 0 : ((s < nb && inb) ? offb[s] + cb : CP_NEG);
             }
         });
         static_for<NS>([&](auto ac) {
diff --git a/tabmat_amd/csrc/finish.hpp b/tabmat_amd/csrc/finish.hpp
--- /dev/null
+++ b/tabmat_amd/csrc/finish.hpp
@@ -0,0 +1,105 @@
+#pragma once
+#include "common.hpp"
+
+namespace tmh {
+
+struct FinishInto {
+    double *out;
+    int64_t p;
+    const int64_t *ri, *ci;
+};
+
+struct PanelMap {
+    int64_t W, cols;
+    __device__ bool operator()(int part, int64_t e, int64_t &a, int64_t &b) const {
+        a = e / W;
+        b = (int64_t)part * W + e % W;
+        return b < cols;
+    }
+};
+
+struct TriangleMap {
+    int TS;
+    int64_t m;
+    __device__ bool operator()(int part, int64_t e, int64_t &a, int64_t &b) const {
+        int I = 0;
+        while ((I + 1) * (I + 2) / 2 <= part) ++I;
+        const int J = part - I * (I + 1) / 2;
+        a = (int64_t)I * TS + e / TS;
+        b = (int64_t)J * TS + e % TS;
+        return a < m && b <= a;
+    }
+};
+
+template <typename F, int NW, typename Map>
+__global__ __launch_bounds__(NW * 64) void finish_partials_kernel(const F *__restrict__ ws, int64_t stride,
+                                                                  int nb, Map map, FinishInto fin) {
+    __shared__ double red[NW][64];
+    const int lane = threadIdx.x & 63;
+    const int wave = threadIdx.x >> 6;
+    const int64_t e = (int64_t)blockIdx.x * 64 + lane;
+    const int part = blockIdx.y;
+    double acc = 0.0;
+    if (e < stride) {
+        const F *p = ws + ((int64_t)part * nb) * stride + e;
+        for (int b = wave; b < nb; b += NW) acc += (double)p[(int64_t)b * stride];
+    }
+    red[wave][lane] = acc;
+    __syncthreads();
+    int64_t a, b;
+    if (wave == 0 && e < stride && map(part, e, a, b)) {
+        double s = 0.0;
+#pragma unroll
+        for (int w = 0; w < NW; w += 4)
+            s += (red[w][lane] + red[w + 1][lane]) + (red[w + 2][lane] + red[w + 3][lane]);
+        const double v = (double)(F)s;
+        const int64_t r = fin.ri[a], c = fin.ci[b];
+        if (r >= 0 && c >= 0) {
+            fin.out[r * fin.p + c] = v;
+            fin.out[c * fin.p + r] = v;
+        }
+    }
+}
+
+template <typename F, typename Map>
+inline int launch_finish_partials(const F *ws, int64_t stride, int nb, int n_parts, Map map,
+                                  const FinishInto &fin, hipStream_t st) {
+    dim3 grid((unsigned)ceil_div(stride, 64), (unsigned)n_parts);
+    const bool small = (int64_t)grid.x * grid.y < 1024 && nb > 16;
+    if (small)
+        hipLaunchKernelGGL((finish_partials_kernel<F, 16, Map>), grid, dim3(1024), 0, st, ws, stride, nb, map,
+                           fin);
+    else
+        hipLaunchKernelGGL((finish_partials_kernel<F, 4, Map>), grid, dim3(256), 0, st, ws, stride, nb, map,
+                           fin);
+    TM_LAUNCH_CHECK();
+    return TM_OK;
+}
+
+template <int UNUSED>
+__global__ void finish_zero_kernel(int64_t nr, int64_t nc, FinishInto fin) {
+    const int64_t e = (int64_t)blockIdx.x * blockDim.x + threadIdx.x;
+    if (e >= nr * nc) return;
+    const int64_t r = fin.ri[e / nc], c = fin.ci[e % nc];
+    if (r >= 0 && c >= 0) {
+        fin.out[r * fin.p + c] = 0.0;
+        fin.out[c * fin.p + r] = 0.0;
+    }
+}
+
+inline int launch_finish_zero(int64_t nr, int64_t nc, const FinishInto &fin, hipStream_t st) {
+    if (nr <= 0 || nc <= 0) return TM_OK;
+    hipLaunchKernelGGL(finish_zero_kernel<0>, dim3((unsigned)ceil_div(nr * nc, 256)), dim3(256), 0, st, nr, nc, fin);
+    TM_LAUNCH_CHECK();
+    return TM_OK;
+}
+
+inline int check_finish(const FinishInto &fin, const char *who) {
+    if (fin.out == nullptr || fin.ri == nullptr || fin.ci == nullptr || fin.p <= 0) {
+        set_error("%s: result, its order and both position arrays are needed", who);
+        return TM_EINVAL;
+    }
+    return TM_OK;
+}
+
+}
diff --git a/tabmat_amd/csrc/sparse_blocks.hip b/tabmat_amd/csrc/sparse_blocks.hip
--- a/tabmat_amd/csrc/sparse_blocks.hip
+++ b/tabmat_amd/csrc/sparse_blocks.hip
@@ -2,6 +2,7 @@
 
 #include "common.hpp"
 #include "reduce.hpp"
+#include "finish.hpp"
 
 namespace tmh {
 
@@ -202,9 +203,11 @@
 template <typename F, bool U8 = false, bool D12 = false>
 static int run_sparse_sandwich_blocks(const F *data, const int32_t *ind, const int32_t *cptr, int64_t n,
                                       int64_t m, int64_t nnz, const int32_t *blocks, const int32_t *wg_tab,
-                                      int n_wg, int max_nb, const F *d, F *out, hipStream_t st) {
+                                      int n_wg, int max_nb, const F *d, F *out, hipStream_t st,
+                                      const FinishInto *fin = nullptr) {
     if (m == 0) return TM_OK;
     if (n == 0 || nnz == 0 || n_wg == 0) {
+        if (fin) return launch_finish_zero(m, m, *fin, st);
         TM_HIP(hipMemsetAsync(out, 0, sizeof(F) * (size_t)(m * m), st));
         return TM_OK;
     }
@@ -233,6 +236,7 @@
                        max_nb, ws, wg_log_ptr());
     prof_end(st);
     TM_LAUNCH_CHECK();
+    if (fin) return launch_finish_partials<F>(ws, (int64_t)TS * TS, max_nb, n_parts, TriangleMap{TS, m}, *fin, st);
     rc = launch_reduce_partials<F>(ws, (int64_t)TS * TS, max_nb, n_parts, tmp, (int64_t)n_parts * TS * TS,
                                    false, st);
     if (rc) return rc;
@@ -295,4 +299,20 @@
                                                                tmh::as_stream(stream));
 }
 
-}
+#define TM_BLOCKS_INTO(NAME, F, D12)                                                                              \
+    int NAME(const F *cm_data, const uint8_t *cm_col8, const int32_t *cptr, int64_t n, int64_t m, int64_t nnz,   \
+             const int32_t *blocks, const int32_t *wg_tab, int n_wg, int max_nb, const F *d, double *res,        \
+             int64_t p, const int64_t *pos, void *stream) {                                                      \
+        const tmh::FinishInto fin{res, p, pos, pos};                                                             \
+        if (int rc = tmh::check_finish(fin, #NAME)) return rc;                                                   \
+        return tmh::run_sparse_sandwich_blocks<F, true, D12>(cm_data, reinterpret_cast<const int32_t *>(cm_col8), \
+                                                             cptr, n, m, nnz, blocks, wg_tab, n_wg, max_nb, d,   \
+                                                             nullptr, tmh::as_stream(stream), &fin);             \
+    }
+TM_BLOCKS_INTO(tm_sparse_sandwich_blocks_u8_into_f32, float, false)
+TM_BLOCKS_INTO(tm_sparse_sandwich_blocks_u8_into_f64, double, false)
+TM_BLOCKS_INTO(tm_sparse_sandwich_blocks_p12_into_f32, float, true)
+TM_BLOCKS_INTO(tm_sparse_sandwich_blocks_p12_into_f64, double, true)
+#undef TM_BLOCKS_INTO
+
+}
diff --git a/tabmat_amd/csrc/sparse_ent.hip b/tabmat_amd/csrc/sparse_ent.hip
--- a/tabmat_amd/csrc/sparse_ent.hip
+++ b/tabmat_amd/csrc/sparse_ent.hip
@@ -1,5 +1,6 @@
 #include "common.hpp"
 #include "reduce.hpp"
+#include "finish.hpp"
 
 namespace tmh {
 
@@ -360,7 +361,8 @@
 
 template <typename F>
 static int run_csr_dense_ent(const F *vals, const uint16_t *meta, const uint32_t *bstart, int64_t n, int64_t m,
-                             const F *B, int64_t r, const F *d, F *out, F *colsum, hipStream_t st) {
+                             const F *B, int64_t r, const F *d, F *out, F *colsum, hipStream_t st,
+                             const FinishInto *fin = nullptr) {
     const int64_t nB = r;
     const int64_t total = m * nB;
     if (total == 0) return TM_OK;
@@ -383,6 +385,7 @@
     const int nz = (int)ceil_div(n_groups, EN_NW);
     const bool want_csum = colsum != nullptr;
     if (n_slabs == 0) {
+        if (fin) return launch_finish_zero(m, nB, *fin, st);
         TM_HIP(hipMemsetAsync(out, 0, sizeof(F) * (size_t)total, st));
         if (want_csum) TM_HIP(hipMemsetAsync(colsum, 0, sizeof(F) * (size_t)m, st));
         return TM_OK;
@@ -411,6 +414,7 @@
                        reinterpret_cast<long long *>((uintptr_t)tune("ent_prof", 0)));
     prof_end(st);
     TM_LAUNCH_CHECK();
+    if (fin) return launch_finish_partials<F>(ws, stride, (int)nblk, n_parts, PanelMap{EN_W, nB}, *fin, st);
     rc = launch_reduce_partials<F>(ws, stride, (int)nblk, n_parts, tmp, n_parts * stride, false, st);
     if (rc) return rc;
     hipLaunchKernelGGL((en_untile_kernel<F>), dim3((unsigned)ceil_div(total, 256)), dim3(256), 0, st, tmp, m,
@@ -441,4 +445,20 @@
                                   double *colsum, void *stream) {
     return tmh::run_csr_dense_ent<double>(vals, meta, bstart, n, m, B, r, d, out, colsum, tmh::as_stream(stream));
 }
-}
+int tm_csr_dense_sandwich_ent_into_f32(const float *vals, const uint16_t *meta, const uint32_t *bstart, int64_t n,
+                                       int64_t m, const float *B, int64_t r, const float *d, double *res,
+                                       int64_t p, const int64_t *ri, const int64_t *ci, void *stream) {
+    const tmh::FinishInto fin{res, p, ri, ci};
+    if (int rc = tmh::check_finish(fin, "tm_csr_dense_sandwich_ent_into")) return rc;
+    return tmh::run_csr_dense_ent<float>(vals, meta, bstart, n, m, B, r, d, nullptr, nullptr, tmh::as_stream(stream),
+                                         &fin);
+}
+int tm_csr_dense_sandwich_ent_into_f64(const double *vals, const uint16_t *meta, const uint32_t *bstart, int64_t n,
+                                       int64_t m, const double *B, int64_t r, const double *d, double *res,
+                                       int64_t p, const int64_t *ri, const int64_t *ci, void *stream) {
+    const tmh::FinishInto fin{res, p, ri, ci};
+    if (int rc = tmh::check_finish(fin, "tm_csr_dense_sandwich_ent_into")) return rc;
+    return tmh::run_csr_dense_ent<double>(vals, meta, bstart, n, m, B, r, d, nullptr, nullptr, tmh::as_stream(stream),
+                                          &fin);
+}
+}
diff --git a/tabmat_amd/ext/sparse.py b/tabmat_amd/ext/sparse.py
--- a/tabmat_amd/ext/sparse.py
+++ b/tabmat_amd/ext/sparse.py
@@ -161,6 +161,21 @@
     return (out[A.inv], cs[A.inv]) if want_colsum else out[A.inv]
 
 
+def ent_kernel_positions(A: SlabEnt, pos):
+    import torch
+
+    kpos = torch.full((A.mk,), -1, dtype=torch.int64, device=pos.device)
+    kpos[A.inv] = pos.to(torch.int64)
+    return kpos
+
+
+def csr_dense_sandwich_ent_into(A: SlabEnt, B: DenseDev, d, out, kpos, pos_b):
+    assert B.n == A.n and ell_supported(B) and A.m > 0 and B.m > 0 and A.n > 0
+    D.same_float("csr_dense_sandwich_ent_into", A.vals, B.buf, d)
+    call("tm_csr_dense_sandwich_ent_into_" + D.fsuf(A.vals), D.p(A.vals), D.p(A.meta), D.p(A.bstart), A.n, A.mk,
+         D.p(B.buf), B.m, D.p(d), D.p(out), out.shape[0], D.p(kpos), D.p(pos_b), D.stream_ptr())
+
+
 def _row_table(A: CsrDev, rows, d, as_set: bool):
     import weakref
 
@@ -263,6 +278,19 @@
          int(cm_data.numel()), D.p(blocks), D.p(wg_tab), int(wg_tab.shape[0]), int(max_nb), D.p(d),
          D.p(out), D.stream_ptr())
     return out
+
+
+def sparse_sandwich_blocks_into(A: CsrDev, d, out, pos) -> bool:
+    if A.m == 0 or A.n == 0 or not K2B_U8:
+        return False
+    D.same_float("sparse_sandwich_blocks_into", A.data, d)
+    cm_data, cm_c8, cptr = A.chunk_major()
+    blocks, wg_tab, max_nb = A.pair_blocks(d12=None)
+    form = "p12" if int(blocks.shape[1]) == 3 else "u8"
+    call(f"tm_sparse_sandwich_blocks_{form}_into_{D.fsuf(A.data)}", D.p(cm_data), D.p(cm_c8), D.p(cptr), A.n, A.m,
+         int(cm_data.numel()), D.p(blocks), D.p(wg_tab), int(wg_tab.shape[0]), int(max_nb), D.p(d),
+         D.p(out), out.shape[0], D.p(pos), D.stream_ptr())
+    return True
 
 
 def sparse_sandwich_pairs(A: CsrDev, d):
diff --git a/tabmat_amd/ext/split.py b/tabmat_amd/ext/split.py
--- a/tabmat_amd/ext/split.py
+++ b/tabmat_amd/ext/split.py
@@ -96,8 +96,22 @@
 class CatPairsPlan:
 
     N_WG = 512
-
-    def __init__(self, cats, pos_arrays, diag_only=False):
+    MAX_PIECES = 4
+    ALL_LEVELS = 2**31 - 1
+
+    @staticmethod
+    def cut_pieces(li, lj, cap, max_pieces):
+        side = 0 if li >= lj else 1
+        long_, short = (li, lj) if side == 0 else (lj, li)
+        if short < 1 or short > cap:
+            return None
+        n = -(-long_ // (cap // short))
+        if n > max_pieces:
+            return None
+        size = -(-long_ // n)
+        return [(side, lo, min(size, long_ - lo)) for lo in range(0, long_, size)]
+
+    def __init__(self, cats, pos_arrays, diag_only=False, split=False):
         from .._lib import lib
         import torch
 
@@ -108,6 +122,8 @@
         roww = int(lib().tm_multi_cat_pairs_row_words())
         L = [int(c[1]) for c in cats]
         bundles = []
+        cut = []
+        self.split_pairs = []
         lone = []
 
         def tot(g):
@@ -119,9 +135,12 @@
 
         def cross(A, B):
             if tot(A) * tot(B) <= cap and len(A) <= slots and len(B) <= slots:
-                bundles.append((A, B, 0))
+                bundles.append((A, B, 0, None))
             elif len(A) == 1 and len(B) == 1:
-                return
+                pieces = self.cut_pieces(L[A[0]], L[B[0]], cap, self.MAX_PIECES) if split else None
+                if pieces is not None:
+                    cut.extend((A, B, 0, pc) for pc in pieces)
+                    self.split_pairs.append((self.cat_ids[A[0]], self.cat_ids[B[0]], pieces))
             elif len(B) == 1 or (len(A) > 1 and (tot(A) >= tot(B) or len(A) > slots)
                                  and not len(B) > slots):
                 a1, a2 = halves(A)
@@ -134,7 +153,7 @@
 
         def tri(G):
             if tot(G) ** 2 <= cap and len(G) <= slots:
-                bundles.append((G, G, 1))
+                bundles.append((G, G, 1, None))
             elif len(G) == 1:
                 lone.append(G[0])
             else:
@@ -153,14 +172,15 @@
             if L[a] > cap:
                 continue
             if cur and (tot(cur) + L[a] > cap or len(cur) >= slots):
-                bundles.append((cur, cur, 2))
+                bundles.append((cur, cur, 2, None))
                 cur = []
             cur.append(a)
         if cur:
-            bundles.append((cur, cur, 2))
+            bundles.append((cur, cur, 2, None))
+        bundles += cut
         self.n_bundles = len(bundles)
-        self.slots = max((max(len(A), len(B)) for A, B, _ in bundles), default=1)
-        def cost(A, B, mode):
+        self.slots = max((max(len(A), len(B)) for A, B, *_ in bundles), default=1)
+        def cost(A, B, mode, piece):
             nt = len(A) * len(B) if mode == 0 else (len(A) * (len(A) + 1) // 2 if mode == 1 else len(A))
             nl = len(A) + (len(B) if mode == 0 else 0)
             return nt + 0.5 * nl + 1.0
@@ -171,20 +191,43 @@
         rows_w = np.zeros((max(self.n_bundles, 1), roww), dtype=np.int32)
         pstart = self.pstart = np.concatenate([[0], np.cumsum(L)]).astype(np.int64)
         desc, self.pairs, wg_map = [], [], []
-        self.bins = max((tot(A) * (tot(B) if mode != 2 else 1) for A, B, mode in bundles), default=1)
-        for y, (A, B, mode) in enumerate(bundles):
-            width = tot(B) if mode != 2 else 1
+        def sides(A, B, piece):
+            LA, LB, fa, fb = [L[a] for a in A], [L[b] for b in B], [0] * len(A), [0] * len(B)
+            if piece is not None:
+                side, lo, cnt = piece
+                if side == 0:
+                    LA, fa = [cnt], [lo]
+                else:
+                    LB, fb = [cnt], [lo]
+            return LA, LB, fa, fb
+
+        def tile(A, B, mode, piece):
+            LA, LB, _, _ = sides(A, B, piece)
+            return sum(LA) * (sum(LB) if mode != 2 else 1)
+
+        self.bins = max((tile(*bd) for bd in bundles), default=1)
+        rng0 = 8 + 4 * slots
+        assert roww >= rng0 + 4
+        for y, (A, B, mode, piece) in enumerate(bundles):
+            LA, LB, fa, fb = sides(A, B, piece)
+            width = sum(LB) if mode != 2 else 1
             r = rows_w[y]
             r[0], r[1], r[2], r[3] = len(A), len(B), mode, width
-            r[4], r[5], r[6] = len(wg_map), share[y], tot(A) * width
+            r[4], r[5], r[6] = len(wg_map), share[y], sum(LA) * width
             wg_map += [y] * share[y]
-            ra = np.concatenate([[0], np.cumsum([L[a] for a in A])]).astype(np.int64)
-            cb = np.concatenate([[0], np.cumsum([L[b] for b in B])]).astype(np.int64)
+            ra = np.concatenate([[0], np.cumsum(LA)]).astype(np.int64)
+            cb = np.concatenate([[0], np.cumsum(LB)]).astype(np.int64)
             for s, a in enumerate(A):
                 r[8 + 2 * s], r[9 + 2 * s] = a, ra[s] * width
             for s, b in enumerate(B):
                 r[8 + 2 * slots + 2 * s], r[9 + 2 * slots + 2 * s] = b, (cb[s] if mode != 2 else 0)
+            r[rng0:rng0 + 4] = (0, self.ALL_LEVELS, 0, self.ALL_LEVELS) if piece is None else \
+                (fa[0], LA[0], fb[0], LB[0])
             base = y * self.bins
+            if piece is not None:
+                a, b = A[0], B[0]
+                desc.append([base, LA[0], LB[0], width, pstart[a] + fa[0], pstart[b] + fb[0], 0, 0])
+                continue
             for s, a in enumerate(A):
                 for t, b in enumerate(B):
                     if (mode == 1 and t < s) or (mode == 2 and t != s):
@@ -205,14 +248,14 @@
         self.h_wg_map = np.asarray(wg_map if wg_map else [0], dtype=np.int32)
         self.h_desc = np.asarray(desc, dtype=np.int64).reshape(-1, 8)
         if pos_arrays is None:
-            self.covered = {(min(i, j), max(i, j)) for i, j, *_ in self.pairs}
+            self.covered = {(min(i, j), max(i, j)) for i, j, *_ in self.pairs + self.split_pairs}
             return
         self.bundles = D.to_dev(rows_w.reshape(-1))
         self.wg_map = D.to_dev(self.h_wg_map)
         self.desc = D.to_dev(self.h_desc)
         self.pos = torch.cat([p.to(torch.int64) for p in pos_arrays]) if pos_arrays else \
             D.zeros((0,), torch.int64)
-        self.covered = {(min(i, j), max(i, j)) for i, j, *_ in self.pairs}
+        self.covered = {(min(i, j), max(i, j)) for i, j, *_ in self.pairs + self.split_pairs}
         self._cat_tab = (None, None)
 
     def cat_tab(self, cats):
@@ -368,6 +411,24 @@
     return res
 
 
+def multi_cat_dense_sandwich_into(cats, d, mat_j: DenseDev, out, gpos, pos_j):
+    assert sum(int(c[1]) for c in cats) > 0 and mat_j.m > 0 and mat_j.n > 0
+    codes, ncols, drop, n = _cat_args(cats)
+    D.same_float("multi_cat_dense_sandwich_into", mat_j.buf, d)
+    call(f"tm_multi_cat_dense_sandwich_into_{D.fsuf(mat_j.buf)}", codes, ncols, drop, n, mat_j.n,
+         D.p(d), D.p(mat_j.buf), mat_j.m, mat_j.order_f, D.p(out), out.shape[0], D.p(gpos), D.p(pos_j),
+         D.stream_ptr())
+
+
+def multi_cat_sparse_sandwich_ent_into(cats, d, E, packed, out, gpos, kpos):
+    assert sum(int(c[1]) for c in cats) > 0 and E.m > 0 and E.n > 0
+    codes, ncols, drop, n = _cat_args(cats)
+    D.same_float("multi_cat_sparse_sandwich_ent_into", E.vals, d)
+    call(f"tm_multi_cat_sparse_sandwich_ent_into_{D.fsuf(E.vals)}", codes, ncols, drop, n, E.n, D.p(d),
+         D.p(E.vals), D.p(E.meta), D.p(E.bstart), E.n_slots(), E.mk, D.p(packed), D.p(out), out.shape[0],
+         D.p(gpos), D.p(kpos), D.stream_ptr())
+
+
 def multi_cat_sparse_sandwich(cats, d, S: SlabCsc):
     total = sum(int(c[1]) for c in cats)
     if total == 0 or S.m == 0 or S.n == 0:
diff --git a/tabmat_amd/sparse_matrix.py b/tabmat_amd/sparse_matrix.py
--- a/tabmat_amd/sparse_matrix.py
+++ b/tabmat_amd/sparse_matrix.py
@@ -247,7 +247,14 @@
         t_narrow = 0.2e-3 + n * w * 4.5e-12 + nnz * w / max(mcols, 1) * 40e-12
         return t_narrow < 0.8 * t_full
 
-    def _sandwich_dev(self, d, rows, cols):
+    def _ent_kpos(self, pos):
+        ent = self._ent()
+        hit = self.__dict__.get("_ent_kpos_hit")
+        if hit is None or hit[0] is not ent or hit[1] is not pos:
+            hit = self.__dict__["_ent_kpos_hit"] = (ent, pos, xs.ent_kernel_positions(ent, pos))
+        return hit[2]
+
+    def _sandwich_dev(self, d, rows, cols, into=None):
         parts = self._row_parts()
         if parts is not None:
             out = None
@@ -328,6 +335,9 @@
             bl = getattr(self, "_blocks_pay", None)
             if bl is None:
                 bl = self._blocks_pay = xs.blocks_sandwich_pays(A)
+            if bl and into is not None and rows is None and cols is None \
+                    and xs.sparse_sandwich_blocks_into(A, d, *into):
+                return True
             res = xs.sparse_sandwich_blocks(A, d) if bl else xs.sparse_sandwich_chunked(A, d)
             if cols is not None:
                 c64 = cols.to(torch.int64)
@@ -426,7 +436,7 @@
                                  D.idx_dev(normalize_index(cols, self.shape[1])))
         return res if on_dev else D.to_host(res)
 
-    def _cross_sandwich_dev(self, other, d, rows, L_cols, R_cols, colsum_box=None):
+    def _cross_sandwich_dev(self, other, d, rows, L_cols, R_cols, colsum_box=None, into=None):
         from .categorical_matrix import CategoricalMatrix
         from .dense_matrix import DenseMatrix
 
@@ -466,6 +476,9 @@
                 if ent is not None and colsum_box is not None:
                     res, cs = xs.csr_dense_sandwich_ent(ent, Bd, d, want_colsum=True)
                     colsum_box.append(cs if L_cols is None else cs[L_cols.to(torch.int64)])
+                elif ent is not None and into is not None and rows is None and L_cols is None and R_cols is None:
+                    xs.csr_dense_sandwich_ent_into(ent, Bd, d, into[0], self._ent_kpos(into[1]), into[2])
+                    return True
                 elif ent is not None:
                     res = xs.csr_dense_sandwich_ent(ent, Bd, d)
                 elif lg is not None and colsum_box is not None:
diff --git a/tabmat_amd/split_matrix.py b/tabmat_amd/split_matrix.py
--- a/tabmat_amd/split_matrix.py
+++ b/tabmat_amd/split_matrix.py
@@ -32,6 +32,8 @@
 ROW_LIST_FRACTION_CATSPARSE = 0.04
 DIAG_FROM_PAIRS = True
 CAT_PAIRS_FUSED = os.environ.get("TABMAT_AMD_CAT_PAIRS", "1") != "0"
+CAT_PAIRS_SPLIT = os.environ.get("TABMAT_AMD_CAT_PAIRS_SPLIT", "1") != "0"
+FUSED_FINISH = os.environ.get("TABMAT_AMD_FUSED_FINISH", "1") != "0"
 FULL_THEN_SELECT = float(os.environ.get("TABMAT_AMD_FULL_THEN_SELECT", "0.5"))
 FULL_RESULT_MAX_BYTES = 256 << 20
 FULL_UNSELECTED_SHARE = 0.2
@@ -376,7 +378,8 @@
         return groups
 
     def _cat_pairs_plan(self):
-        plan = self.__dict__.get("_cp_plan", False)
+        key = "_cp_plan" if CAT_PAIRS_SPLIT else "_cp_plan_whole"
+        plan = self.__dict__.get(key, False)
         if plan is False:
             plan = None
             ids = [i for i, m in enumerate(self.matrices)
@@ -384,8 +387,8 @@
             if len(ids) >= 1:
                 pos = self._full_dev_indices()
                 plan = xsplit.CatPairsPlan([(i, self.matrices[i].shape[1]) for i in ids],
-                                           [pos[i] for i in ids])
-            self.__dict__["_cp_plan"] = plan
+                                           [pos[i] for i in ids], split=CAT_PAIRS_SPLIT)
+            self.__dict__[key] = plan
         return plan
 
     def _cat_hist_plan(self):
@@ -401,12 +404,18 @@
             self.__dict__["_ch_plan"] = plan
         return plan
 
-    def _fused_cats(self, mw, cats, cat_ids, d_eff, rows, total, budget, d_rows=None):
+    def _fused_cats(self, mw, cats, cat_ids, d_eff, rows, total, budget, d_rows=None, into=None):
         if isinstance(mw, DenseMatrix) and xsplit.multi_cat_dense_wide_ok(cats, mw._dev_c()):
             if rows is not None and D.nlen(rows) <= 0.5 * self.shape[0]:
                 return xsplit.multi_cat_dense_sandwich(cats, d_rows, mw._dev_c(), rows)
+            if into is not None and mw.shape[0] > 0:
+                xsplit.multi_cat_dense_sandwich_into(cats, d_eff, mw._dev_c(), *into)
+                return True
             return xsplit.multi_cat_dense_sandwich(cats, d_eff, mw._dev_c())
         if isinstance(mw, DenseMatrix) and xsplit.multi_cat_dense_tile_ok(cats, mw._dev_c()):
+            if into is not None and mw.shape[0] > 0:
+                xsplit.multi_cat_dense_sandwich_into(cats, d_eff, mw._dev_c(), *into)
+                return True
             return xsplit.multi_cat_dense_sandwich(cats, d_eff, mw._dev_c())
         if isinstance(mw, DenseMatrix):
             if xsplit.cat_dense_sorted_ok(mw._dev_c()):
@@ -431,6 +440,10 @@
                 key = tuple(cat_ids)
                 if key not in pk_cache:
                     pk_cache[key] = xsplit.pack_codes(cats)
+                if into is not None and ent.n > 0 and ent.m > 0:
+                    xsplit.multi_cat_sparse_sandwich_ent_into(cats, d_eff, ent, pk_cache[key], into[0], into[1],
+                                                              mw._ent_kpos(into[2]))
+                    return True
                 return xsplit.multi_cat_sparse_sandwich_ent(cats, d_eff, ent, pk_cache[key])
             return xsplit.multi_cat_sparse_sandwich(cats, d_eff, mw._slab())
         return None
@@ -457,6 +470,8 @@
                         break
                     k += 1
                 parts = [(a, b, self[a:b]) for a, b in zip(cuts[:-1], cuts[1:]) if b > a]
+                for _, _, part in parts:
+                    part.__dict__["_is_row_part"] = True
             self.__dict__["_row_parts"] = parts
         return parts
 
@@ -665,6 +680,9 @@
         from .ext import dense as xd
 
         mats = self.matrices
+        in_place = (FUSED_FINISH and rows is None and cols_host is None and colsum is None and center is None
+                    and xtv is None and not _cm.DETERMINISTIC and not self.__dict__.get("_is_row_part")
+                    and d.dtype == D.torch_dtype(self.dtype) and out.dtype == torch.float64)
         cat_ids = [i for i, m in enumerate(mats) if isinstance(m, CategoricalMatrix) and not empty[i]
                    and m.shape[1] > 0]
         budget = (128 * 1024) // 8
@@ -678,8 +696,18 @@
             for w, mw in enumerate(mats):
                 if empty[w] or mw.dtype != self.dtype or d.dtype != D.torch_dtype(self.dtype):
                     continue
-                stacked = self._fused_cats(mw, cats, grp, d_eff, rows, total, budget, d)
+                into = None
+                if in_place and total > 0 and mw.shape[1] > 0:
+                    cache = self.__dict__.setdefault("_group_pos", {})
+                    gpos = cache.get(tuple(grp))
+                    if gpos is None:
+                        gpos = cache[tuple(grp)] = torch.cat([pos_d[i] for i in grp])
+                    into = (out, gpos, pos_d[w])
+                stacked = self._fused_cats(mw, cats, grp, d_eff, rows, total, budget, d, into=into)
                 if stacked is None:
+                    continue
+                if stacked is True:
+                    done.update((min(i, w), max(i, w)) for i in grp)
                     continue
                 whole = cols_host is None and len(grp) > 1
                 if whole:
@@ -739,6 +767,7 @@
                         diag_scattered.add(i)
                 else:
                     done.add((i, j))
+            done.update((min(i, j), max(i, j)) for i, j, _ in plan.split_pairs)
         complete = [isinstance(m, CategoricalMatrix) and not m.drop_first and not m._has_missings
                     and sub_d[k] is None and not empty[k] for k, m in enumerate(mats)]
         for i, mi in enumerate(mats):
@@ -777,6 +806,10 @@
             elif isinstance(mi, DenseMatrix) and center is not None and center.get(i) is not None:
                 res = mi._sandwich_dev(d, rows, sub_d[i], center=center.get(i))
                 xsplit.scatter_block(res, pos_d[i], pos_d[i], out)
+            elif in_place and isinstance(mi, SparseMatrix):
+                res = mi._sandwich_dev(d, None, None, into=(out, pos_d[i]))
+                if res is not True:
+                    xsplit.scatter_block(res, pos_d[i], pos_d[i], out)
             else:
                 res = mi._sandwich_dev(d, rows, sub_d[i])
                 xsplit.scatter_block(res, pos_d[i], pos_d[i], out)
@@ -794,6 +827,13 @@
                                                        colsum_box=box)
                     if box:
                         colsum[si] = box[0]
+                    if si != i:
+                        res = res.T
+                elif in_place and isinstance(mats[si], SparseMatrix) and isinstance(mats[di], DenseMatrix):
+                    res = mats[si]._cross_sandwich_dev(mats[di], d, None, None, None,
+                                                       into=(out, pos_d[si], pos_d[di]))
+                    if res is True:
+                        continue
                     if si != i:
                         res = res.T
                 else:
```
